# li199603/easy_gaussian_splatting

Hardware: AMD Instinct MI355X
Metric: train iters/sec + forward render fps, 1M Gaussians @ 1080p (higher is better)
Workload: dtype f32

## Files before the change

easy_gaussian_splatting_amd/_native.py:

```python
from __future__ import annotations

import ctypes as ct
import os
import subprocess
import threading
from typing import Optional

_HERE = os.path.dirname(os.path.abspath(__file__))
LIB_PATH = os.environ.get("GS_LIB_PATH") or os.path.join(_HERE, "libgsraster.so")
CSRC_DIR = os.path.join(_HERE, "csrc")
VARIANT_DIR = os.path.join(os.path.dirname(_HERE), "build", "variants")

GS_TILE = 16
GS_BUCKET = 64
GS_UNIT = 32
GS_REC_FLOATS = 12
GS_ROW_FLOATS = 12
GS_ROUND_BASE, GS_ROUND_SPLIT, GS_ROUND_LIVE, GS_ROUND_FRONT_N, GS_ROUND_LISTED_ALL, GS_ROUND_WORDS = 0, 1, 2, 3, 4, 8

_lib: Optional[ct.CDLL] = None
_lock = threading.Lock()

_P = ct.c_void_p
_I = ct.c_int
_L = ct.c_int64
_F = ct.c_float
_Z = ct.c_size_t

SIGNATURES = {
    "gs_version": (_I, []),
    "gs_build_flags": (ct.c_char_p, []),
    "gs_last_error": (ct.c_char_p, []),
    "gs_arch": (ct.c_char_p, []),
    "gs_bin_groups": (_I, [_L]),
    "gs_bin_workspace_bytes": (_Z, [_I, _L, _I, _I]),
    "gs_project_fwd": (_I, [_P, _I, _L, _I, _I, _P, _P, _P, _P, _P, _P, _I, _P, _P, _I, _I, _F, _F, _F, _F, _I, _I, _I,
                            _P, _P, _P, _P, _P, _P, _P, _P, _P, _P]),
    "gs_bin_count": (_I, [_P, _I, _L, _I, _I, _P, _P, _Z, _P, _P, _P, _P, _P]),
    "gs_bin_emit_sort": (_I, [_P, _I, _L, _I, _I, _P, _P, _P, _Z, _P, _L, _L, _P, _P, _P, _P, _P, _P]),
    "gs_bins_workspace_bytes": (_Z, [_I, _L, _I, _I, _I, _L]),
    "gs_bins_count": (_I, [_P, _I, _L, _I, _I, _I, _P, _P, _P, _Z, _P, _L, _L, _P, _P, _P, _P, _P, _P]),
    "gs_bins_lists": (_I, [_P, _I, _L, _I, _I, _I, _P, _P, _Z, _P, _L, _P, _P, _P, _P, _P, _P]),
    "gs_walk_state_ints": (_Z, [_L]),
    "gs_blend_fwd": (_I, [_P, _I, _I, _I, _P, _P, _P, _P, _P, _P, _L, _P, _P, _P, _P, _P, _P, _P, _L, _P, _L, _P]),
    "gs_blend_bwd": (_I, [_P, _I, _I, _I, _P, _P, _P, _P, _L, _P, _P, _P, _P, _P, _P, _P, _P, _P, _P]),
    "gs_unit_classes_ints": (_Z, [_L, _I, _I, _I]),
    "gs_rec_colors": (_I, [_P, _I, _L, _I, _P, _I, _P, _P]),
    "gs_blend_fwd_ch": (_I, [_P, _I, _I, _I, _I, _P, _P, _P, _P, _P, _P, _L, _P, _P, _P, _P, _P, _P, _P, _L, _P, _L, _P, _P]),
    "gs_blend_bwd_ch": (_I, [_P, _I, _I, _I, _I, _P, _P, _P, _P, _L, _P, _P, _P, _P, _P, _P, _P, _P, _P, _P, _P]),
    "gs_channel_grads": (_I, [_P, _I, _L, _I, _I, _P, _P, _P, _P, _P, _P, _P]),
    "gs_project_bwd": (_I, [_P, _I, _L, _I, _I, _P, _P, _P, _P, _P, _I, _P, _P, _I, _I, _F, _F, _F,
                            _P, _P, _P, _P, _P, _P, _P, _P, _P, _P, _P, _P, _P, _P, _P, _P, _P, _P, _P, _I, _P, _P, _P, _P]),
    "gs_cam_partials_doubles": (_Z, [_I, _L]),
    "gs_project_bwd_cam": (_I, [_P, _I, _L, _I, _I, _P, _P, _P, _P, _P, _I, _P, _P, _I, _I, _F, _F, _F,
                                _P, _P, _P, _P, _P, _P, _P, _P, _P, _P, _P, _P, _P, _P, _P, _P, _P, _P, _P, _I, _P, _P, _P, _P,
                                _P, _P, _P]),
    "gs_row_sums": (_I, [_P, _I, _L, _P, _P, _P, _P, _P, _P, _P, _P, _P, _P, _F, _P, _P]),
    "gs_sh_adam_views": (_I, [_P, _I, _L, _I, _I, _P, _P, _L, _P, _P, _P, _P, _P, _P, _F, _F, _F, _F, _F, _L, _F, _P]),
    "gs_sh_grad_views": (_I, [_P, _I, _L, _I, _I, _P, _P, _P, _P, _P]),
    "gs_loss_workspace_floats": (_Z, [_I, _I]),
    "gs_l1_ssim_fwd": (_I, [_P, _I, _I, _F, _P, _P, _P, _I, _P, _P]),
    "gs_l1_ssim_bwd": (_I, [_P, _I, _I, _F, _P, _P, _P, _I, _P, _P, _P]),
    "gs_l1_ssim_fwd_slots": (_I, [_P, _I, _I, _F, _P, _P, _I, _I, _P, _P]),
    "gs_l1_ssim_bwd_slots": (_I, [_P, _I, _I, _F, _P, _P, _I, _P, _P, _P]),
    "gs_clamp01": (_I, [_P, _L, _P, _P, _P]),
    "gs_pack_view_step": (_I, [_P, _L, _F, _P, _P, _P, _P, _P, _P, _P]),
    "gs_update_statistics": (_I, [_P, _L, _F, _P, _P, _P, _P, _P]),
    "gs_guard_set": (_I, [_P, _L, _L]),
    "gs_guard_set_call": (_I, [_P, _L, _L]),
    "gs_info_mirror_set": (_I, [_P]),
    "gs_walk_mirror_set": (_I, [_P]),
    "gs_rounds_set": (_I, [_P, _P, _P, _P, _I]),
    "gs_round_split": (_I, [_P, _L, _P, _P, _F, _P, _P]),
    "gs_round_footprints": (_I, [_P, _L, _I, _I, _P, _P, _P, _P]),
    "gs_round_status": (_I, [_P, _P, _P]),
    "gs_step_status": (_I, [_P, _P, _P, _P, _P, _P, _I, _P]),
    "gs_guard_flag_out": (_I, [_P, _P, _P, _P]),
    "gs_guard_merge": (_I, [_P, _P, _P, _I, _L]),
    "gs_step_applied": (_I, [_P, _P, _P]),
    "gs_adam_hyper": (_I, [_P, _I, _P, _F, _F, _L, _P]),
    "gs_step_inputs": (_I, [_P, _I, _P, _F, _F, _L, _P, _P, _P, _P, _P, _P, _P, _P]),
    "gs_adam_step_dev": (_I, [_P, _L, _P, _P, _P, _I, _P, _P, _P, _F, _F, _F, _F, _P, _P]),
    "gs_scan_rows_workspace_ints": (_Z, [_I, _L]),
    "gs_scan_rows_i32": (_I, [_P, _I, _L, _P, _P, _P]),
    "gs_refine_flags": (_I, [_P, _L, _I, _F, _F, _F, _F, _F, _P, _P, _P, _P, _P, _P, _P]),
    "gs_refine_apply": (_I, [_P, _L, _I, _I, _P, _P, _L, _L, _L, _P, _P, _P, _P, _P, _P, _P, _P, _P, _P, _P]),
    "gs_project_bwd_adam": (_I, [_P, _L, _I, _I, _P, _P, _P, _P, _P, _P, _I, _I, _F, _F, _F, _P, _P, _P, _P, _P, _P, _P, _P, _F, _F, _F, _P, _P,
                                  _P, _P, _P, _P]),
    "gs_project_bwd_adam_reg": (_I, [_P, _L, _I, _I, _P, _P, _P, _P, _P, _P, _I, _I, _F, _F, _F, _P, _P, _P, _P, _P, _P, _P, _P, _F, _F, _F, _P,
                                      _P, _P, _P, _P, _P, _F, _F]),
    "gs_scale_reg_workspace_floats": (_Z, [_L]),
    "gs_scale_reg": (_I, [_P, _L, _P, _F, _F, _P, _P, _P]),
    "gs_workspace_query": (_I, [_I, _L, _I, _I, _L, _L, _L, _L, _I, _I, _P, _P]),
    "gs_workspace_bind": (_I, [_P, _P, _L, _P, _L, _P, _L, _P, _P]),
    "gs_adam_step": (_I, [_P, _L, _P, _P, _P, _I, _P, _P, _P, _P, _F, _F, _F, _L, _F]),
    "gs_adam_step_stats": (_I, [_P, _L, _P, _P, _P, _I, _P, _P, _P, _P, _F, _F, _F, _L, _F, _L, _P, _P, _P, _P]),
}


class NativeLibraryError(RuntimeError):
    pass


def build(verbose: bool = False, clean: bool = False) -> str:
    if clean:
        subprocess.run(["make", "-C", CSRC_DIR, "clean"], capture_output=True, text=True)
    proc = subprocess.run(["make", "-C", CSRC_DIR, "-j4"], capture_output=True, text=True)
    if verbose or proc.returncode != 0:
        print(proc.stdout)
        print(proc.stderr)
    if proc.returncode != 0:
        raise NativeLibraryError("building libgsraster.so failed:\n" + proc.stderr[-4000:])
    return LIB_PATH


def build_variant(name: str, extra_flags: str) -> str:
    import glob
    import shutil
    import tempfile
    os.makedirs(VARIANT_DIR, exist_ok=True)
    out = os.path.join(VARIANT_DIR, f"libgsraster_{name}.so")
    srcs = [f for pat in ("*.hip", "*.h", "*.inc", "Makefile") for f in glob.glob(os.path.join(CSRC_DIR, pat))]
    if os.path.exists(out) and all(os.path.getmtime(out) >= os.path.getmtime(f) for f in srcs + [os.path.join(_HERE, "..", "include", "gs_raster.h")]):
        return out
    d = tempfile.mkdtemp(prefix=f"gsvar_{name}_")
    try:
        header = os.path.abspath(os.path.join(_HERE, "..", "include", "gs_raster.h"))
        for f in srcs:
            text = open(f).read().replace("../../include/gs_raster.h", header)
            open(os.path.join(d, os.path.basename(f)), "w").write(text)
        proc = subprocess.run(["make", "-C", d, "-j4", f"EXTRA={extra_flags}", f"LIB={out}"], capture_output=True, text=True)
        if proc.returncode != 0:
            raise NativeLibraryError(f"building {out} failed:\n" + proc.stderr[-4000:])
    finally:
        shutil.rmtree(d, ignore_errors=True)
    return out


def lib() -> ct.CDLL:
    global _lib
    if _lib is None:
        with _lock:
            if _lib is None:
                if not os.path.exists(LIB_PATH):
                    raise NativeLibraryError(
# ... 28 lines not shown
```

easy_gaussian_splatting_amd/csrc/gs_blend.hip:

```cpp
#include <algorithm>

#include "gs_common.h"
#include "gs_math.h"

namespace gs {

#ifdef GS_BWD_CHECK
struct BwdCheck {
    float* fwd_T;
    int32_t* fwd_cnt;
    float2* unit_out;
    int2* unit_hdr;
};
static BwdCheck g_bwd_check = {nullptr, nullptr, nullptr, nullptr};
#define GS_IF_CHECK(...) __VA_ARGS__
#else
#define GS_IF_CHECK(...)
#endif

constexpr int kUnit = GS_UNIT;
constexpr int kChunk = 8;
constexpr int kUnitLog = 128;
constexpr int kWalkUnits = GS_WALK_UNITS, kWalkStorage = GS_WALK_STORAGE, kWalkRows = GS_WALK_ROWS,
              kWalkFlags = GS_WALK_FLAGS, kWalkSkip = GS_WALK_SKIP;
constexpr int kScanThreads = 256, kScanPerThread = 32, kScanChunk = kScanThreads * kScanPerThread;

struct BlendFwdArgs {
    const int32_t* tile_order;
    int C, W, H, tw, tiles;
    const float4* rec;
    const float* bg;
    const int32_t *isect_offsets, *flatten_ids, *slots;
    float *out_colors, *out_alphas;
    float4* ckpt;
    int2* qlist;
    int32_t* qcnt;
    uint8_t* qmask;
    int4* unit_desc;
    int32_t* walk;
    int cap_units;
    unsigned long long* flags;
    const int64_t* guard;
    int64_t* rblk;
    uint8_t* live;
    float4* tstate;
    int4* trec;
    int solo;
    GS_IF_CHECK(BwdCheck chk;)
};

#ifdef GS_CLOCK_PROBE
__device__ unsigned long long gs_clk_acc[4];
struct ClockProbe {
    long long c0, w0; int slot;
    __device__ ClockProbe(int s) : c0(clock64()), w0(wall_clock64()), slot(s) {}
    __device__ ~ClockProbe() {
        if ((threadIdx.x & 63) == 0) {
            atomicAdd(&gs_clk_acc[slot], (unsigned long long)(clock64() - c0));
            atomicAdd(&gs_clk_acc[slot + 1], (unsigned long long)(wall_clock64() - w0));
        }
    }
};
#define GS_CLOCK_PROBE_SCOPE(slot) ClockProbe clock_probe_(slot)
#else
#define GS_CLOCK_PROBE_SCOPE(slot)
#endif

#ifdef GS_EXACT_MATH
__device__ __forceinline__ float fast_exp2(float x) { return (float)exp2((double)x); }
__device__ __forceinline__ float fast_rcp(float x) { return (float)(1.0 / (double)x); }
#else
__device__ __forceinline__ float fast_exp2(float x) { return __builtin_amdgcn_exp2f(x); }
__device__ __forceinline__ float fast_rcp(float x) { return __builtin_amdgcn_rcpf(x); }
#endif

constexpr float kDoneScale = 18446744073709551616.f;
constexpr float kDoneInv = 5.421010862427522e-20f;
__device__ __forceinline__ bool px_live(float T) { return T <= 1.f; }
__device__ __forceinline__ float px_final_T(float T) { return T > 2.f ? T * kDoneInv : T; }
__device__ __forceinline__ void blend_masked(const float am, const float r, const float g, const float b, float& T, float& cr,
                                             float& cg, float& cb) {
    float w = am * T;
    float Tn = fmaf(-am, T, T);
    const bool stop = Tn <= kTMin;
    if (__builtin_expect(__builtin_amdgcn_ballot_w64(stop) != 0ull, 0)) {
        w = stop ? 0.f : w;
        Tn = stop ? T * kDoneScale : Tn;
    }
    cr = fmaf(r, w, cr); cg = fmaf(g, w, cg); cb = fmaf(b, w, cb);
    T = Tn;
}
__device__ __forceinline__ void blend_pair(const float alpha, const bool ok, const float r,
                                           const float g, const float b, float& T, float& cr,
                                           float& cg, float& cb) {
    blend_masked(ok ? alpha : 0.f, r, g, b, T, cr, cg, cb);
}
__device__ __forceinline__ void blend_masked4(const float am, const float r, const float g, const float b, const float c3, float& T,
                                              float& cr, float& cg, float& cb, float& ca) {
    float w = am * T;
    float Tn = fmaf(-am, T, T);
    const bool stop = Tn <= kTMin;
    if (__builtin_expect(__builtin_amdgcn_ballot_w64(stop) != 0ull, 0)) {
        w = stop ? 0.f : w;
        Tn = stop ? T * kDoneScale : Tn;
    }
    cr = fmaf(r, w, cr); cg = fmaf(g, w, cg); cb = fmaf(b, w, cb); ca = fmaf(c3, w, ca);
    T = Tn;
}
__device__ __forceinline__ void blend_pair4(const float alpha, const bool ok, const float r, const float g, const float b,
                                            const float c3, float& T, float& cr, float& cg, float& cb, float& ca) {
    blend_masked4(ok ? alpha : 0.f, r, g, b, c3, T, cr, cg, cb, ca);
}

#define GS_FWD_ATTR __attribute__((amdgpu_waves_per_eu(CKPT ? 5 : 1, 8)))

__device__ __forceinline__ int64_t slots_in_use(int64_t n, const int64_t* guard) {
    return guard != nullptr ? min(n, guard[0]) : n;
}

__global__ __launch_bounds__(256) void qmask_clear_kernel(uint8_t* __restrict__ q, int64_t n_cap, int32_t* __restrict__ walk, int walk_ints,
                                                          const int64_t* __restrict__ guard, const int64_t* __restrict__ rblk, int phase) {
    bool skip = guard_tripped(guard);
    if (phase == 2) skip = skip || walk[kWalkSkip] != 0;
    if (blockIdx.x == 0 && threadIdx.x == 0) walk[kWalkSkip] = skip ? 1 : 0;
    if (skip) return;
    const int64_t first = phase == 2 ? min(rblk[GS_ROUND_BASE], slots_in_use(n_cap, guard)) : 0;
    const int64_t n = slots_in_use(n_cap, guard) - first;
    q += first;
    if (phase != 2)
        for (int i = (int)blockIdx.x * 256 + (int)threadIdx.x; i < walk_ints; i += (int)gridDim.x * 256)
            if (i != kWalkSkip) walk[i] = 0;
    const int64_t head = min(n, (int64_t)((16 - ((uintptr_t)q & 15)) & 15));
    const int64_t n16 = (n - head) >> 4;
    uint4* q16 = reinterpret_cast<uint4*>(q + head);
    for (int64_t i = (int64_t)blockIdx.x * 256 + threadIdx.x; i < n16; i += (int64_t)gridDim.x * 256) q16[i] = make_uint4(0u, 0u, 0u, 0u);
    if (blockIdx.x == 0) {
        if ((int64_t)threadIdx.x < head) q[threadIdx.x] = 0;
        const int64_t tail0 = head + (n16 << 4);
        if (tail0 + (int64_t)threadIdx.x < n) q[tail0 + threadIdx.x] = 0;
    }
}

template <bool CKPT, int WAVES, int ROUND, int NC>
__device__ __forceinline__ void blend_fwd_body(const BlendFwdArgs& a, float* __restrict__ ckpt_ext) {
    static_assert(NC >= 1 && NC <= 4 && (NC == 3 || ROUND == 0), "channels 1..4; depth rounds with 3 channels only");
    __shared__ float4 srec_all[WAVES][GS_BUCKET * 3];
    __shared__ int2 ulog_all[CKPT ? WAVES : 1][CKPT ? kUnitLog : 1];
    __shared__ int uring_all[CKPT ? WAVES : 1][CKPT ? 16 : 1];
    float4* srec = srec_all[threadIdx.x >> 6];
    int2* ulog = ulog_all[CKPT ? (threadIdx.x >> 6) : 0];
    int* uring = uring_all[CKPT ? (threadIdx.x >> 6) : 0];
    const int ti = CKPT ? __builtin_amdgcn_readfirstlane((int)blockIdx.x * WAVES + (int)(threadIdx.x >> 6))
                        : (int)blockIdx.x * WAVES + (int)(threadIdx.x >> 6);
    if (ti >= a.C * a.tiles) return;
    if (CKPT ? a.walk[kWalkSkip] != 0 : guard_tripped(a.guard)) return;
    if (ROUND == 2 && a.rblk[GS_ROUND_LIVE] == 0) return;
    GS_CLOCK_PROBE_SCOPE(0);
    const int t = a.tile_order ? a.tile_order[ti] : ti;
    const int cam = t / a.tiles, tt = t - cam * a.tiles;
    const int tyi = tt / a.tw, txi = tt - tyi * a.tw;
    const int lane = threadIdx.x & 63;
    const int x0 = txi * GS_TILE, y0 = tyi * GS_TILE;
    const int px0 = x0 + (lane & 7), py0 = y0 + (lane >> 3);
    const float fx0 = (float)px0 + 0.5f, fy0 = (float)py0 + 0.5f, fx1 = fx0 + 8.f, fy1 = fy0 + 8.f;
    const int lo = a.isect_offsets[t], hi = a.isect_offsets[t + 1];
    const int len = hi - lo;
    const int nb = (len + GS_BUCKET - 1) / GS_BUCKET;
    const unsigned long long lt_mask = (1ull << lane) - 1ull;
    if (ROUND == 2 && (len == 0 || a.live[t] == 0)) return;

    float T[4], cr[4], cg[4], cb[4];
    float ca[4];
    int cnt[4] = {0, 0, 0, 0};
    int pool_next = 0, pool_left = 0, log_n = 0;
    int room[4] = {0, 0, 0, 0};
    const int range_len = (a.cap_units / GS_WALK_RANGES) & ~(kChunk - 1), range0 = (ti & (GS_WALK_RANGES - 1)) * range_len;
    int32_t* range_ctr = a.walk + GS_WALK_RANGE0 + 32 * (ti & (GS_WALK_RANGES - 1));
    GS_IF_CHECK(int taken[4] = {0, 0, 0, 0};)
#pragma unroll
    for (int k = 0; k < 4; ++k) {
        cr[k] = cg[k] = cb[k] = 0.f;
        ca[k] = 0.f;
        T[k] = ((px0 + 8 * (k & 1)) < a.W && (py0 + 8 * (k >> 1)) < a.H) ? 1.f : kDoneScale;
    }
    if (ROUND == 2) {
#pragma unroll
        for (int k = 0; k < 4; ++k) {
            const float4 s4 = a.tstate[((size_t)t * 4 + k) * 64 + lane];
            T[k] = s4.x; cr[k] = s4.y; cg[k] = s4.z; cb[k] = s4.w;
        }
        if (CKPT) {
            const int4 rc = a.trec[2 * (size_t)t], ru = a.trec[2 * (size_t)t + 1];
            cnt[0] = __builtin_amdgcn_readfirstlane(rc.x); cnt[1] = __builtin_amdgcn_readfirstlane(rc.y);
            cnt[2] = __builtin_amdgcn_readfirstlane(rc.z); cnt[3] = __builtin_amdgcn_readfirstlane(rc.w);
            const int ru4[4] = {ru.x, ru.y, ru.z, ru.w};
#pragma unroll
            for (int k = 0; k < 4; ++k) {
                room[k] = -cnt[k] & (kUnit - 1);
                if (lane == 0 && cnt[k] > 0) uring[4 * k + (((cnt[k] - 1) / kUnit) & 3)] = ru4[k];
            }
        }
    }
    const float qxlo[2] = {(float)x0 + 0.5f, (float)x0 + 8.5f}, qxhi[2] = {(float)x0 + 7.5f, (float)x0 + 15.5f};
    const float qylo[2] = {(float)y0 + 0.5f, (float)y0 + 8.5f}, qyhi[2] = {(float)y0 + 7.5f, (float)y0 + 15.5f};

    auto publish = [&]() {
        if (log_n == 0) return;
        int base = 0;
        if (lane == 0) base = atomicAdd(a.walk + kWalkUnits, log_n);
        base = __builtin_amdgcn_readfirstlane(base);
        __builtin_amdgcn_wave_barrier();
        for (int j = lane; j < log_n; j += 64) {
            const int2 e = ulog[j];
            if (base + j < a.cap_units) a.unit_desc[base + j] = make_int4(4 * t + (e.y & 3), e.y >> 2, e.x, 0);
// ... 115 lines not shown
    if (ROUND == 1) {
        const bool lv = __builtin_amdgcn_ballot_w64(px_live(T[0]) || px_live(T[1]) || px_live(T[2]) || px_live(T[3])) != 0ull;
        if (lane == 0) {
            a.live[t] = lv ? 1 : 0;
            if (lv) atomicAdd(reinterpret_cast<unsigned long long*>(a.rblk + GS_ROUND_LIVE), 1ull);
            if (lv && a.solo && a.flags) atomicOr(a.flags, (unsigned long long)GS_FLAG_BACK);
        }
        if (lv && !a.solo) {
#pragma unroll
            for (int k = 0; k < 4; ++k) a.tstate[((size_t)t * 4 + k) * 64 + lane] = make_float4(T[k], cr[k], cg[k], cb[k]);
            if (CKPT && lane == 0) {
                a.trec[2 * (size_t)t] = make_int4(cnt[0], cnt[1], cnt[2], cnt[3]);
                int ru[4];
#pragma unroll
                for (int k = 0; k < 4; ++k) ru[k] = cnt[k] > 0 ? uring[4 * k + (((cnt[k] - 1) / kUnit) & 3)] : 0;
                a.trec[2 * (size_t)t + 1] = make_int4(ru[0], ru[1], ru[2], ru[3]);
            }
        }
    }
    float bgr = 0.f, bgg = 0.f, bgb = 0.f, bga = 0.f;
    if (a.bg) {
        bgr = a.bg[NC * cam];
        if (NC > 1) bgg = a.bg[NC * cam + 1];
        if (NC > 2) bgb = a.bg[NC * cam + 2];
        if (NC > 3) bga = a.bg[NC * cam + 3];
    }
#pragma unroll
    for (int k = 0; k < 4; ++k) {
        const int px = px0 + 8 * (k & 1), py = py0 + 8 * (k >> 1);
        if (px < a.W && py < a.H) {
            const size_t o = ((size_t)cam * a.H + py) * a.W + px;
            const float Tf = px_final_T(T[k]);
            a.out_colors[NC * o] = cr[k] + Tf * bgr;
            if (NC > 1) a.out_colors[NC * o + 1] = cg[k] + Tf * bgg;
            if (NC > 2) a.out_colors[NC * o + 2] = cb[k] + Tf * bgb;
            if (NC > 3) a.out_colors[NC * o + 3] = ca[k] + Tf * bga;
            a.out_alphas[o] = 1.f - Tf;
            GS_IF_CHECK(if (CKPT && a.chk.fwd_T) { a.chk.fwd_T[o] = Tf; a.chk.fwd_cnt[o] = taken[k]; })
        }
    }
}

template <bool CKPT, int WAVES, int ROUND>
__global__ __launch_bounds__(64 * WAVES) GS_FWD_ATTR void blend_fwd_kernel(const BlendFwdArgs a) {
    blend_fwd_body<CKPT, WAVES, ROUND, 3>(a, nullptr);
}
template <bool CKPT, int WAVES, int NC>
__global__ __launch_bounds__(64 * WAVES) __attribute__((amdgpu_waves_per_eu(CKPT ? (NC == 4 ? 4 : 5) : 1, 8))) void chan_fwd_kernel(const BlendFwdArgs a, float* ckpt_ext) {
    blend_fwd_body<CKPT, WAVES, 0, NC>(a, ckpt_ext);
}

struct RowScanArgs {
    const uint8_t* qmask;
    int32_t* row_base;
    int32_t* walk;
    int64_t n_cap, cap_rows;
    unsigned long long* flags;
    const int64_t* guard;
    volatile int64_t* mirror;
};

__device__ __forceinline__ int32_t row_counts32(const uint8_t* __restrict__ qmask, int64_t i0, int64_t n, uint32_t (&w)[8]) {
#pragma unroll
    for (int j = 0; j < 8; ++j) w[j] = 0u;
    if (i0 + kScanPerThread <= n) {
        const uint4 x = reinterpret_cast<const uint4*>(qmask + i0)[0], y = reinterpret_cast<const uint4*>(qmask + i0)[1];
        w[0] = x.x; w[1] = x.y; w[2] = x.z; w[3] = x.w; w[4] = y.x; w[5] = y.y; w[6] = y.z; w[7] = y.w;
    } else {
        for (int j = 0; j < kScanPerThread; ++j)
            if (i0 + j < n) w[j >> 2] |= (uint32_t)qmask[i0 + j] << (8 * (j & 3));
    }
    int32_t tot = 0;
#pragma unroll
    for (int j = 0; j < 8; ++j) {
        uint32_t v = w[j] & 0x0f0f0f0fu;
        v = v - ((v >> 1) & 0x55555555u);
        v = (v & 0x33333333u) + ((v >> 2) & 0x33333333u);
        w[j] = v;
        tot += (int32_t)((v * 0x01010101u) >> 24);
    }
    return tot;
}

__global__ __launch_bounds__(kScanThreads) void row_count_kernel(const RowScanArgs a) {
    __shared__ int32_t scratch[20];
    if (a.walk[kWalkSkip] != 0) return;
    const int64_t n = slots_in_use(a.n_cap, a.guard);
    const int64_t c0 = (int64_t)blockIdx.x * kScanChunk;
    if (c0 > n) return;
    uint32_t w[8];
    const int32_t tot = row_counts32(a.qmask, c0 + (int64_t)threadIdx.x * kScanPerThread, n, w);
    int32_t block_tot;
    block_excl_scan_add<int32_t>(tot, scratch, &block_tot);
    if (threadIdx.x == 0) a.walk[GS_WALK_WORDS + blockIdx.x] = block_tot;
}

__global__ __launch_bounds__(1024) void row_chunk_scan_kernel(const RowScanArgs a) {
    __shared__ int32_t scratch[20];
    if (a.walk[kWalkSkip] != 0) return;
    const int64_t n = slots_in_use(a.n_cap, a.guard);
    const int nb = (int)(n / kScanChunk) + 1;
    int32_t* part = a.walk + GS_WALK_WORDS;
    const int per = (nb + 1023) / 1024;
    const int j0 = (int)threadIdx.x * per, j1 = min(nb, j0 + per);
    int32_t mine = 0;
    for (int j = j0; j < j1; ++j) mine += part[j];
    int32_t total;
    int32_t run = block_excl_scan_add<int32_t>(mine, scratch, &total);
    for (int j = j0; j < j1; ++j) { const int32_t c = part[j]; part[j] = run; run += c; }
    if (threadIdx.x == 0) {
        int32_t fullest = 0;
        for (int r = 0; r < GS_WALK_RANGES; ++r) fullest = max(fullest, a.walk[GS_WALK_RANGE0 + 32 * r]);
        a.walk[kWalkStorage] = GS_WALK_RANGES * fullest;
        a.walk[kWalkRows] = total;
        int fl = a.walk[kWalkFlags];
        if (a.flags && (fl & GS_FLAG_UNITS)) atomicOr(a.flags, (unsigned long long)GS_FLAG_UNITS);
        if ((int64_t)total > a.cap_rows) {
            fl |= GS_FLAG_ROWS;
            a.walk[kWalkFlags] = fl;
            if (a.flags) atomicOr(a.flags, (unsigned long long)GS_FLAG_ROWS);
        }
        if (a.mirror) {
            a.mirror[0] = a.walk[kWalkUnits]; a.mirror[1] = a.walk[kWalkStorage]; a.mirror[2] = total; a.mirror[3] = fl;
            __threadfence_system();
        }
    }
}

__global__ __launch_bounds__(kScanThreads) void row_base_kernel(const RowScanArgs a) {
    __shared__ int32_t scratch[20];
    if (a.walk[kWalkSkip] != 0) return;
    const int64_t n = slots_in_use(a.n_cap, a.guard);
    const int64_t c0 = (int64_t)blockIdx.x * kScanChunk;
    if (c0 > n) return;
    const int64_t i0 = c0 + (int64_t)threadIdx.x * kScanPerThread;
    uint32_t w[8];
    const int32_t tot = row_counts32(a.qmask, i0, n, w);
    int32_t block_tot;
    const int32_t run = block_excl_scan_add<int32_t>(tot, scratch, &block_tot) + a.walk[GS_WALK_WORDS + blockIdx.x];
    int32_t first16 = 0;
#pragma unroll
    for (int j = 0; j < 4; ++j) first16 += (int32_t)((w[j] * 0x01010101u) >> 24);
    if (i0 <= n) a.row_base[i0 >> 4] = run;
    if (i0 + 16 <= n) a.row_base[(i0 >> 4) + 1] = run + first16;
}

struct BlendBwdArgs {
    int C, W, H, tw, tiles;
    const float4* rec;
    const int32_t* walk;
    const int2* qlist;
    const int32_t* qcnt;
    const int4* unit_desc;
    const float4* ckpt;
    const uint8_t* qmask;
    const int32_t* row_base;
    int cap_units;
    const int32_t* cls_hdr;
    const int4* cls_desc;
    int cls_cap;
    const float *out_colors, *out_alphas, *v_colors, *v_alphas;
    float4* rows;
    const int64_t* guard;
    GS_IF_CHECK(BwdCheck chk;)
};

constexpr int kBwdWaves = 4;
constexpr int kPipeLanes = 8;
constexpr int kPerLane = kUnit / kPipeLanes;
static_assert(kPerLane == 4, "bwd_wave is instantiated for 1 .. 4 entries per lane");
constexpr int kUnitsPerWave = 64 / kPipeLanes;
constexpr int kUnitPixels = 64;
constexpr int kBwdSteps = kUnitPixels + kPipeLanes - 1;

__device__ __forceinline__ float dpp_row_shr1(float v) {
    return __builtin_bit_cast(float, __builtin_amdgcn_update_dpp(__builtin_bit_cast(int, v), __builtin_bit_cast(int, v), 0x111, 0xf, 0xf, false));
}


#ifdef GS_BWD_ACC64
typedef double acc_t;
#define GS_ACC_FMA(a, b, c) ((double)(a) * (double)(b) + (c))
#else
typedef float acc_t;
#define GS_ACC_FMA(a, b, c) fmaf((a), (b), (c))
#endif
struct EntryState {
    float mx, my, hA, Bc, hC, op, colr, colg, colb, At, Bt, Ct;
    acc_t s_mx, s_my, s_ax, s_ay, s_A, s_B, s_C, s_vs, s_r, s_g, s_b;
    bool has;
    float col3; acc_t s_3;
};

template <int NC>
__device__ __forceinline__ void bwd_pair(EntryState& e, const float4 d0, const float v3, const float2 d1, float& T, float& P) {
    const float dx = e.mx - d1.x, dy = e.my - d1.y;
    const float sigma = fmaf(dy, fmaf(e.hC, dy, e.Bc * dx), e.hA * dx * dx);
    const float vis = fast_exp2(-sigma);
    const float ov = e.op * vis;
    const float alpha = fminf(kAlphaMax, ov);
    const bool ok = T > 0.f && sigma >= 0.f && alpha >= kAlphaMin;
    const float w = alpha * T;
    const float Tn = fmaf(-alpha, T, T);
    const bool stop = ok && Tn <= kTMin;
    const bool contrib = ok && !stop;
    float cv = e.colr * d0.x + e.colg * d0.y + e.colb * d0.z;
    if constexpr (NC == 4) cv = fmaf(e.col3, v3, cv);
    const float wm = contrib ? w : 0.f;
    const float Pn = fmaf(wm, cv, P);
    const float ra = fast_rcp(1.f - alpha);
    const float v_alpha = fmaf(T, cv, ra * (d0.w + Pn));
    e.s_r = GS_ACC_FMA(wm, d0.x, e.s_r); e.s_g = GS_ACC_FMA(wm, d0.y, e.s_g); e.s_b = GS_ACC_FMA(wm, d0.z, e.s_b);
    if constexpr (NC == 4) e.s_3 = GS_ACC_FMA(wm, v3, e.s_3);
    const float vs = (contrib && ov <= kAlphaMax) ? -ov * v_alpha : 0.f;
    const float hx = vs * dx, hy = vs * dy;
    e.s_A = GS_ACC_FMA(hx, dx, e.s_A); e.s_B = GS_ACC_FMA(hx, dy, e.s_B); e.s_C = GS_ACC_FMA(hy, dy, e.s_C);
    const float gx = fmaf(e.At, hx, e.Bt * hy), gy = fmaf(e.Bt, hx, e.Ct * hy);
    e.s_mx += (acc_t)gx; e.s_my += (acc_t)gy; e.s_ax += (acc_t)fabsf(gx); e.s_ay += (acc_t)fabsf(gy);
    e.s_vs += (acc_t)vs;
    T = contrib ? Tn : (stop ? -1.f : T);
    P = Pn;
}

template <int E, int NC>
__device__ __forceinline__ void bwd_wave(const BlendBwdArgs& a, const int4 ud, const bool valid, const int unit, float4* sd0, float* sd1,
                                         float2* sck, const int r, const float* __restrict__ ckpt_ext) {
    const int tq = ud.x, su = ud.z;
// ... 52 lines not shown
    }
#pragma unroll
    for (int i = 0; i < kPix; ++i) {
        const int p = r + kPipeLanes * i;
        const bool inside = valid && (qx0 + (p & 7)) < a.W && (qy0 + (p >> 3)) < a.H;
        const float vr = l_vr[i], vg = l_vg[i], vb = l_vb[i];
        const float Tf = 1.f - l_oa[i];
        const float va = a.v_alphas ? l_va[i] : 0.f;
        float Ev = Tf * va - (l_cr[i] * vr + l_cg[i] * vg + l_cb[i] * vb);
        const float4 ck = first_unit ? make_float4(1.f, 0.f, 0.f, 0.f) : l_ck[i];
        float Pk = ck.y * vr + ck.z * vg + ck.w * vb;
        if constexpr (NC == 4) {
            const float v3 = l_v3[i];
            Ev = Tf * va - fmaf(l_c3[i], v3, l_cr[i] * vr + l_cg[i] * vg + l_cb[i] * vb);
            Pk = fmaf(first_unit ? 0.f : l_k3[i], v3, Pk);
            sd1[p] = inside ? v3 : 0.f;
        }
        sd0[p] = inside ? make_float4(vr, vg, vb, Ev) : make_float4(0.f, 0.f, 0.f, 0.f);
        sck[p] = inside ? make_float2(ck.x, Pk) : make_float2(-1.f, 0.f);
    }

    EntryState e[E];
    int slot[E];
#pragma unroll
    for (int i = 0; i < E; ++i) {
        const int en = E * r + i;
        e[i].has = en < n_in;
        slot[i] = e[i].has ? gs[i].y : 0;
        const float4 z4 = make_float4(0.f, 0.f, 0.f, 0.f);
        const float4 q0 = e[i].has ? rq[i][0] : z4, q1 = e[i].has ? rq[i][1] : z4, q2 = e[i].has ? rq[i][2] : z4;
        e[i].mx = q0.x; e[i].my = q0.y; e[i].hA = q0.z; e[i].Bc = q0.w; e[i].hC = q1.x; e[i].op = q1.y;
        e[i].colr = q2.x; e[i].colg = q2.y; e[i].colb = q2.z;
        e[i].col3 = q2.w; e[i].s_3 = (acc_t)0;
        e[i].At = 2.f * kLn2 * q0.z; e[i].Bt = kLn2 * q0.w; e[i].Ct = 2.f * kLn2 * q1.x;
        e[i].s_mx = e[i].s_my = e[i].s_ax = e[i].s_ay = e[i].s_A = e[i].s_B = e[i].s_C = e[i].s_vs = (acc_t)0;
        e[i].s_r = e[i].s_g = e[i].s_b = (acc_t)0;
    }
    __builtin_amdgcn_wave_barrier();

    float T_out = -1.f, P_out = 0.f;
    GS_IF_CHECK(float D_out = -1.f, C_out = 0.f; if (valid && r == 0 && a.chk.unit_hdr) a.chk.unit_hdr[unit] = make_int2(tq, ud.y);)
    for (int s = 0; s < kBwdSteps; ++s) {
        float T = dpp_row_shr1(T_out), P = dpp_row_shr1(P_out);
        const int p = s - r;
        const bool act = (unsigned)p < (unsigned)kUnitPixels;
        const int pc = min(max(p, 0), kUnitPixels - 1);
        const float4 d0 = sd0[pc];
        const float v3 = NC == 4 ? sd1[pc] : 0.f;
        const float2 ck = sck[pc];
        const float2 d1 = make_float2(fx0 + (float)(pc & 7), fy0 + (float)(pc >> 3));
        if (r == 0) { T = ck.x; P = ck.y; }
        T = act ? T : -1.f;
        GS_IF_CHECK(float D = dpp_row_shr1(D_out), Cn = dpp_row_shr1(C_out); if (r == 0) { D = ck.x; Cn = 0.f; } if (!act) { D = -1.f; Cn = 0.f; })
#pragma unroll
        for (int i = 0; i < E; ++i) {
            GS_IF_CHECK(const float T_before = T;)
            bwd_pair<NC>(e[i], d0, v3, d1, T, P);
            GS_IF_CHECK(if (T > 0.f && T < T_before) { D = T; Cn += 1.f; })
        }
        GS_IF_CHECK(D_out = D; C_out = Cn;
                    if (valid && act && r == kPipeLanes - 1 && a.chk.unit_out) a.chk.unit_out[(size_t)unit * 64 + p] = make_float2(D, Cn);)
        T_out = T; P_out = P;
    }

    int row[E];
#pragma unroll
    for (int i = 0; i < E; ++i) {
        int m;
        row[i] = rows_before(a.row_base, a.qmask, slot[i], &m);
        row[i] += __popc((unsigned)m & ((1u << q) - 1u));
    }
#pragma unroll
    for (int i = 0; i < E; ++i) {
        if (e[i].has) {
            float4* rp = a.rows + (GS_ROW_FLOATS / 4) * (size_t)row[i];
            const float v_op = e[i].op > 0.f ? (float)(-e[i].s_vs / (acc_t)e[i].op) : 0.f;
            rp[0] = make_float4((float)e[i].s_mx, (float)e[i].s_my, (float)e[i].s_ax, (float)e[i].s_ay);
            rp[1] = make_float4((float)((acc_t)0.5f * e[i].s_A), (float)e[i].s_B, (float)((acc_t)0.5f * e[i].s_C), v_op);
            rp[2] = make_float4((float)e[i].s_r, (float)e[i].s_g, (float)e[i].s_b, NC == 4 ? (float)e[i].s_3 : 0.f);
        }
    }
}

constexpr int kClsHdrInts = 16, kClsThreads = 1024;
__global__ __launch_bounds__(64) void unit_classes_clear_kernel(int32_t* __restrict__ hdr) {
    if (threadIdx.x < kClsHdrInts) hdr[threadIdx.x] = 0;
}
__global__ __launch_bounds__(kClsThreads) void unit_classes_kernel(const int32_t* __restrict__ walk, const int4* __restrict__ unit_desc,
                                                                   const int32_t* __restrict__ qcnt, int cap_units, int cls_cap,
                                                                   int32_t* __restrict__ hdr, int4* __restrict__ cls, const int64_t* __restrict__ guard) {
    __shared__ int s_cnt[kClsThreads / 64][4], s_base[kClsThreads / 64][4];
    if (guard_tripped(guard)) return;
    const int n_units = min(walk[kWalkUnits], cap_units);
    if ((int)blockIdx.x * kClsThreads >= n_units) return;
    const int u = (int)blockIdx.x * kClsThreads + (int)threadIdx.x, wave = threadIdx.x >> 6, lane = threadIdx.x & 63;
    int c = 0;
    int4 ud = make_int4(0, 0, 0, 0);
    if (u < n_units) {
        ud = unit_desc[u];
        const int n_in = min(kUnit, qcnt[ud.x] - ud.y * kUnit);
        c = min(max((n_in + kPipeLanes - 1) / kPipeLanes, 1), 4);
        ud.w = u;
    }
    unsigned long long m[4];
#pragma unroll
    for (int k = 0; k < 4; ++k) m[k] = __ballot(c == k + 1);
    if (lane < 4) s_cnt[wave][lane] = (int)__popcll(lane == 0 ? m[0] : (lane == 1 ? m[1] : (lane == 2 ? m[2] : m[3])));
    __syncthreads();
    if (threadIdx.x < 4) {
        int tot = 0;
        for (int w = 0; w < kClsThreads / 64; ++w) { s_base[w][threadIdx.x] = tot; tot += s_cnt[w][threadIdx.x]; }
        const int base = tot ? atomicAdd(hdr + 1 + threadIdx.x, tot) : 0;
        for (int w = 0; w < kClsThreads / 64; ++w) s_base[w][threadIdx.x] += base;
    }
    __syncthreads();
    if (c) {
        const unsigned long long mine = c == 1 ? m[0] : (c == 2 ? m[1] : (c == 3 ? m[2] : m[3]));
        const int i = s_base[wave][c - 1] + (int)__popcll(mine & ((1ull << lane) - 1ull));
        if (i < (c == 4 ? cap_units : cls_cap)) cls[(c == 4 ? 0 : cap_units + (3 - c) * cls_cap) + i] = ud;
    }
}

template <int NC>
__device__ __forceinline__ void blend_bwd_body(const BlendBwdArgs& a, const float* __restrict__ ckpt_ext) {
    __shared__ float4 sd0_all[kBwdWaves][kUnitsPerWave][64];
    __shared__ float2 sck_all[kBwdWaves][kUnitsPerWave][64];
    const int wave = threadIdx.x >> 6, lane = threadIdx.x & 63;
    const int pipe = lane / kPipeLanes, r = lane & (kPipeLanes - 1);
    if (guard_tripped(a.guard)) return;
    constexpr int kPerBlock = kBwdWaves * kUnitsPerWave;
    int cls = 4, blk = (int)blockIdx.x, n_units, first = 0;
    if (a.cls_hdr == nullptr) {
        n_units = min(a.walk[kWalkUnits], a.cap_units);
    } else {
        const int b4 = (a.cap_units + kPerBlock - 1) / kPerBlock, bt = (a.cls_cap + kPerBlock - 1) / kPerBlock;
        if (blk >= b4) {
            const int k = (blk - b4) / bt;
            cls = 3 - k; blk -= b4 + k * bt; first = a.cap_units + k * a.cls_cap;
        }
        n_units = min(a.cls_hdr[cls], cls == 4 ? a.cap_units : a.cls_cap);
    }
    const int in_class = (blk * kBwdWaves + wave) * kUnitsPerWave + pipe;
    if ((blk * kBwdWaves + wave) * kUnitsPerWave >= n_units) return;
    GS_CLOCK_PROBE_SCOPE(2);
    const bool valid = in_class < n_units;
    float4* sd0 = sd0_all[wave][pipe];
    float2* sck = sck_all[wave][pipe];
    float* sd1 = nullptr;
    if constexpr (NC == 4) {
        __shared__ float sd1_all[kBwdWaves][kUnitsPerWave][64];
        sd1 = sd1_all[wave][pipe];
    }

    int4 ud = make_int4(0, 0, 0, 0);
    if (valid) ud = a.cls_hdr ? a.cls_desc[first + in_class] : a.unit_desc[in_class];
    const int unit = a.cls_hdr ? ud.w : in_class;
    if (cls == 4) bwd_wave<4, NC>(a, ud, valid, unit, sd0, sd1, sck, r, ckpt_ext);
    else if (cls == 3) bwd_wave<3, NC>(a, ud, valid, unit, sd0, sd1, sck, r, ckpt_ext);
    else if (cls == 2) bwd_wave<2, NC>(a, ud, valid, unit, sd0, sd1, sck, r, ckpt_ext);
    else bwd_wave<1, NC>(a, ud, valid, unit, sd0, sd1, sck, r, ckpt_ext);
}

__global__ __launch_bounds__(kBwdWaves * 64) void blend_bwd_kernel(const BlendBwdArgs a) {
    blend_bwd_body<3>(a, nullptr);
}
template <int NC>
__global__ __launch_bounds__(kBwdWaves * 64) void chan_bwd_kernel(const BlendBwdArgs a, const float* ckpt_ext) {
    blend_bwd_body<NC>(a, ckpt_ext);
}

}

using namespace gs;

#ifdef GS_BWD_CHECK
extern "C" int gs_debug_bwd_check_set(float* fwd_T, int32_t* fwd_cnt, float* unit_out, int32_t* unit_hdr) {
    g_bwd_check.fwd_T = fwd_T; g_bwd_check.fwd_cnt = fwd_cnt;
    g_bwd_check.unit_out = reinterpret_cast<float2*>(unit_out); g_bwd_check.unit_hdr = reinterpret_cast<int2*>(unit_hdr);
    return GS_OK;
}
#endif

#ifdef GS_CLOCK_PROBE
extern "C" int gs_debug_clock_probe(int64_t* out4, int reset) {
    unsigned long long h[4] = {0, 0, 0, 0};
    if (out4) { GS_HIP_CHECK(hipMemcpyFromSymbol(h, HIP_SYMBOL(gs_clk_acc), sizeof(h))); for (int i = 0; i < 4; ++i) out4[i] = (int64_t)h[i]; }
    if (reset) { unsigned long long z[4] = {0, 0, 0, 0}; GS_HIP_CHECK(hipMemcpyToSymbol(HIP_SYMBOL(gs_clk_acc), z, sizeof(z))); }
    return GS_OK;
}
#endif

extern "C" size_t gs_walk_state_ints(int64_t n_isects) {
    if (n_isects < 0) return 0;
    return (size_t)GS_WALK_WORDS + (size_t)(n_isects / kScanChunk + 1);
}

template <int NC>
static int blend_fwd_launch(void* stream, int C, int width, int height, const float* rec,
                            const float* backgrounds, const int32_t* isect_offsets, const int32_t* tile_order,
                            const int32_t* flatten_ids, const int32_t* slots, int64_t n_isects, float* render_colors,
                            float* render_alphas, float* ckpt, int32_t* qlist, int32_t* qcnt, uint8_t* qmask,
                            int32_t* unit_desc, int64_t cap_units, int32_t* row_base, int64_t cap_rows, int32_t* walk_state,
                            float* ckpt_ext) {
    GS_REQUIRE(C >= 1 && width > 0 && height > 0 && n_isects >= 0, "C>=1, positive image size, n_isects>=0");
    GS_REQUIRE(isect_offsets && render_colors && render_alphas, "null pointer");
    const bool train = ckpt != nullptr;
    GS_REQUIRE(!train || (qlist && qcnt && qmask && unit_desc && row_base && walk_state && slots), "training mode needs every list output");
    GS_REQUIRE(!train || (cap_units >= kChunk * GS_WALK_RANGES && cap_units < (1ll << 26) && cap_rows >= 0 && cap_rows < (1ll << 31)),
               "training mode: 256 <= cap_units < 2^26 work units, cap_rows < 2^31 gradient rows");
    GS_REQUIRE(!train || n_isects < (1ll << 31) - kScanChunk, "training mode: the slots of a call are indexed by int32");
    static_assert(kScanPerThread == 32, "row_base_kernel writes two groups of 16 slots per thread");
    GS_REQUIRE(!train || (((uintptr_t)qmask & 15) == 0 && ((uintptr_t)row_base & 15) == 0 && ((uintptr_t)walk_state & 7) == 0),
               "training mode: qmask / row_base 16-byte aligned, walk_state 8-byte aligned");
    BlendFwdArgs a;
    a.C = C; a.W = width; a.H = height;
    a.tw = (width + GS_TILE - 1) / GS_TILE;
    a.tiles = a.tw * ((height + GS_TILE - 1) / GS_TILE);
    a.rec = reinterpret_cast<const float4*>(rec); a.bg = backgrounds; a.isect_offsets = isect_offsets;
    a.flatten_ids = flatten_ids; a.slots = slots;
    a.out_colors = render_colors; a.out_alphas = render_alphas;
    a.ckpt = reinterpret_cast<float4*>(ckpt); a.qlist = reinterpret_cast<int2*>(qlist); a.qcnt = qcnt; a.qmask = qmask;
    a.unit_desc = reinterpret_cast<int4*>(unit_desc); a.walk = walk_state; a.cap_units = (int)cap_units;
    a.tile_order = tile_order;
    a.guard = current_guard().info;
    a.flags = a.guard ? reinterpret_cast<unsigned long long*>(const_cast<int64_t*>(a.guard) + 3) : nullptr;
    const Rounds R = current_rounds();
    const int phase = (R.phase == 1 || R.phase == 4) ? 1 : (R.phase == 2 ? 2 : 0);
    a.solo = R.phase == 4 ? 1 : 0;
    GS_REQUIRE(R.phase != 4 || a.flags != nullptr, "depth rounds, front round alone: needs a step guard (gs_guard_set)");
    GS_REQUIRE(phase == 0 || C == 1, "depth rounds: one camera per call");
    GS_REQUIRE(phase == 0 || !train || R.tile_rec, "depth rounds, training mode: gs_rounds_set needs tile_rec");
    GS_REQUIRE(NC == 3 || phase == 0, "depth rounds render 3 channels only (tile_state holds T, r, g, b): clear gs_rounds_set");
    GS_REQUIRE(NC != 4 || !train || ckpt_ext, "channels = 4, training mode: ckpt_ext (cap_units * 64 floats) is required");
    a.rblk = R.blk; a.live = R.live; a.tstate = R.state; a.trec = reinterpret_cast<int4*>(R.tile_rec);
    GS_IF_CHECK(a.chk = g_bwd_check;)
    const unsigned n_tiles = (unsigned)(C * a.tiles);
    hipStream_t st = (hipStream_t)stream;
    constexpr int kFwdWaves = 4;
    const dim3 grid((n_tiles + kFwdWaves - 1) / kFwdWaves), block(64 * kFwdWaves);
    if (train) {
        const int walk_ints = (int)gs_walk_state_ints(n_isects);
        const unsigned cg = (unsigned)std::min<int64_t>(1024, std::max<int64_t>(1, (n_isects / 16 + 255) / 256));
        hipLaunchKernelGGL(qmask_clear_kernel, dim3(cg), dim3(256), 0, st, qmask, n_isects, walk_state, walk_ints, a.guard,
                           (const int64_t*)R.blk, phase);
        GS_LAUNCH_CHECK("qmask_clear_kernel");
        if constexpr (NC != 3) hipLaunchKernelGGL((chan_fwd_kernel<true, kFwdWaves, NC>), grid, block, 0, st, a, ckpt_ext);
        else if (phase == 1) hipLaunchKernelGGL((blend_fwd_kernel<true, kFwdWaves, 1>), grid, block, 0, st, a);
        else if (phase == 2) hipLaunchKernelGGL((blend_fwd_kernel<true, kFwdWaves, 2>), grid, block, 0, st, a);
        else hipLaunchKernelGGL((blend_fwd_kernel<true, kFwdWaves, 0>), grid, block, 0, st, a);
        GS_LAUNCH_CHECK("blend_fwd_kernel");
        if (phase == 1 && !a.solo) return GS_OK;
        RowScanArgs s;
        s.qmask = qmask; s.row_base = row_base; s.walk = walk_state; s.n_cap = n_isects; s.cap_rows = cap_rows;
        s.flags = a.flags; s.guard = a.guard; s.mirror = current_walk_mirror();
        const unsigned chunks = (unsigned)(n_isects / kScanChunk + 1);
        hipLaunchKernelGGL(row_count_kernel, dim3(chunks), dim3(kScanThreads), 0, st, s);
        hipLaunchKernelGGL(row_chunk_scan_kernel, dim3(1), dim3(1024), 0, st, s);
        hipLaunchKernelGGL(row_base_kernel, dim3(chunks), dim3(kScanThreads), 0, st, s);
        GS_LAUNCH_CHECK("row_base_kernel");
    } else {
        if constexpr (NC != 3) hipLaunchKernelGGL((chan_fwd_kernel<false, kFwdWaves, NC>), grid, block, 0, st, a, nullptr);
        else if (phase == 1) hipLaunchKernelGGL((blend_fwd_kernel<false, kFwdWaves, 1>), grid, block, 0, st, a);
        else if (phase == 2) hipLaunchKernelGGL((blend_fwd_kernel<false, kFwdWaves, 2>), grid, block, 0, st, a);
        else hipLaunchKernelGGL((blend_fwd_kernel<false, kFwdWaves, 0>), grid, block, 0, st, a);
        GS_LAUNCH_CHECK("blend_fwd_kernel");
    }
    return GS_OK;
}

extern "C" int gs_blend_fwd(void* stream, int C, int width, int height, const float* rec,
                            const float* backgrounds, const int32_t* isect_offsets, const int32_t* tile_order,
                            const int32_t* flatten_ids, const int32_t* slots, int64_t n_isects, float* render_colors,
                            float* render_alphas, float* ckpt, int32_t* qlist, int32_t* qcnt, uint8_t* qmask,
                            int32_t* unit_desc, int64_t cap_units, int32_t* row_base, int64_t cap_rows, int32_t* walk_state) {
    return blend_fwd_launch<3>(stream, C, width, height, rec, backgrounds, isect_offsets, tile_order, flatten_ids, slots, n_isects,
                               render_colors, render_alphas, ckpt, qlist, qcnt, qmask, unit_desc, cap_units, row_base, cap_rows,
                               walk_state, nullptr);
}

extern "C" int gs_blend_fwd_ch(void* stream, int C, int width, int height, int channels, const float* rec,
                               const float* backgrounds, const int32_t* isect_offsets, const int32_t* tile_order,
                               const int32_t* flatten_ids, const int32_t* slots, int64_t n_isects, float* render_colors,
                               float* render_alphas, float* ckpt, int32_t* qlist, int32_t* qcnt, uint8_t* qmask,
                               int32_t* unit_desc, int64_t cap_units, int32_t* row_base, int64_t cap_rows, int32_t* walk_state,
                               float* ckpt_ext) {
    GS_REQUIRE(channels >= 1 && channels <= 4, "channels must be 1, 2, 3 or 4");
#define GS_FWD_CH(NC) blend_fwd_launch<NC>(stream, C, width, height, rec, backgrounds, isect_offsets, tile_order, flatten_ids, slots, \
                                           n_isects, render_colors, render_alphas, ckpt, qlist, qcnt, qmask, unit_desc, cap_units,   \
                                           row_base, cap_rows, walk_state, ckpt_ext)
    switch (channels) {
        case 1: return GS_FWD_CH(1);
        case 2: return GS_FWD_CH(2);
        case 3: return GS_FWD_CH(3);
        default: return GS_FWD_CH(4);
    }
#undef GS_FWD_CH
}

static int64_t cls_region(int C, int width, int height) {
    const int64_t tiles = (int64_t)((width + GS_TILE - 1) / GS_TILE) * ((height + GS_TILE - 1) / GS_TILE);
    const int64_t per_block = kBwdWaves * kUnitsPerWave;
    return (4 * (int64_t)C * tiles + per_block - 1) / per_block * per_block;
}

extern "C" size_t gs_unit_classes_ints(int64_t cap_units, int C, int width, int height) {
    if (cap_units < 0 || C < 1 || width <= 0 || height <= 0) return 0;
    return (size_t)kClsHdrInts + 4 * ((size_t)cap_units + 3 * (size_t)cls_region(C, width, height));
}

template <int NC>
static int blend_bwd_launch(void* stream, int C, int width, int height, const float* rec,
                            const int32_t* qlist, const int32_t* qcnt, const int32_t* unit_desc, int64_t cap_units,
                            const float* ckpt, const uint8_t* qmask, const int32_t* row_base, const int32_t* walk_state,
                            const float* render_colors, const float* render_alphas, const float* v_render_colors,
                            const float* v_render_alphas, float* rows, int32_t* unit_classes, const float* ckpt_ext) {
    GS_REQUIRE(C >= 1 && width > 0 && height > 0 && cap_units >= 0 && cap_units < (1ll << 26), "C>=1, positive image size, 0 <= cap_units < 2^26");
    if (cap_units == 0) return GS_OK;
    GS_REQUIRE(rec && qlist && qcnt && unit_desc && ckpt && qmask && row_base && walk_state, "null list pointer");
    GS_REQUIRE(render_colors && render_alphas && v_render_colors && rows, "null image pointer");
    GS_REQUIRE(NC != 4 || ckpt_ext, "channels = 4: ckpt_ext (gs_blend_fwd_ch's fourth-channel checkpoints) is required");
    BlendBwdArgs a;
    a.C = C; a.W = width; a.H = height;
    a.tw = (width + GS_TILE - 1) / GS_TILE;
    a.tiles = a.tw * ((height + GS_TILE - 1) / GS_TILE);
    a.rec = reinterpret_cast<const float4*>(rec);
    a.qlist = reinterpret_cast<const int2*>(qlist); a.qcnt = qcnt; a.walk = walk_state;
    a.unit_desc = reinterpret_cast<const int4*>(unit_desc); a.cap_units = (int)cap_units;
    a.ckpt = reinterpret_cast<const float4*>(ckpt); a.qmask = qmask; a.row_base = row_base;
    a.out_colors = render_colors;
    a.out_alphas = render_alphas; a.v_colors = v_render_colors; a.v_alphas = v_render_alphas;
    a.rows = reinterpret_cast<float4*>(rows);
    a.guard = current_guard().info;
    GS_IF_CHECK(a.chk = g_bwd_check;)
    unsigned grid = (unsigned)((cap_units + kUnitsPerWave * kBwdWaves - 1) / (kUnitsPerWave * kBwdWaves));
    a.cls_hdr = nullptr; a.cls_desc = nullptr; a.cls_cap = 0;
    if (unit_classes) {
        GS_REQUIRE(((uintptr_t)unit_classes & 15) == 0, "unit_classes must be 16-byte aligned");
        a.cls_hdr = unit_classes; a.cls_desc = reinterpret_cast<const int4*>(unit_classes + kClsHdrInts);
        a.cls_cap = (int)cls_region(C, width, height);
        hipLaunchKernelGGL(unit_classes_clear_kernel, dim3(1), dim3(64), 0, (hipStream_t)stream, unit_classes);
        hipLaunchKernelGGL(unit_classes_kernel, dim3((unsigned)((cap_units + kClsThreads - 1) / kClsThreads)), dim3(kClsThreads), 0, (hipStream_t)stream,
                           walk_state, a.unit_desc, qcnt, (int)cap_units, a.cls_cap, unit_classes, reinterpret_cast<int4*>(unit_classes + kClsHdrInts),
                           a.guard);
        GS_LAUNCH_CHECK("unit_classes_kernel");
        grid += 3u * (unsigned)(a.cls_cap / (kUnitsPerWave * kBwdWaves));
    }
    if constexpr (NC == 3) hipLaunchKernelGGL(blend_bwd_kernel, dim3(grid), dim3(kBwdWaves * 64), 0, (hipStream_t)stream, a);
    else hipLaunchKernelGGL((chan_bwd_kernel<NC>), dim3(grid), dim3(kBwdWaves * 64), 0, (hipStream_t)stream, a, ckpt_ext);
    GS_LAUNCH_CHECK("blend_bwd_kernel");
    return GS_OK;
}

extern "C" int gs_blend_bwd(void* stream, int C, int width, int height, const float* rec,
                            const int32_t* qlist, const int32_t* qcnt, const int32_t* unit_desc, int64_t cap_units,
                            const float* ckpt, const uint8_t* qmask, const int32_t* row_base, const int32_t* walk_state,
                            const float* render_colors, const float* render_alphas, const float* v_render_colors,
                            const float* v_render_alphas, float* rows, int32_t* unit_classes) {
    return blend_bwd_launch<3>(stream, C, width, height, rec, qlist, qcnt, unit_desc, cap_units, ckpt, qmask, row_base, walk_state,
                               render_colors, render_alphas, v_render_colors, v_render_alphas, rows, unit_classes, nullptr);
}

extern "C" int gs_blend_bwd_ch(void* stream, int C, int width, int height, int channels, const float* rec,
                               const int32_t* qlist, const int32_t* qcnt, const int32_t* unit_desc, int64_t cap_units,
                               const float* ckpt, const uint8_t* qmask, const int32_t* row_base, const int32_t* walk_state,
                               const float* render_colors, const float* render_alphas, const float* v_render_colors,
                               const float* v_render_alphas, float* rows, int32_t* unit_classes, const float* ckpt_ext) {
    GS_REQUIRE(channels >= 1 && channels <= 4, "channels must be 1, 2, 3 or 4");
#define GS_BWD_CH(NC) blend_bwd_launch<NC>(stream, C, width, height, rec, qlist, qcnt, unit_desc, cap_units, ckpt, qmask, row_base, \
                                           walk_state, render_colors, render_alphas, v_render_colors, v_render_alphas, rows,         \
                                           unit_classes, ckpt_ext)
    switch (channels) {
        case 1: return GS_BWD_CH(1);
        case 2: return GS_BWD_CH(2);
        case 3: return GS_BWD_CH(3);
        default: return GS_BWD_CH(4);
    }
#undef GS_BWD_CH
}
```

easy_gaussian_splatting_amd/csrc/gs_capi.hip:

```cpp
#include <stdarg.h>

#include "gs_common.h"

namespace gs {
static thread_local char g_err[512] = "";
void set_error(const char* fmt, ...) {
    va_list ap;
    va_start(ap, fmt);
    vsnprintf(g_err, sizeof(g_err), fmt, ap);
    va_end(ap);
}
static thread_local Guard g_guard = {nullptr, 0, 0, 0};
Guard current_guard() { return g_guard; }
static thread_local int64_t* g_info_mirror = nullptr;
int64_t* current_info_mirror() { return g_info_mirror; }
static thread_local int64_t* g_walk_mirror = nullptr;
int64_t* current_walk_mirror() { return g_walk_mirror; }
static thread_local Rounds g_rounds = {nullptr, nullptr, nullptr, nullptr, 0};
Rounds current_rounds() { return g_rounds; }
}

extern "C" int gs_rounds_set(int64_t* rounds_dev, uint8_t* tile_live, float* tile_state, int32_t* tile_rec, int phase) {
    if (phase < 0 || phase > 4 || (phase != 0 && !rounds_dev) || ((phase == 1 || phase == 2 || phase == 4) && (!tile_live || !tile_state))) {
        gs::set_error("invalid argument: phase 0 (off), 1 (front round), 2 (back round), 3 (behind both) or 4 (front round alone); a round needs its buffers");
        return GS_ERR_ARG;
    }
    if ((((uintptr_t)tile_state) & 15) != 0 || (((uintptr_t)tile_rec) & 15) != 0) {
        gs::set_error("invalid argument: tile_state / tile_rec 16-byte aligned");
        return GS_ERR_ARG;
    }
    gs::g_rounds.blk = phase ? rounds_dev : nullptr;
    gs::g_rounds.live = phase ? tile_live : nullptr;
    gs::g_rounds.state = phase ? reinterpret_cast<float4*>(tile_state) : nullptr;
    gs::g_rounds.tile_rec = phase ? tile_rec : nullptr;
    gs::g_rounds.phase = phase;
    return GS_OK;
}

extern "C" int gs_info_mirror_set(int64_t* info_host_mapped) {
    gs::g_info_mirror = info_host_mapped;
    return GS_OK;
}

extern "C" int gs_walk_mirror_set(int64_t* walk_host_mapped) {
    gs::g_walk_mirror = walk_host_mapped;
    return GS_OK;
}

extern "C" int gs_guard_set(const int64_t* info_dev, int64_t cap_isects, int64_t cap_tile) {
    if (info_dev != nullptr && (cap_isects <= 0 || cap_tile <= 0)) {
        gs::set_error("invalid argument: a guard needs positive capacities");
        return GS_ERR_ARG;
    }
    gs::g_guard.info = info_dev;
    gs::g_guard.cap_isects = info_dev ? cap_isects : 0;
    gs::g_guard.cap_tile = info_dev ? cap_tile : 0;
    gs::g_guard.per_call = 0;
    return GS_OK;
}

extern "C" int gs_guard_set_call(const int64_t* info_dev, int64_t cap_isects, int64_t cap_tile) {
    if (int rc = gs_guard_set(info_dev, cap_isects, cap_tile)) return rc;
    gs::g_guard.per_call = info_dev != nullptr;
    return GS_OK;
}

namespace gs {
__global__ void step_status_kernel(const int64_t* __restrict__ info, const int64_t* __restrict__ applied,
                                   volatile int64_t* __restrict__ status, const float* __restrict__ loss3,
                                   float* __restrict__ loss_ring, int ring_len, const int32_t* __restrict__ walk,
                                   const int64_t* __restrict__ rblk) {
    if (threadIdx.x < 4) status[threadIdx.x] = info[threadIdx.x];
    if (threadIdx.x == 7) status[7] = rblk ? rblk[GS_ROUND_LIVE] : -1;
    if (threadIdx.x == 4) status[4] = applied ? applied[0] : 0;
    if (threadIdx.x == 5) status[5] = walk ? walk[GS_WALK_STORAGE] : 0;
    if (threadIdx.x == 6) status[6] = walk ? walk[GS_WALK_ROWS] : 0;
    if (loss_ring != nullptr && applied != nullptr && info[3] == 0 && threadIdx.x < 3 && applied[0] > 0)
        loss_ring[3 * ((applied[0] - 1) % ring_len) + threadIdx.x] = loss3[threadIdx.x];
    __threadfence_system();
}
}

extern "C" int gs_step_status(void* stream, const int64_t* info_dev, const int64_t* applied_dev, int64_t* status,
                              const float* loss3_dev, float* loss_ring_dev, int ring_len, const int32_t* walk_state) {
    if (!info_dev || !status || (loss_ring_dev && (!loss3_dev || ring_len <= 0))) {
        gs::set_error("invalid argument: null pointer / empty ring");
        return GS_ERR_ARG;
    }
    const gs::Rounds R = gs::current_rounds();
    hipLaunchKernelGGL(gs::step_status_kernel, dim3(1), dim3(64), 0, (hipStream_t)stream, info_dev, applied_dev, status, loss3_dev,
                       loss_ring_dev, ring_len, walk_state, (const int64_t*)(R.phase == 3 ? R.blk : nullptr));
    GS_LAUNCH_CHECK("step_status_kernel");
    return GS_OK;
}

namespace gs {
__global__ void guard_flag_out_kernel(const int64_t* __restrict__ info, float* __restrict__ dst0, float* __restrict__ dst1) {
    const float f = info[3] != 0 ? 1.f : 0.f;
    if (dst0) dst0[0] = f;
    if (dst1) dst1[0] = f;
}
__global__ void guard_merge_kernel(int64_t* __restrict__ info, const float* __restrict__ src, int n, int64_t stride) {
    bool any = false;
    for (int i = threadIdx.x; i < n; i += 64) any |= src[(int64_t)i * stride] != 0.f;
    if (__ballot(any) != 0ull && threadIdx.x == 0) info[3] |= GS_FLAG_PEER;
}
__global__ void step_applied_kernel(const int64_t* __restrict__ info, int64_t* __restrict__ applied) {
    if (info[3] == 0) applied[0] += 1;
}
}

extern "C" int gs_guard_flag_out(void* stream, const int64_t* info_dev, float* dst0, float* dst1) {
    if (!info_dev || (!dst0 && !dst1)) { gs::set_error("invalid argument: null pointer"); return GS_ERR_ARG; }
    hipLaunchKernelGGL(gs::guard_flag_out_kernel, dim3(1), dim3(1), 0, (hipStream_t)stream, info_dev, dst0, dst1);
    GS_LAUNCH_CHECK("guard_flag_out_kernel");
    return GS_OK;
}

extern "C" int gs_guard_merge(void* stream, int64_t* info_dev, const float* flags, int n, int64_t stride) {
    if (!info_dev || !flags || n < 1) { gs::set_error("invalid argument: null pointer / n < 1"); return GS_ERR_ARG; }
    hipLaunchKernelGGL(gs::guard_merge_kernel, dim3(1), dim3(64), 0, (hipStream_t)stream, info_dev, flags, n, stride);
    GS_LAUNCH_CHECK("guard_merge_kernel");
    return GS_OK;
}

extern "C" int gs_step_applied(void* stream, const int64_t* info_dev, int64_t* applied_dev) {
    if (!info_dev || !applied_dev) { gs::set_error("invalid argument: null pointer"); return GS_ERR_ARG; }
    hipLaunchKernelGGL(gs::step_applied_kernel, dim3(1), dim3(1), 0, (hipStream_t)stream, info_dev, applied_dev);
// ... 12 lines not shown
```

easy_gaussian_splatting_amd/csrc/gs_common.h:

```cpp
#pragma once
#include <hip/hip_runtime.h>
#include <stdint.h>
#include <stdio.h>
#include <string.h>

#include <map>
#include <mutex>
#include <utility>

#include "../../include/gs_raster.h"

namespace gs {

void set_error(const char* fmt, ...);

#define GS_HIP_CHECK(expr)                                                                   \
    do {                                                                                     \
        hipError_t _e = (expr);                                                              \
        if (_e != hipSuccess) {                                                              \
            gs::set_error("%s failed: %s (%s:%d)", #expr, hipGetErrorString(_e), __FILE__,   \
                          __LINE__);                                                         \
            return GS_ERR_HIP;                                                               \
        }                                                                                    \
    } while (0)

#define GS_LAUNCH_CHECK(name)                                                                \
    do {                                                                                     \
        hipError_t _e = hipGetLastError();                                                   \
        if (_e != hipSuccess) {                                                              \
            gs::set_error("launch of %s failed: %s", name, hipGetErrorString(_e));           \
            return GS_ERR_HIP;                                                               \
        }                                                                                    \
    } while (0)

inline int ensure_lds(const void* fn, size_t bytes) {
    if (bytes > 64 * 1024) {
        static std::mutex mu;
        static std::map<std::pair<int, const void*>, size_t> done;
        int dev = 0;
        GS_HIP_CHECK(hipGetDevice(&dev));
        std::lock_guard<std::mutex> lock(mu);
        size_t& have = done[{dev, fn}];
        if (have < bytes) {
            GS_HIP_CHECK(hipFuncSetAttribute(fn, hipFuncAttributeMaxDynamicSharedMemorySize, (int)bytes));
            have = bytes;
        }
    }
    return GS_OK;
}

#define GS_REQUIRE(cond, msg)                                                                \
    do {                                                                                     \
        if (!(cond)) {                                                                       \
            gs::set_error("invalid argument: %s (%s)", msg, #cond);                          \
            return GS_ERR_ARG;                                                               \
        }                                                                                    \
    } while (0)

constexpr int kWave = 64;

struct Guard {
    const int64_t* info;
    int64_t cap_isects;
    int64_t cap_tile;
    int per_call;
};
Guard current_guard();
int64_t* current_info_mirror();
int64_t* current_walk_mirror();
__device__ __forceinline__ bool guard_tripped(const int64_t* info) { return info != nullptr && info[3] != 0; }

struct Rounds {
    int64_t* blk;
    uint8_t* live;
    float4* state;
    int32_t* tile_rec;
    int phase;
};
Rounds current_rounds();
__device__ __forceinline__ bool round_idle(const int64_t* blk, int phase) { return phase == 2 && blk[GS_ROUND_LIVE] == 0; }

__device__ __forceinline__ int rows_before(const int32_t* __restrict__ row_base16, const uint8_t* __restrict__ qmask, int s, int* slot_mask = nullptr) {
    const int g = s >> 4, k = s & 15;
    const uint4 q = reinterpret_cast<const uint4*>(qmask)[g];
    const uint32_t w[4] = {q.x, q.y, q.z, q.w};
    int n = row_base16[g];
#pragma unroll
    for (int j = 0; j < 4; ++j) {
        const int b = min(max(k - 4 * j, 0), 4);
        const uint32_t m = b >= 4 ? 0xffffffffu : ((1u << (8 * b)) - 1u);
        n += __popc(w[j] & m & 0x0f0f0f0fu);
    }
    if (slot_mask) *slot_mask = (int)((w[k >> 2] >> (8 * (k & 3))) & 0xfu);
    return n;
}

struct BinLayout {
    int groups;
    int64_t per_group;
    size_t hist_off;
    size_t tile_cnt_off;
    size_t grp_tot_off;
    size_t grp_base_off;
    size_t items_off;
    size_t total;
};
BinLayout bin_layout(int C, int64_t N, int tiles);

__device__ __forceinline__ int div_by_width(int i, float inv_w) { return (int)(((float)i + 0.5f) * inv_w); }

__device__ __forceinline__ int lane_id() { return threadIdx.x & 63; }

template <typename T>
__device__ __forceinline__ T wave_incl_scan_add(T v) {
#pragma unroll
    for (int d = 1; d < 64; d <<= 1) {
        T o = __shfl_up(v, d, 64);
        if (lane_id() >= d) v += o;
    }
    return v;
}

template <typename T>
__device__ __forceinline__ T wave_reduce_add(T v) {
#pragma unroll
    for (int d = 32; d > 0; d >>= 1) v += __shfl_xor(v, d, 64);
    return v;
}

__device__ __forceinline__ float wave_reduce_add_dpp(float v) {
#define GS_DPP_ADD(ctrl, row_mask) \
    v += __builtin_bit_cast(float, __builtin_amdgcn_update_dpp(0, __builtin_bit_cast(int, v), ctrl, row_mask, 0xf, false))
    GS_DPP_ADD(0xB1, 0xf);
    GS_DPP_ADD(0x4E, 0xf);
    GS_DPP_ADD(0x141, 0xf);
    GS_DPP_ADD(0x140, 0xf);
    GS_DPP_ADD(0x142, 0xa);
    GS_DPP_ADD(0x143, 0xc);
#undef GS_DPP_ADD
    return __builtin_bit_cast(float, __builtin_amdgcn_readlane(__builtin_bit_cast(int, v), 63));
}

template <typename T>
__device__ __forceinline__ T block_excl_scan_add(T v, T* scratch, T* total) {
    const int lane = lane_id(), wave = threadIdx.x >> 6, nw = (blockDim.x + 63) >> 6;
    T incl = wave_incl_scan_add(v);
    if (lane == 63) scratch[wave] = incl;
    __syncthreads();
    if (wave == 0) {
        T w = lane < nw ? scratch[lane] : T(0);
        T wi = wave_incl_scan_add(w);
        if (lane < nw) scratch[lane] = wi - w;
// ... 65 lines not shown
```

easy_gaussian_splatting_amd/csrc/gs_loss.hip:

```cpp
#include "gs_common.h"

namespace gs {

constexpr int kLT = 32;
constexpr int kHalo = 5;
constexpr int kLR = kLT + 2 * kHalo;
constexpr int kLRP = kLR + 1;
constexpr int kHP = kLT + 1;
static_assert(kLT * (kLT / 4) == 256 && kLR * 6 <= 256 && kLR % 6 == 0, "thread mapping of the staging and the separable passes");
static_assert(kLR % 2 == 0 && kLR * 3 <= 128, "backward staging: two 128-thread halves, one staged row each");
constexpr int64_t kLossMaxPixels = (int64_t)1 << 28;
constexpr int kLossMaxWidth = 1 << 20;
constexpr float kC1 = 0.01f * 0.01f, kC2 = 0.03f * 0.03f;

#define GS_WIN_TAPS {1.0283800845e-03f, 7.5987581352e-03f, 3.6000772128e-02f, 1.0936068951e-01f, 2.1300553771e-01f, \
                     2.6601172486e-01f, 2.1300553771e-01f, 1.0936068951e-01f, 3.6000772128e-02f, 7.5987581352e-03f, 1.0283800845e-03f}

struct LossArgs {
    int H, W;
    int clamp_input;
    float lambda_ssim;
    const float *render, *gt, *mask;
    const float* const* slots;
    float* maps;
    float* partial;
    const float* gout;
    float* v_render;
};

__device__ __forceinline__ int clampi(int v, int lo, int hi) { return v < lo ? lo : (v > hi ? hi : v); }
__device__ __forceinline__ float ld_off(const float* base, unsigned byte_off) {
    return *reinterpret_cast<const float*>(reinterpret_cast<const char*>(base) + byte_off);
}
__device__ __forceinline__ void st_off(float* base, unsigned byte_off, float v) {
    *reinterpret_cast<float*>(reinterpret_cast<char*>(base) + byte_off) = v;
}

struct F3 { float x, y, z; };
__device__ __forceinline__ F3 ld3_off(const float* base, unsigned byte_off) {
    return *reinterpret_cast<const F3*>(reinterpret_cast<const char*>(base) + byte_off);
}
__device__ __forceinline__ void st3_off(float* base, unsigned byte_off, float x, float y, float z) {
    *reinterpret_cast<F3*>(reinterpret_cast<char*>(base) + byte_off) = F3{x, y, z};
}

__device__ __forceinline__ bool loss_tile(const LossArgs& a, int& x0, int& y0) {
    const int ntx = (a.W + kLT - 1) / kLT, nt = ntx * ((a.H + kLT - 1) / kLT), per = (nt + 7) >> 3;
    const int id = blockIdx.x, t = (id & 7) * per + (id >> 3);
    if ((id >> 3) >= per || t >= nt) return false;
    const int ty = t / ntx;
    x0 = (t - ty * ntx) * kLT; y0 = ty * kLT;
    return true;
}

__device__ __forceinline__ bool loss_tile_channel(const LossArgs& a, int& x0, int& y0, int& ch) {
    const int ntx = (a.W + kLT - 1) / kLT, nt = ntx * ((a.H + kLT - 1) / kLT), per = (nt + 7) >> 3;
    const int id = blockIdx.x, k = id >> 3, local = k / 3, t = (id & 7) * per + local;
    ch = k - 3 * local;
    if (t >= nt) return false;
    const int ty = t / ntx;
    x0 = (t - ty * ntx) * kLT; y0 = ty * kLT;
    return true;
}

constexpr int kHOut = 6, kHWin = kHOut + 10;

template <bool MASK>
__global__ __launch_bounds__(256) void l1_ssim_fwd_kernel(const LossArgs a) {
    constexpr float kWin[11] = GS_WIN_TAPS;
    extern __shared__ __attribute__((aligned(16))) float lds[];
    float* sx = lds;
    float* sy = sx + kLR * kLRP;
    float* hp = sy + kLR * kLRP;
    __shared__ float red[2][4];
    int x0, y0;
    if (!loss_tile(a, x0, y0)) {
        if (threadIdx.x == 0) { a.partial[2 * blockIdx.x] = 0.f; a.partial[2 * blockIdx.x + 1] = 0.f; }
        return;
    }
    const int tid = threadIdx.x;
    const unsigned row_bytes = 12u * (unsigned)a.W;
    const float* gt_img = a.slots ? a.slots[0] : a.gt;
    const float* mask_img = a.slots ? a.slots[1] : a.mask;
    constexpr int kPer = kLR / 6;
    float rv[kPer][3], gv[kPer][3], mv[MASK ? kPer : 1];
    if (tid < kLR * 6) {
        const int rg = tid / kLR, col = tid - rg * kLR;
        const int cx = clampi(x0 - kHalo + col, 0, a.W - 1), ytop = y0 - kHalo + rg;
#pragma unroll
        for (int i = 0; i < kPer; ++i) {
            const unsigned cy = (unsigned)clampi(ytop + 6 * i, 0, a.H - 1);
            const unsigned o = __umul24(cy, row_bytes) + 12u * (unsigned)cx;
            const F3 g3 = ld3_off(gt_img, o), r3 = ld3_off(a.render, o);
            gv[i][0] = g3.x; gv[i][1] = g3.y; gv[i][2] = g3.z;
            rv[i][0] = r3.x; rv[i][1] = r3.y; rv[i][2] = r3.z;
            if (MASK) mv[i] = ld_off(mask_img, __umul24(cy, 4u * (unsigned)a.W) + 4u * (unsigned)cx);
        }
    }
    float l1 = 0.f, ssim_sum = 0.f;
#pragma unroll 1
    for (int ch = 0; ch < 3; ++ch) {
        int t = tid;
        asm volatile("" : "+v"(t));
        const bool st_on = t < kLR * 6;
        const int rg = t / kLR, col = t - rg * kLR;
        if (st_on) {
            const int gx = x0 - kHalo + col;
            const bool col_own = col >= kHalo && col < kHalo + kLT && gx < a.W;
            float* dx = sx + rg * kLRP + col;
            float* dy = sy + rg * kLRP + col;
#pragma unroll
            for (int i = 0; i < kPer; ++i) {
                const int row = rg + 6 * i, gy = y0 - kHalo + row;
                const float g = gv[i][0];
                float r = rv[i][0];
                if (a.clamp_input) r = fminf(fmaxf(r, 0.f), 1.f);
                if (MASK) r = mv[i] * g + (1.f - mv[i]) * r;
                dx[6 * i * kLRP] = r;
                dy[6 * i * kLRP] = g;
                if (col_own && row >= kHalo && row < kHalo + kLT && gy < a.H) l1 += fabsf(r - g);
                gv[i][0] = gv[i][1]; gv[i][1] = gv[i][2];
                rv[i][0] = rv[i][1]; rv[i][1] = rv[i][2];
            }
        }
        __syncthreads();
        float* maps_c = a.maps + (size_t)ch * a.H * a.W * 3;
        {
            const bool h_on = st_on;
            const int row = col, c0 = min(kHOut * rg, kLT - kHOut);
            if (h_on) {
                float* h = hp + row * kHP + c0;
                float xv[kHWin], yv[kHWin];
#pragma unroll
                for (int i = 0; i < kHWin; ++i) { xv[i] = sx[row * kLRP + c0 + i]; yv[i] = sy[row * kLRP + c0 + i]; }
#pragma unroll
                for (int j = 0; j < kHOut; ++j) {
                    float m0 = kWin[0] * xv[j], m1 = kWin[0] * yv[j], m2 = kWin[0] * fmaf(xv[j], xv[j], yv[j] * yv[j]),
                          m3 = kWin[0] * (xv[j] * yv[j]);
#pragma unroll
                    for (int kk = 1; kk < 11; ++kk) {
                        const float w = kWin[kk], x = xv[j + kk], y = yv[j + kk];
                        m0 = fmaf(w, x, m0); m1 = fmaf(w, y, m1); m2 = fmaf(w, fmaf(x, x, y * y), m2); m3 = fmaf(w, x * y, m3);
                    }
                    h[j] = m0; h[kLR * kHP + j] = m1; h[2 * kLR * kHP + j] = m2; h[3 * kLR * kHP + j] = m3;
                }
            }
        }
        __syncthreads();
        {
            const int q = t / kLT, vcol = t - q * kLT, r0 = 4 * q;
            float mom[4][4];
#pragma unroll
            for (int mi = 0; mi < 4; ++mi) {
                float hv[14];
#pragma unroll
                for (int i = 0; i < 14; ++i) hv[i] = hp[mi * kLR * kHP + (r0 + i) * kHP + vcol];
#pragma unroll
                for (int j = 0; j < 4; ++j) {
                    float acc = kWin[0] * hv[j];
#pragma unroll
                    for (int kk = 1; kk < 11; ++kk) acc = fmaf(kWin[kk], hv[j + kk], acc);
                    mom[mi][j] = acc;
                }
            }
            const int gx = x0 + vcol;
#pragma unroll
            for (int j = 0; j < 4; ++j) {
                const int gy = y0 + r0 + j;
                const float mu_x = mom[0][j], mu_y = mom[1][j], ess = mom[2][j], exy = mom[3][j];
                const bool interior = gy >= kHalo && gy < a.H - kHalo && gx >= kHalo && gx < a.W - kHalo;
                if (gy < a.H && gx < a.W) {
                    float dmu = 0.f, dxx = 0.f, dxy = 0.f;
                    if (interior) {
                        const float mm = mu_x * mu_x + mu_y * mu_y, sxy = exy - mu_x * mu_y;
                        const float n1 = 2.f * mu_x * mu_y + kC1, n2 = 2.f * sxy + kC2;
                        const float d1 = mm + kC1, d2 = (ess - mm) + kC2;
                        const float i1 = __builtin_amdgcn_rcpf(d1), i2 = __builtin_amdgcn_rcpf(d2), inv = i1 * i2;
                        const float sv = n1 * n2 * inv;
                        ssim_sum += sv;
                        dxx = -sv * i2;
                        dxy = 2.f * n1 * inv;
                        dmu = 2.f * mu_y * (n2 - n1) * inv + 2.f * mu_x * sv * (i2 - i1);
                    }
                    st3_off(maps_c, __umul24((unsigned)gy, row_bytes) + 12u * (unsigned)gx, dmu, dxx, dxy);
                }
            }
        }
        if (ch < 2) __syncthreads();
    }
    l1 = wave_reduce_add(l1);
    ssim_sum = wave_reduce_add(ssim_sum);
    if (lane_id() == 0) { red[0][tid >> 6] = l1; red[1][tid >> 6] = ssim_sum; }
    __syncthreads();
    if (tid == 0) {
        a.partial[2 * blockIdx.x] = red[0][0] + red[0][1] + red[0][2] + red[0][3];
        a.partial[2 * blockIdx.x + 1] = red[1][0] + red[1][1] + red[1][2] + red[1][3];
    }
}

__global__ __launch_bounds__(256) void loss_reduce_kernel(int nblocks, const float* __restrict__ partial, int H, int W,
                                                          float lambda_ssim, float* __restrict__ out) {
    __shared__ double red[2][4];
    double s0 = 0.0, s1 = 0.0;
    for (int i = threadIdx.x; i < nblocks; i += 256) { s0 += partial[2 * i]; s1 += partial[2 * i + 1]; }
#pragma unroll
    for (int d = 32; d > 0; d >>= 1) { s0 += __shfl_xor(s0, d, 64); s1 += __shfl_xor(s1, d, 64); }
    if (lane_id() == 0) { red[0][threadIdx.x >> 6] = s0; red[1][threadIdx.x >> 6] = s1; }
    __syncthreads();
    if (threadIdx.x == 0) {
        const double l1 = (red[0][0] + red[0][1] + red[0][2] + red[0][3]) / ((double)H * W * 3.0);
        const double cnt = (double)(H - 2 * kHalo) * (double)(W - 2 * kHalo) * 3.0;
        const double ssim = (red[1][0] + red[1][1] + red[1][2] + red[1][3]) / cnt;
        out[0] = (float)l1; out[1] = (float)(1.0 - ssim);
        out[2] = (float)((1.0 - lambda_ssim) * l1 + lambda_ssim * (1.0 - ssim));
    }
}

__global__ __launch_bounds__(256) void l1_ssim_bwd_kernel(const LossArgs a) {
    constexpr float kWin[11] = GS_WIN_TAPS;
    extern __shared__ __attribute__((aligned(16))) float lds[];
    float* sm = lds;
    float* hp = lds;
    int x0, y0, ch;
    if (!loss_tile_channel(a, x0, y0, ch)) return;
    const int tid = threadIdx.x;
    const size_t plane = (size_t)a.H * a.W;
    const float g = a.gout[0];
    const float cnt = (float)(a.H - 2 * kHalo) * (float)(a.W - 2 * kHalo) * 3.f;
    const float k_ssim = -g * a.lambda_ssim / cnt;
    const float k_l1 = g * (1.f - a.lambda_ssim) / ((float)a.H * (float)a.W * 3.f);
    const unsigned row_bytes = 12u * (unsigned)a.W;
    const int q = tid / kLT, ocol = tid - q * kLT, r0 = 4 * q, ogx = x0 + ocol;
    const bool col_in = ogx < a.W;
    const unsigned o0 = __umul24((unsigned)min(y0 + r0, a.H - 1), row_bytes) + 12u * (unsigned)min(ogx, a.W - 1);
    const float* mask_img = a.slots ? a.slots[1] : a.mask;
    const float* gt_c = (a.slots ? a.slots[0] : a.gt) + ch;
    const float* render_c = a.render + ch;
    float gtv[4], rr[4], mk[4];
#pragma unroll
    for (int j = 0; j < 4; ++j) {
        const unsigned o = o0 + (y0 + r0 + j < a.H ? j * row_bytes : 0u);
        gtv[j] = ld_off(gt_c, o); rr[j] = ld_off(render_c, o);
        if (mask_img) mk[j] = ld_off(mask_img, o / 3u);
    }
    {
        constexpr int kRowsPer = kLR / 2;
        const int half = __builtin_amdgcn_readfirstlane(tid >> 7), jj = tid & 127;
        const int scol = jj / 3, smi = jj - scol * 3;
        const int sgx = x0 - kHalo + scol;
        const float* maps_c = a.maps + (size_t)ch * plane * 3;
        if (jj < kLR * 3) {
            const bool col_ok = sgx >= 0 && sgx < a.W;
            const unsigned lane_off = 4u * (unsigned)(clampi(sgx, 0, a.W - 1) * 3 + smi);
            float v[kRowsPer];
            const int gy0 = y0 - kHalo + half;
            const char* rowp = reinterpret_cast<const char*>(maps_c) + (int64_t)gy0 * row_bytes;
#pragma unroll
            for (int i = 0; i < kRowsPer; ++i) {
                const int gy = gy0 + 2 * i;
                v[i] = 0.f;
                if (gy >= 0 && gy < a.H) v[i] = ld_off(reinterpret_cast<const float*>(rowp), lane_off);
                rowp += 2 * row_bytes;
            }
            float* d = sm + (smi * kLR + half) * kLRP + scol;
#pragma unroll
            for (int i = 0; i < kRowsPer; ++i) d[2 * i * kLRP] = col_ok ? v[i] : 0.f;
        }
    }
    __syncthreads();
    {
        const bool h_on = tid < kLR * 6;
        const int hg = tid / kLR, row = tid - hg * kLR, c0 = min(kHOut * hg, kLT - kHOut);
        float ho[3][kHOut];
        if (h_on) {
#pragma unroll
            for (int mi = 0; mi < 3; ++mi) {
                float w[kHWin];
#pragma unroll
                for (int i = 0; i < kHWin; ++i) w[i] = sm[(mi * kLR + row) * kLRP + c0 + i];
#pragma unroll
                for (int j = 0; j < kHOut; ++j) {
                    float acc = kWin[0] * w[j];
#pragma unroll
                    for (int k = 1; k < 11; ++k) acc = fmaf(kWin[k], w[j + k], acc);
                    ho[mi][j] = acc;
                }
            }
        }
        __syncthreads();
        if (h_on) {
#pragma unroll
            for (int mi = 0; mi < 3; ++mi)
#pragma unroll
                for (int j = 0; j < kHOut; ++j) hp[mi * kLR * kHP + row * kHP + c0 + j] = ho[mi][j];
        }
    }
    __syncthreads();
    {
        float c[3][4];
#pragma unroll
        for (int mi = 0; mi < 3; ++mi) {
            float hv[14];
#pragma unroll
            for (int i = 0; i < 14; ++i) hv[i] = hp[mi * kLR * kHP + (r0 + i) * kHP + ocol];
#pragma unroll
            for (int j = 0; j < 4; ++j) {
                float acc = kWin[0] * hv[j];
#pragma unroll
                for (int k = 1; k < 11; ++k) acc = fmaf(kWin[k], hv[j + k], acc);
                c[mi][j] = acc;
            }
        }
        float* out_c = a.v_render + ch;
#pragma unroll
        for (int j = 0; j < 4; ++j) {
            if (y0 + r0 + j >= a.H || !col_in) continue;
            float r = rr[j], keep = 1.f;
            if (a.clamp_input) { keep = (r >= 0.f && r <= 1.f) ? 1.f : 0.f; r = fminf(fmaxf(r, 0.f), 1.f); }
            if (mask_img) { r = mk[j] * gtv[j] + (1.f - mk[j]) * r; keep *= 1.f - mk[j]; }
            const float d = r - gtv[j];
            const float sgn = d > 0.f ? 1.f : (d < 0.f ? -1.f : 0.f);
            st_off(out_c, o0 + j * row_bytes, keep * (k_ssim * (c[0][j] + 2.f * r * c[1][j] + gtv[j] * c[2][j]) + k_l1 * sgn));
        }
    }
}

__global__ __launch_bounds__(256) void clamp01_kernel(int64_t n4, int64_t n, const float* __restrict__ x,
                                                      const float* __restrict__ v_out, float* __restrict__ out) {
    const int64_t i = (int64_t)blockIdx.x * blockDim.x + threadIdx.x;
    if (i < n4) {
        const float4 a = reinterpret_cast<const float4*>(x)[i];
        float4 r;
        if (v_out) {
            const float4 g = reinterpret_cast<const float4*>(v_out)[i];
            r.x = (a.x >= 0.f && a.x <= 1.f) ? g.x : 0.f; r.y = (a.y >= 0.f && a.y <= 1.f) ? g.y : 0.f;
            r.z = (a.z >= 0.f && a.z <= 1.f) ? g.z : 0.f; r.w = (a.w >= 0.f && a.w <= 1.f) ? g.w : 0.f;
        } else {
            r.x = fminf(fmaxf(a.x, 0.f), 1.f); r.y = fminf(fmaxf(a.y, 0.f), 1.f);
            r.z = fminf(fmaxf(a.z, 0.f), 1.f); r.w = fminf(fmaxf(a.w, 0.f), 1.f);
        }
        reinterpret_cast<float4*>(out)[i] = r;
    }
    if (i == 0)
        for (int64_t k = n4 * 4; k < n; ++k) {
            const float a = x[k];
            out[k] = v_out ? ((a >= 0.f && a <= 1.f) ? v_out[k] : 0.f) : fminf(fmaxf(a, 0.f), 1.f);
        }
}

}

using namespace gs;

extern "C" int gs_clamp01(void* stream, int64_t n, const float* x, const float* v_out, float* out) {
    GS_REQUIRE(n >= 0, "n >= 0");
    if (n == 0) return GS_OK;
    GS_REQUIRE(x && out, "null pointer");
    GS_REQUIRE((((uintptr_t)x | (uintptr_t)out | (uintptr_t)v_out) & 15) == 0, "buffers must be 16-byte aligned");
    const int64_t n4 = n >> 2, blocks = (n4 + 255) / 256;
    hipLaunchKernelGGL(clamp01_kernel, dim3((unsigned)(blocks > 0 ? blocks : 1)), dim3(256), 0, (hipStream_t)stream, n4, n, x, v_out, out);
    GS_LAUNCH_CHECK("clamp01_kernel");
    return GS_OK;
}

static int loss_tile_count(int height, int width) { return ((width + kLT - 1) / kLT) * ((height + kLT - 1) / kLT); }
static dim3 loss_grid(int nt) { return dim3((unsigned)(8 * ((nt + 7) / 8))); }

extern "C" size_t gs_loss_workspace_floats(int height, int width) {
    const size_t nb = (size_t)((width + kLT - 1) / kLT) * ((height + kLT - 1) / kLT);
    return 9 * (size_t)height * width + 2 * (nb + 8);
}

static int loss_fwd_launch(void* stream, int height, int width, float lambda_ssim, const float* render, const float* gt,
                           const float* mask, const float* const* slots, bool has_mask, int clamp_input, float* workspace, float* out3) {
    GS_REQUIRE(height > 2 * kHalo && width > 2 * kHalo, "image must be larger than the 11x11 window");
    GS_REQUIRE((int64_t)height * width <= kLossMaxPixels && width <= kLossMaxWidth && height <= (1 << 24),
               "image too large for the loss kernels' 32-bit byte offsets (H * W <= 2^28, W <= 2^20, H <= 2^24: row indices go through 24-bit multiplies)");
    GS_REQUIRE(render && (gt || slots) && workspace && out3, "null pointer");
    LossArgs a;
    a.H = height; a.W = width; a.lambda_ssim = lambda_ssim; a.render = render; a.gt = gt; a.mask = mask; a.slots = slots;
    a.clamp_input = clamp_input != 0;
    a.maps = workspace; a.partial = workspace + 9 * (size_t)height * width; a.gout = nullptr; a.v_render = nullptr;
    const int blocks = (int)loss_grid(loss_tile_count(height, width)).x;
    const size_t lds = sizeof(float) * (2 * kLR * kLRP + 4 * kLR * kHP);
    hipStream_t st = (hipStream_t)stream;
    if (has_mask) hipLaunchKernelGGL(l1_ssim_fwd_kernel<true>, dim3((unsigned)blocks), dim3(256), lds, st, a);
    else hipLaunchKernelGGL(l1_ssim_fwd_kernel<false>, dim3((unsigned)blocks), dim3(256), lds, st, a);
    GS_LAUNCH_CHECK("l1_ssim_fwd_kernel");
    hipLaunchKernelGGL(loss_reduce_kernel, dim3(1), dim3(256), 0, st, blocks, a.partial, height, width, lambda_ssim, out3);
    GS_LAUNCH_CHECK("loss_reduce_kernel");
    return GS_OK;
}

static int loss_bwd_launch(void* stream, int height, int width, float lambda_ssim, const float* render, const float* gt,
                           const float* mask, const float* const* slots, int clamp_input, const float* workspace,
                           const float* v_total, float* v_render) {
    GS_REQUIRE(height > 2 * kHalo && width > 2 * kHalo, "image must be larger than the 11x11 window");
    GS_REQUIRE((int64_t)height * width <= kLossMaxPixels && width <= kLossMaxWidth && height <= (1 << 24),
               "image too large for the loss kernels' 32-bit byte offsets (H * W <= 2^28, W <= 2^20, H <= 2^24: row indices go through 24-bit multiplies)");
    GS_REQUIRE(render && (gt || slots) && workspace && v_total && v_render, "null pointer");
    LossArgs a;
    a.H = height; a.W = width; a.lambda_ssim = lambda_ssim; a.render = render; a.gt = gt; a.mask = mask; a.slots = slots;
    a.clamp_input = clamp_input != 0;
    a.maps = const_cast<float*>(workspace); a.partial = nullptr; a.gout = v_total; a.v_render = v_render;
    const size_t lds = sizeof(float) * (3 * kLR * kLRP);
    hipLaunchKernelGGL(l1_ssim_bwd_kernel, dim3(3 * loss_grid(loss_tile_count(height, width)).x), dim3(256), lds, (hipStream_t)stream, a);
    GS_LAUNCH_CHECK("l1_ssim_bwd_kernel");
    return GS_OK;
}

extern "C" int gs_l1_ssim_fwd(void* stream, int height, int width, float lambda_ssim, const float* render,
                              const float* gt, const float* mask, int clamp_input, float* workspace, float* out3) {
    return loss_fwd_launch(stream, height, width, lambda_ssim, render, gt, mask, nullptr, mask != nullptr, clamp_input, workspace, out3);
}

extern "C" int gs_l1_ssim_bwd(void* stream, int height, int width, float lambda_ssim, const float* render,
                              const float* gt, const float* mask, int clamp_input, const float* workspace,
                              const float* v_total, float* v_render) {
    return loss_bwd_launch(stream, height, width, lambda_ssim, render, gt, mask, nullptr, clamp_input, workspace, v_total, v_render);
}

extern "C" int gs_l1_ssim_fwd_slots(void* stream, int height, int width, float lambda_ssim, const float* render,
                                    const float* const* slots_dev, int has_mask, int clamp_input, float* workspace, float* out3) {
    GS_REQUIRE(slots_dev != nullptr, "slots_dev is required");
    return loss_fwd_launch(stream, height, width, lambda_ssim, render, nullptr, nullptr, slots_dev, has_mask != 0, clamp_input, workspace, out3);
}

extern "C" int gs_l1_ssim_bwd_slots(void* stream, int height, int width, float lambda_ssim, const float* render,
                                    const float* const* slots_dev, int clamp_input, const float* workspace,
                                    const float* v_total, float* v_render) {
    GS_REQUIRE(slots_dev != nullptr, "slots_dev is required");
    return loss_bwd_launch(stream, height, width, lambda_ssim, render, nullptr, nullptr, slots_dev, clamp_input, workspace, v_total, v_render);
}
```

easy_gaussian_splatting_amd/loss.py:

```python
from __future__ import annotations

from typing import Dict

import torch
import torch.nn.functional as F
from torch import Tensor


def _gaussian_window(size: int, sigma: float, device, dtype) -> Tensor:
    x = torch.arange(size, device=device, dtype=dtype) - (size - 1) / 2.0
    g = torch.exp(-(x / sigma) ** 2 / 2)
    return g / g.sum()


def ssim(preds: Tensor, target: Tensor, data_range: float = 1.0, kernel_size: int = 11,
         sigma: float = 1.5, k1: float = 0.01, k2: float = 0.03) -> Tensor:
    c1, c2 = (k1 * data_range) ** 2, (k2 * data_range) ** 2
    ch = preds.shape[1]
    pad = (kernel_size - 1) // 2
    g = _gaussian_window(kernel_size, sigma, preds.device, preds.dtype)
    kern_h = g.view(1, 1, -1, 1).expand(ch * 5, 1, -1, 1).contiguous()
    kern_w = g.view(1, 1, 1, -1).expand(ch * 5, 1, 1, -1).contiguous()
    p = F.pad(preds, (pad, pad, pad, pad), mode="reflect")
    t = F.pad(target, (pad, pad, pad, pad), mode="reflect")
    stack = torch.cat([p, t, p * p, t * t, p * t], dim=1)
    out = F.conv2d(F.conv2d(stack, kern_h, groups=ch * 5), kern_w, groups=ch * 5)
    mu_p, mu_t, e_pp, e_tt, e_pt = out.split(ch, dim=1)
    s_pp = e_pp - mu_p * mu_p
    s_tt = e_tt - mu_t * mu_t
    s_pt = e_pt - mu_p * mu_t
    num = (2 * mu_p * mu_t + c1) * (2 * s_pt + c2)
    den = (mu_p * mu_p + mu_t * mu_t + c1) * (s_pp + s_tt + c2)
    full = num / den
    full = full[..., pad:-pad, pad:-pad]
    return full.mean()


class _FusedL1SSIM(torch.autograd.Function):

    @staticmethod
    def forward(ctx, render_img: Tensor, gt_img: Tensor, mask, lambda_ssim: float, clamp_input: bool = False):
        from . import _native as nat
        L = nat.lib()
        H, W = render_img.shape[:2]
        dev = render_img.device
        ctx.set_materialize_grads(False)
        r, g = render_img.contiguous(), gt_img.contiguous()
        m = None if mask is None else mask.contiguous()
        ws = torch.empty((int(L.gs_loss_workspace_floats(H, W)),), dtype=torch.float32, device=dev)
        out = torch.empty((3,), dtype=torch.float32, device=dev)
        st = torch.cuda.current_stream(dev).cuda_stream
        with torch.cuda.device(dev):
            nat.check(L.gs_l1_ssim_fwd(st, H, W, float(lambda_ssim), r.data_ptr(), g.data_ptr(),
                                       None if m is None else m.data_ptr(), int(clamp_input), ws.data_ptr(), out.data_ptr()),
                      "gs_l1_ssim_fwd")
        ctx.clamp_input = bool(clamp_input)
        ctx.save_for_backward(r, g, ws) if m is None else ctx.save_for_backward(r, g, ws, m)
        ctx.lam = float(lambda_ssim)
        total, l1, ssim_loss = out[2], out[0], out[1]
        ctx.mark_non_differentiable(l1, ssim_loss)
        return total, l1, ssim_loss

    @staticmethod
    def backward(ctx, v_total, _v_l1, _v_ssim):
        from . import _native as nat
        L = nat.lib()
        saved = ctx.saved_tensors
        if v_total is None:
            return None, None, None, None, None
        r, g, ws = saved[:3]
        m = saved[3] if len(saved) > 3 else None
        H, W = r.shape[:2]
        v_render = torch.empty_like(r)
        vt = v_total.contiguous().float()
        st = torch.cuda.current_stream(r.device).cuda_stream
        with torch.cuda.device(r.device):
            nat.check(L.gs_l1_ssim_bwd(st, H, W, ctx.lam, r.data_ptr(), g.data_ptr(), None if m is None else m.data_ptr(),
                                       int(ctx.clamp_input), ws.data_ptr(), vt.data_ptr(), v_render.data_ptr()), "gs_l1_ssim_bwd")
        return v_render, None, None, None, None


class LossComputer:

    def __init__(self, lambda_ssim: float = 0.2, fused: bool = True, clamp_input: bool = False,
                 model=None, lambda_scale: float = 0.0):
        self.lambda_ssim = lambda_ssim
        self.fused = fused
        self.clamp_input = clamp_input
        self.model = model
        self.lambda_scale = lambda_scale

    def _add_regularization(self, d: Dict[str, Tensor]) -> Dict[str, Tensor]:
        if self.model is not None:
            reg = self.model.get_regularization_dict()
            if "scale_reg" in reg:
                d["scale_reg"] = reg["scale_reg"]
                d["total"] = d["total"] + self.lambda_scale * reg["scale_reg"]
        return d

    def get_loss_dict(self, render_img: Tensor, gt_img: Tensor, mask: Tensor = None) -> Dict[str, Tensor]:
        if self.fused and render_img.is_cuda and render_img.dtype == torch.float32:
            total, l1, ssim_loss = _FusedL1SSIM.apply(render_img, gt_img, mask, self.lambda_ssim, self.clamp_input)
            return self._add_regularization({"l1": l1, "ssim": ssim_loss, "total": total})
        if self.clamp_input:
            render_img = torch.clamp(render_img, min=0.0, max=1.0)
        if mask is not None:
            m = mask.unsqueeze(2)
            render_img = m * gt_img + (1.0 - m) * render_img
        l1 = F.l1_loss(render_img, gt_img)
        r = render_img.permute(2, 0, 1)[None]
        g = gt_img.permute(2, 0, 1)[None]
        ssim_loss = 1.0 - ssim(g, r)
        total = (1.0 - self.lambda_ssim) * l1 + self.lambda_ssim * ssim_loss
        return self._add_regularization({"l1": l1, "ssim": ssim_loss, "total": total})
```

easy_gaussian_splatting_amd/rendering.py:

```python
from __future__ import annotations

import ctypes as _ct
import math
import os
import threading
import time
import weakref
from typing import Dict, Optional, Tuple

import torch
from torch import Tensor

from . import _native as nat
from . import workspace as WS

_TILE = nat.GS_TILE
_BWD_CLASSES = os.environ.get("GS_BWD_CLASSES", "1") != "0"


def _ptr(t: Optional[Tensor]) -> Optional[int]:
    return None if t is None else t.data_ptr()


def _stream(device: torch.device) -> int:
# ... 352 lines not shown
        if tiles > MAX_TILES_PER_TILE_PIPELINE:
            raise NotImplementedError("list arrays of a two-round call at this image size: render with GS_ROUNDS=off to read them")
        if torch.cuda.is_current_stream_capturing():
            raise RuntimeError("meta's list arrays of a two-round call are built on first access with a host read-back: read them "
                               "before the capture starts, or render with GS_ROUNDS=off")
        L, dev = nat.lib(), self.depths.device
        with torch.cuda.device(dev):
            st = _stream(dev)
            i32 = dict(dtype=torch.int32, device=dev)
            ws_bytes = int(L.gs_bin_workspace_bytes(C, N, tw, th))
            ws = torch.empty((ws_bytes,), dtype=torch.uint8, device=dev)
            offs, bko, info = torch.empty((C * tiles + 1,), **i32), torch.empty((C * tiles + 1,), **i32), torch.zeros((8,), dtype=torch.int64, device=dev)
            host = torch.zeros((4,), dtype=torch.int64)
            bbox = self.lease.ptr(WS.BBOX)
            nat.check(L.gs_bin_count(st, C, N, tw, th, bbox, ws.data_ptr(), ws_bytes, offs.data_ptr(), bko.data_ptr(), None, info.data_ptr(),
                                     host.data_ptr()), "gs_bin_count")
            n_isects, max_tile = int(host[0]), int(host[2])
            keys = torch.empty((max(n_isects, 1),), dtype=torch.int64, device=dev)
            flat, cum = torch.empty((max(n_isects, 1),), **i32), torch.empty((C * N,), **i32)
            nat.check(L.gs_bin_emit_sort(st, C, N, tw, th, bbox, self.depths.data_ptr(), ws.data_ptr(), ws_bytes, offs.data_ptr(), n_isects,
                                         max(max_tile, 1), keys.data_ptr(), None, cum.data_ptr(), None, flat.data_ptr(), None), "gs_bin_emit_sort")
        return {"flatten_ids": flat[:n_isects], "isect_offsets": offs[: C * tiles].view(C, th, tw)}


def _sort_class(n: int) -> int:
    for c in (1024, 4096, 8192, 16384):
        if n <= c:
            return c
    return 1 << 30


def _forward_stages(means, quats, scales, opacities, colors, colors_rest, viewmats, Ks, backgrounds, cfg, need_grad):
    L = nat.lib()
    dev = means.device
    C, N = viewmats.shape[0], means.shape[0]
    W, H = cfg["width"], cfg["height"]
    sh_degree = cfg["sh_degree"]
    tw, th = math.ceil(W / _TILE), math.ceil(H / _TILE)
    tiles = tw * th
    st = _stream(dev)
    f32 = dict(dtype=torch.float32, device=dev)
    i32 = dict(dtype=torch.int32, device=dev)

    if sh_degree is None:
        deg, K = -1, 0
        per_cam = 1 if colors.dim() == 3 else 0
    else:
        deg, per_cam = int(sh_degree), 0
        K = colors.shape[1] + (0 if colors_rest is None else colors_rest.shape[1])
    ch = 3 if sh_degree is not None else int(colors.shape[-1])

    radii = torch.empty((C, N), **i32)
    means2d = torch.empty((C, N, 2), **f32)
    depths = torch.empty((C, N), **f32)
    conics = torch.empty((C, N, 3), **f32)
    render_colors = torch.empty((C, H, W, ch), **f32)
    render_alphas = torch.empty((C, H, W, 1), **f32)

    lazy_ref = bool(cfg.get("lazy_ref_lists"))
    rect_ref = torch.empty((C * N, 2), **i32) if lazy_ref else None
    dev_index = dev.index if dev.index is not None else torch.cuda.current_device()
    hint_key = (dev_index, C, W, H, bool(need_grad), cfg["tile_culling"])
    with _state_lock:
        hint = dict(_hints.get(hint_key, {}))
    two_level = binning_choice(hint.get("footprint"), tiles) == "bins"
    shift = bin_shift_for(hint.get("footprint")) if two_level else 0
    rmode = cfg.get("rounds") or rounds_mode()
    rounds = (not need_grad) and C == 1 and N > 0 and ch == 3 and rmode != "off" and (rmode == "on" or (
        two_level and int(hint.get("n", -1)) == N and int(hint.get("listed_one_round", 0)) >= ROUNDS_MIN_LISTED and not hint.get("rounds_off")))
    rb = _round_buffers(dev, st, N, tiles) if rounds else None
    eager_ids = os.environ.get("GS_EAGER_ISECT_IDS") == "1"
    factorised = cfg.get("sh_grads") == "colors_pre"
    flags = (WS.F_TRAIN if need_grad else 0) | (WS.F_TWO_LEVEL if two_level else 0) | (WS.F_ISECT_IDS if eager_ids else 0)
    cap = max(int(hint.get("cap", 0)), 2 * C * N + 4096 if not hint else 0, 4096)
    cap_tile = int(hint.get("cap_tile", 1024)) if not two_level else (1 << 30)
    coarse_cap = max(int(hint.get("entries", 0)), 2 * C * N + 1024) if two_level else 0
    coarse_list_cap = int(hint.get("longest", 0)) if two_level else 0
    cap, coarse_cap = _quantize_up(cap), (_quantize_up(coarse_cap) if two_level else 0)
    cap_units = cap_rows = 0
    if need_grad:
        cap_units = _quantize_up(max(int(hint.get("cap_units", 0)), (cap // 16 + 12 * C * tiles) if "cap_units" not in hint else 0, 256))
        cap_rows = _quantize_up(max(int(hint.get("cap_rows", 0)), cap if "cap_rows" not in hint else 0, 4096))
    walk = _WalkRecord() if need_grad else None

    lease = WS.pool.acquire(dev, st)
    lease.bind(WS.Layout(C, N, W, H, cap, coarse_cap, shift, flags, max(cap_units, 256), cap_rows), st)
    P = lease.ptr
    info_dev = lease.view(WS.INFO, 8)
    info_host = _pinned_info(dev)
    bin_bytes = lambda: int(L.gs_bins_workspace_bytes(C, N, tw, th, shift, coarse_cap) if two_level else L.gs_bin_workspace_bytes(C, N, tw, th))

    use_jac = bool(need_grad and _SH_JAC and deg >= 1)

    def project(stage: int, tag: str):
        _stage(tag, dev, lambda: nat.check(L.gs_project_fwd(
            st, C, N, K, deg, _ptr(means), _ptr(quats), _ptr(scales), _ptr(opacities), _ptr(colors), _ptr(colors_rest),
            per_cam, _ptr(viewmats), _ptr(Ks), W, H, cfg["eps2d"], cfg["near_plane"], cfg["far_plane"],
            cfg["radius_clip"], cfg["tile_culling"], stage, cfg.get("activations", 0), _ptr(radii), _ptr(means2d), _ptr(depths), _ptr(conics),
            P(WS.COLORS_POST), P(WS.REC), P(WS.BBOX), P(WS.TILES_PER_GAUSS), _ptr(rect_ref),
            P(WS.SH_JAC) if use_jac else None), "gs_project_fwd"))

    def bbox_ptr():
        return rb["bbox"].data_ptr() if rounds else P(WS.BBOX)

    def count():
        if two_level:
            nat.check(L.gs_bins_count(st, C, N, tw, th, shift, bbox_ptr(), _ptr(depths), P(WS.BIN), bin_bytes(),
                                      P(WS.COARSE_KEYS), coarse_cap, coarse_list_cap, P(WS.CUM_TILES), P(WS.ISECT_OFFSETS),
                                      P(WS.BUCKET_OFFSETS), P(WS.TILE_ORDER), P(WS.INFO), None), "gs_bins_count")
        else:
            nat.check(L.gs_bin_count(st, C, N, tw, th, bbox_ptr(), P(WS.BIN), bin_bytes(), P(WS.ISECT_OFFSETS),
                                     P(WS.BUCKET_OFFSETS), P(WS.TILE_ORDER), P(WS.INFO), None), "gs_bin_count")

    def lists_and_blend():
        if two_level:
            _stage("gs_bin_emit_sort", dev, lambda: nat.check(L.gs_bins_lists(
                st, C, N, tw, th, shift, bbox_ptr(), P(WS.BIN), bin_bytes(), P(WS.COARSE_KEYS), coarse_cap,
                P(WS.CUM_TILES), P(WS.ISECT_OFFSETS), P(WS.ISECT_IDS), P(WS.FLATTEN_IDS), P(WS.SLOTS), P(WS.INFO)), "gs_bins_lists"))
        else:
            _stage("gs_bin_emit_sort", dev, lambda: nat.check(L.gs_bin_emit_sort(
                st, C, N, tw, th, bbox_ptr(), _ptr(depths), P(WS.BIN), bin_bytes(), P(WS.ISECT_OFFSETS), cap,
                min(cap_tile, cap), P(WS.KEYS_TMP), P(WS.SLOT_GID), P(WS.CUM_TILES), P(WS.ISECT_IDS), P(WS.FLATTEN_IDS),
                P(WS.SLOTS)), "gs_bin_emit_sort"))
        if walk is not None:
            nat.check(L.gs_walk_mirror_set(walk.host.data_ptr()), "gs_walk_mirror_set")
        try:
            if ch == 3:
                _stage("gs_blend_fwd", dev, lambda: nat.check(L.gs_blend_fwd(
                    st, C, W, H, P(WS.REC), _ptr(backgrounds), P(WS.ISECT_OFFSETS), P(WS.TILE_ORDER),
                    P(WS.FLATTEN_IDS), P(WS.SLOTS), cap, _ptr(render_colors), _ptr(render_alphas), P(WS.CKPT), P(WS.QLIST), P(WS.QCNT),
                    P(WS.QMASK), P(WS.UNIT_DESC), lease.layout.cap_units, P(WS.ROW_BASE), lease.layout.cap_rows, P(WS.WALK_STATE)),
                    "gs_blend_fwd"))
            else:
                _stage("gs_blend_fwd", dev, lambda: nat.check(L.gs_blend_fwd_ch(
                    st, C, W, H, ch, P(WS.REC), _ptr(backgrounds), P(WS.ISECT_OFFSETS), P(WS.TILE_ORDER),
                    P(WS.FLATTEN_IDS), P(WS.SLOTS), cap, _ptr(render_colors), _ptr(render_alphas), P(WS.CKPT), P(WS.QLIST), P(WS.QCNT),
                    P(WS.QMASK), P(WS.UNIT_DESC), lease.layout.cap_units, P(WS.ROW_BASE), lease.layout.cap_rows, P(WS.WALK_STATE),
                    lease.ckpt_ext() if (need_grad and ch == 4) else None), "gs_blend_fwd_ch"))
        finally:
            if walk is not None:
                L.gs_walk_mirror_set(None)
                walk.event = torch.cuda.Event()
                walk.event.record(tstream)

    if ch == 3:
        project(1 if _SPLIT_PROJECT else 0, "gs_project_fwd")
    else:
        project(1, "gs_project_fwd")
        _stage("gs_rec_colors", dev, lambda: nat.check(L.gs_rec_colors(st, C, N, ch, _ptr(colors), per_cam, _ptr(radii), P(WS.REC)),
                                                       "gs_rec_colors"))
    sizes = {"attempt": 0, "waited": 0, "info": None}
    tstream = torch.cuda.current_stream(dev)

    def enqueue_attempt():
        nat.check(L.gs_guard_set_call(P(WS.INFO), cap, min(cap_tile, cap)), "gs_guard_set_call")
        nat.check(L.gs_info_mirror_set(info_host.data_ptr()), "gs_info_mirror_set")
        try:
            if rounds:
                if sizes["attempt"] == 0 and _SPLIT_PROJECT:
                    project(2, "gs_project_fwd_color")
                nat.check(L.gs_round_split(st, N, _ptr(depths), P(WS.TILES_PER_GAUSS), ROUND_FRACTION, rb["hist"].data_ptr(), rb["blk"].data_ptr()),
                          "gs_round_split")
                ev = None
                for phase in (1, 2):
                    nat.check(L.gs_rounds_set(rb["blk"].data_ptr(), rb["live"].data_ptr(), rb["state"].data_ptr(), None, phase), "gs_rounds_set")
                    nat.check(L.gs_info_mirror_set(info_host.data_ptr()), "gs_info_mirror_set")
                    _stage("gs_round_footprints", dev, lambda: nat.check(L.gs_round_footprints(
                        st, N, tw, th, P(WS.BBOX), _ptr(depths), rb["bbox"].data_ptr(), rb["tpg"].data_ptr()), "gs_round_footprints"))
                    _stage("gs_bin_count", dev, count)
                    nat.check(L.gs_info_mirror_set(None), "gs_info_mirror_set")
                    if phase == 2:
                        ev = torch.cuda.Event()
                        ev.record(tstream)
                    lists_and_blend()
                    if phase == 1 and not deferred:
                        nat.check(L.gs_round_status(st, rb["blk"].data_ptr(), rb["host"].data_ptr()), "gs_round_status")
                        ev = torch.cuda.Event()
                        ev.record(tstream)
                        t_wait = time.perf_counter_ns()
                        ev.synchronize()
                        sizes["waited"] += time.perf_counter_ns() - t_wait
                        if int(info_host[3]) != 0 or int(rb["host"][nat.GS_ROUND_LIVE]) == 0:
                            break
                return ev
            _stage("gs_bin_count", dev, count)
            nat.check(L.gs_info_mirror_set(None), "gs_info_mirror_set")
            ev = torch.cuda.Event()
            ev.record(tstream)
            if sizes["attempt"] == 0 and _SPLIT_PROJECT and ch == 3:
                project(2, "gs_project_fwd_color")
            lists_and_blend()
        finally:
            L.gs_guard_set(None, 0, 0)
            L.gs_info_mirror_set(None)
            L.gs_rounds_set(None, None, None, None, 0)
        return ev

    def settle(ev, whole_stream: bool) -> bool:
        nonlocal cap, cap_tile, coarse_cap, coarse_list_cap, info_dev
        t_wait = time.perf_counter_ns()
        if whole_stream:
            tstream.synchronize()
        else:
            ev.synchronize()
        sizes["waited"] += time.perf_counter_ns() - t_wait
        info = sizes["info"] = [int(v) for v in info_host.tolist()]
        n_isects, max_tile, fl = info[0], info[2], info[3]
        if fl == 0:
            return True
        sizes["attempt"] += 1
        if sizes["attempt"] > 6:
            raise nat.NativeLibraryError(f"rasterization: list capacities did not settle (info {info})")
        if two_level and fl & 12:
            if fl & 4:
                coarse_cap = info[4] + (info[4] >> 2) + 1024
            coarse_list_cap = 0
            with _state_lock:
                stats["coarse_retries"] += 1
        else:
            if fl & 1:
                cap = n_isects + (n_isects >> 3) + 1024
            if fl & 2:
                cap_tile = _sort_class(max_tile)
        with _state_lock:
# ... 15 lines not shown
                       cap_tile=max(_sort_class(max_tile + (max_tile >> 2)), int(old.get("cap_tile", 1024))), footprint=n_isects / max(1, C * N),
                       mode="bins" if two_level else "tiles", n=N, listed_one_round=n_isects)
            if rounds:
                new["footprint"], new["listed_one_round"] = info[7] / max(1, C * N), info[7]
                strikes = int(old.get("live_strikes", 0)) + 1 if info[6] > ROUNDS_MAX_LIVE * C * tiles else 0
                new["live_strikes"], new["rounds_off"] = strikes, strikes >= 3
            elif old.get("rounds_off") and int(old.get("n", -1)) == N:
                new["rounds_off"] = True
            if two_level:
                new.update(entries=max(info[4] + (info[4] >> 2) + 1024, int(old.get("entries", 0) * 0.995)),
                           longest=max(info[5] + (info[5] >> 2) + 64, int(old.get("longest", 0) * 0.995)))
            _hints[hint_key] = new
            _coarse_hint[dev_index] = dict(mode=new["mode"], footprint=new["footprint"])

    deferred = bool(cfg.get("defer_size_check")) and bool(hint) and int(hint.get("n", N)) == N
    ev0 = enqueue_attempt()
    state_late = {}
    if deferred:
        n_buckets_bound = cap // nat.GS_BUCKET + C * tiles + 1

        def resolve_late() -> bool:
            late = False
            ev, whole = ev0, False
            with torch.cuda.device(dev):
                while not settle(ev, whole):
                    late = True
                    ev, whole = enqueue_attempt(), True
            learn()
            state_late["n_isects"], state_late["n_buckets"] = sizes["info"][0], sizes["info"][1]
            if late:
                with _state_lock:
                    stats["late_overflows"] += 1
            return late

        pending = _PendingCheck(resolve_late)
        _pending_checks().append(pending)
        with _state_lock:
            stats["deferred_calls"] += 1
        n_isects, n_buckets, max_tile = None, n_buckets_bound, None
    else:
        pending = None
        ev, whole = ev0, False
        while not settle(ev, whole):
            ev, whole = enqueue_attempt(), True
        learn()
        n_isects, n_buckets, max_tile = sizes["info"][0], sizes["info"][1], sizes["info"][2]

    def isects() -> int:
        if pending is not None:
            pending.resolve()
            return state_late["n_isects"]
        return n_isects

    ref = WS.LeaseRef(lease)
    lazy = _LazyMeta.Lazy
    if lazy_ref:
        ref_lists = _ReferenceLists(rect_ref, depths, C, N, tw, th, eager_ids)
        list_entries = {"tiles_per_gauss": lazy(lambda: ref_lists.get("tiles_per_gauss")),
                        "isect_ids": lazy(lambda: ref_lists.get("isect_ids")) if eager_ids else _LazyMeta.PENDING,
                        "flatten_ids": lazy(lambda: ref_lists.get("flatten_ids")),
                        "isect_offsets": lazy(lambda: ref_lists.get("isect_offsets"))}
    elif rounds:
        one = _OneRoundLists(lease, depths, C, N, tw, th)
        list_entries = {"tiles_per_gauss": lazy(lambda: lease.view(WS.TILES_PER_GAUSS, C * N).clone().view(C, N)),
                        "isect_ids": _LazyMeta.PENDING, "flatten_ids": lazy(lambda: one.get("flatten_ids")),
                        "isect_offsets": lazy(lambda: one.get("isect_offsets"))}
    else:
        list_entries = {
            "tiles_per_gauss": lazy(lambda: (isects(), lease.view(WS.TILES_PER_GAUSS, C * N).clone().view(C, N))[1]),
            "isect_ids": lazy(lambda: lease.view(WS.ISECT_IDS, isects()).clone()) if eager_ids else _LazyMeta.PENDING,
            "flatten_ids": lazy(lambda: lease.view(WS.FLATTEN_IDS, isects()).clone()),
            "isect_offsets": lazy(lambda: (isects(), lease.view(WS.ISECT_OFFSETS, C * tiles).clone().view(C, th, tw))[1])}
    meta = _LazyMeta({
        "camera_ids": None, "gaussian_ids": None,
        "radii": radii, "means2d": means2d, "depths": depths, "conics": conics,
        "opacities": opacities[None, :].expand(C, N),
        "tile_width": tw, "tile_height": th, **list_entries,
        "width": W, "height": H, "tile_size": _TILE, "n_cameras": C,
    })
    if not lazy_ref:
        meta._lease = ref
    state = dict(C=C, N=N, K=K, deg=deg, per_cam=per_cam, ch=ch, sh_jac=use_jac, n_isects=n_isects, n_buckets=n_buckets, radii=radii, lease=lease,
                 lease_ref=WS.LeaseRef(lease) if need_grad else None, factorised=factorised, pending=pending, late=state_late,
                 walk=walk, hint_key=hint_key, backgrounds=backgrounds)
    if pending is not None:
        pending.lease_ref = WS.LeaseRef(lease)
    del ref
    return render_colors, render_alphas, meta, state


def _settle_walk(s: dict, cfg: dict, render_colors: Tensor, render_alphas: Tensor) -> int:
    walk, lease = s.get("walk"), s["lease"]
    if walk is None:
        return 0
    L = nat.lib()
    dev = render_colors.device
    walk.event.synchronize()
    units, storage, rows, fl = (int(v) for v in walk.host.tolist())
    if fl < 0:
        raise nat.NativeLibraryError("rasterization: the forward of this call left no walk record (was it skipped by a step guard?)")
    tries = 0
    while fl & (WS.FLAG_UNITS | WS.FLAG_ROWS):
        tries += 1
        if tries > 3:
            raise nat.NativeLibraryError(f"rasterization: the walk capacities did not settle (units {storage}, rows {rows}, flags {fl})")
        lay = lease.layout
        cu = _quantize_up(storage + (storage >> 2) + 512) if fl & WS.FLAG_UNITS else lay.cap_units
        cr = _quantize_up(rows + (rows >> 2) + 4096) if fl & WS.FLAG_ROWS else lay.cap_rows
        C, N, W, H, cap, coarse_cap, shift, flags = lay.key[:8]
        lease.grow_walk(WS.Layout(C, N, W, H, cap, coarse_cap, shift, flags, cu, cr))
        P = lease.ptr
        with _state_lock:
            stats["walk_reruns"] += 1
        with torch.cuda.device(dev):
            st = _stream(dev)
            sc, sa = torch.empty_like(render_colors), torch.empty_like(render_alphas)
            nat.check(L.gs_walk_mirror_set(walk.host.data_ptr()), "gs_walk_mirror_set")
            try:
                if s["ch"] == 3:
                    nat.check(L.gs_blend_fwd(st, C, W, H, P(WS.REC), _ptr(s["backgrounds"]), P(WS.ISECT_OFFSETS), P(WS.TILE_ORDER),
                                             P(WS.FLATTEN_IDS), P(WS.SLOTS), s["n_isects"], _ptr(sc), _ptr(sa), P(WS.CKPT), P(WS.QLIST),
                                             P(WS.QCNT), P(WS.QMASK), P(WS.UNIT_DESC), cu, P(WS.ROW_BASE), cr, P(WS.WALK_STATE)), "gs_blend_fwd")
                else:
                    nat.check(L.gs_blend_fwd_ch(st, C, W, H, s["ch"], P(WS.REC), _ptr(s["backgrounds"]), P(WS.ISECT_OFFSETS),
                                                P(WS.TILE_ORDER), P(WS.FLATTEN_IDS), P(WS.SLOTS), s["n_isects"], _ptr(sc), _ptr(sa), P(WS.CKPT),
                                                P(WS.QLIST), P(WS.QCNT), P(WS.QMASK), P(WS.UNIT_DESC), cu, P(WS.ROW_BASE), cr, P(WS.WALK_STATE),
                                                lease.ckpt_ext() if s["ch"] == 4 else None), "gs_blend_fwd_ch")
            finally:
                L.gs_walk_mirror_set(None)
            torch.cuda.current_stream(dev).synchronize()
        units, storage, rows, fl = (int(v) for v in walk.host.tolist())
    with _state_lock:
        old = _hints.get(s["hint_key"])
        if old is not None:
            old["cap_units"] = max(storage + (storage >> 2) + 512, int(old.get("cap_units", 0) * 0.995))
            old["cap_rows"] = max(rows + (rows >> 2) + 4096, int(old.get("cap_rows", 0) * 0.995))
    return rows


class _Rasterize(torch.autograd.Function):

    @staticmethod
    def forward(ctx, means, quats, scales, opacities, colors, colors_rest, viewmats, Ks, backgrounds, cfg, holder, campos=None):
        ctx.camera_grads = bool(cfg.get("camera_grads")) and ctx.needs_input_grad[6]
        need_grad = bool(cfg.get("grad_enabled", True)) and (any(ctx.needs_input_grad[:6]) or ctx.camera_grads)
        ctx.set_materialize_grads(False)
        render_colors, render_alphas, meta, state = _forward_stages(
            means, quats, scales, opacities, colors, colors_rest, viewmats, Ks, backgrounds, cfg, need_grad)
        holder.meta = meta
        if holder.debug is not None and need_grad:
            lease, tiles = state["lease"], meta["tile_width"] * meta["tile_height"]
            wstate = lease.view(WS.WALK_STATE, 8).clone()
            holder.debug.update(unit_counter=wstate[WS.WALK_UNITS:WS.WALK_UNITS + 1], walk_state=wstate,
                                qcnt=lease.view(WS.QCNT, state["C"] * tiles * 4).clone(), unit_entries=nat.GS_UNIT)
            if state["n_isects"] is not None:
                holder.debug["walked_isects"] = lease.view(WS.QMASK, max(state["n_isects"], 1))[: state["n_isects"]].count_nonzero()
        holder.lease_ref = state.pop("lease_ref")
        holder.out_ptrs = (render_colors.data_ptr(), render_alphas.data_ptr())
        ctx.cfg, ctx.holder, ctx.state = cfg, holder, state
        ctx.split = colors_rest is not None
        if need_grad:
            extra = (colors_rest,) if ctx.split else ()
            ctx.save_for_backward(means, quats, scales, colors, viewmats, Ks, render_colors, render_alphas, opacities, *extra)
        return render_colors, render_alphas

    @staticmethod
    def backward(ctx, v_render_colors, v_render_alphas):
        L = nat.lib()
        means, quats, scales, colors, viewmats, Ks, render_colors, render_alphas, opacities = ctx.saved_tensors[:9]
        colors_rest = ctx.saved_tensors[9] if ctx.split else None
        s, cfg, holder = ctx.state, ctx.cfg, ctx.holder
        dev = means.device
        st = _stream(dev)
        C, N, K = s["C"], s["N"], s["K"]
        W, H = cfg["width"], cfg["height"]
        f32 = dict(dtype=torch.float32, device=dev)
        v_rc = torch.zeros_like(render_colors) if v_render_colors is None else v_render_colors.contiguous()
        v_ra = None if v_render_alphas is None else v_render_alphas.contiguous()
        lease, factorised = s["lease"], s["factorised"]
        if s.get("pending") is not None:
            if s["pending"].resolve():
                raise RuntimeError("rasterization(_size_check='deferred'): the forward of this call outgrew its list capacities and was "
                                   "repaired only now -- the loss and the upstream gradient of this backward were computed from unwritten "
                                   "memory.  Re-run the step (the capacities have been raised), or use the default immediate size check.")
            s["n_isects"], s["n_buckets"] = s["late"]["n_isects"], s["late"]["n_buckets"]
        P = lease.ptr
        n_rows = _settle_walk(s, cfg, render_colors, render_alphas)
        ucls = torch.empty((int(L.gs_unit_classes_ints(lease.layout.cap_units, C, W, H)),), dtype=torch.int32, device=dev) if _BWD_CLASSES else None
        ch = s["ch"]
        if ch == 3:
            _stage("gs_blend_bwd", dev, lambda: nat.check(L.gs_blend_bwd(st, C, W, H, P(WS.REC), P(WS.QLIST), P(WS.QCNT),
                                     P(WS.UNIT_DESC), lease.layout.cap_units, P(WS.CKPT), P(WS.QMASK), P(WS.ROW_BASE), P(WS.WALK_STATE),
                                     _ptr(render_colors), _ptr(render_alphas), _ptr(v_rc), _ptr(v_ra), P(WS.ROWS), _ptr(ucls)), "gs_blend_bwd"))
        else:
            _stage("gs_blend_bwd", dev, lambda: nat.check(L.gs_blend_bwd_ch(st, C, W, H, ch, P(WS.REC), P(WS.QLIST), P(WS.QCNT),
                                     P(WS.UNIT_DESC), lease.layout.cap_units, P(WS.CKPT), P(WS.QMASK), P(WS.ROW_BASE), P(WS.WALK_STATE),
                                     _ptr(render_colors), _ptr(render_alphas), _ptr(v_rc), _ptr(v_ra), P(WS.ROWS), _ptr(ucls),
                                     lease.ckpt_ext() if ch == 4 else None), "gs_blend_bwd_ch"))
        go = holder.grad_out or {}
        for k_, shp in (("means", (N, 3)), ("quats", (N, 4)), ("scales", (N, 3)), ("opacities", (N,)), ("grad_norm", (N,)), ("count", (N,))):
            if k_ in go and not (go[k_].shape == shp and go[k_].is_contiguous() and go[k_].dtype == torch.float32 and go[k_].device == dev):
                raise ValueError(f"_grad_out['{k_}'] must be a contiguous float32 tensor of shape {shp} on {dev}")
        if ("grad_norm" in go) != ("count" in go) or ("count" in go and not (factorised and C == 1)):
            raise ValueError("_grad_out['grad_norm'] / ['count'] come together, with _sh_grads='colors_pre' and a single camera")
        v_means = go["means"] if "means" in go else torch.empty((N, 3), **f32)
        v_quats = go["quats"] if "quats" in go else torch.empty((N, 4), **f32)
        v_scales = go["scales"] if "scales" in go else torch.empty((N, 3), **f32)
        v_opac = go["opacities"] if "opacities" in go else torch.empty((N,), **f32)
        v_colors = None if factorised else torch.empty(colors.shape, **f32)
        v_pc, pc_cam = (v_colors, s["per_cam"]) if ch == 3 else (torch.empty((C, N, 3), **f32), 1)
        v_rest = torch.empty(colors_rest.shape, **f32) if (ctx.split and not factorised) else None
        v_pre = row_sums = None
        if factorised:
            row_sums = torch.empty((C * N, 12), **f32)
            pay = holder.view_payload
            if pay is not None:
                if not (C == 1 and pay.dim() == 1 and pay.numel() >= 4 * N + 16 and pay.is_contiguous() and pay.dtype == torch.float32 and pay.device == dev):
                    raise ValueError(f"_view_payload must be a contiguous 1-D float32 tensor of >= 4 N + 16 elements on {dev} (single camera)")
                v_pre, rad_out, cam_out = pay[:3 * N].view(1, N, 3), pay[3 * N:4 * N], pay[4 * N:4 * N + 16]
            else:
                v_pre, rad_out, cam_out = torch.empty((C, N, 3), **f32), None, None
            _stage("gs_row_sums", dev, lambda: nat.check(L.gs_row_sums(
                st, C, N, _ptr(s["radii"]), P(WS.COLORS_POST), P(WS.TILES_PER_GAUSS), P(WS.CUM_TILES), P(WS.ROWS), P(WS.ROW_BASE), P(WS.QMASK),
                _ptr(row_sums), _ptr(v_pre), _ptr(rad_out), float(max(W, H)), _ptr(viewmats), _ptr(cam_out)), "gs_row_sums"))
            if holder.means2d_ref is not None and holder.means2d_ref() is not None:
                holder.means2d_ref().colors_pre_grad = v_pre
            if holder.on_colors_pre is not None:
                holder.on_colors_pre(v_pre)
        v_abs = torch.empty((C, N, 2), **f32)
        dbg = holder.debug
        v_m2 = v_cn = v_cp = None
        m2_out = holder.means2d_ref() if holder.means2d_ref is not None else None
        if dbg is not None or (m2_out is not None and m2_out.requires_grad):
            v_m2 = torch.empty((C, N, 2), **f32)
        if dbg is not None:
            v_cn = torch.empty((C, N, 3), **f32)
            v_cp = torch.empty((C, N, 3), **f32)
        v_viewmats = v_campos = None
        bwd_args = lambda: (st, C, N, K, s["deg"], _ptr(means), _ptr(quats), _ptr(scales), _ptr(colors),
                            _ptr(colors_rest), pc_cam, _ptr(viewmats), _ptr(Ks), W, H, cfg["eps2d"],
                            cfg["near_plane"], cfg["far_plane"], _ptr(s["radii"]),
                            P(WS.COLORS_POST), P(WS.TILES_PER_GAUSS), P(WS.CUM_TILES),
                            P(WS.ROWS), P(WS.ROW_BASE), P(WS.QMASK), _ptr(v_means), _ptr(v_quats), _ptr(v_scales), _ptr(v_opac),
                            _ptr(v_pc), _ptr(v_rest), _ptr(v_abs), _ptr(v_m2), _ptr(v_cn), _ptr(v_cp), None,
                            _ptr(opacities), cfg.get("activations", 0), P(WS.SH_JAC) if s.get("sh_jac") else None,
                            _ptr(row_sums), _ptr(go.get("grad_norm")), _ptr(go.get("count")))
        if ctx.camera_grads:
            v_m2 = torch.empty((C, N, 2), **f32) if v_m2 is None else v_m2
            v_cn = torch.empty((C, N, 3), **f32) if v_cn is None else v_cn
            v_cp = torch.empty((C, N, 3), **f32) if v_cp is None else v_cp
            partials = torch.empty((int(L.gs_cam_partials_doubles(C, N)),), dtype=torch.float64, device=dev)
            v_viewmats, v_campos = torch.empty((C, 4, 4), **f32), torch.empty((C, 3), **f32)
            _stage("gs_project_bwd", dev, lambda: nat.check(L.gs_project_bwd_cam(*bwd_args(), _ptr(partials), _ptr(v_viewmats), _ptr(v_campos)),
                                                            "gs_project_bwd_cam"))
        else:
            _stage("gs_project_bwd", dev, lambda: nat.check(L.gs_project_bwd(*bwd_args()), "gs_project_bwd"))
        if ch != 3:
            _stage("gs_channel_grads", dev, lambda: nat.check(L.gs_channel_grads(
                st, C, N, ch, s["per_cam"], _ptr(s["radii"]), P(WS.TILES_PER_GAUSS), P(WS.CUM_TILES), P(WS.ROWS), P(WS.ROW_BASE),
                P(WS.QMASK), _ptr(v_colors)), "gs_channel_grads"))
        if holder.grad_out is not None:
            holder.grad_out["_written"] = True
        if dbg is not None:
            dbg.update(v_means2d=v_m2, v_conics=v_cn, v_colors_post=v_cp,
                       rows=lease.view(WS.ROWS, max(n_rows, 1) * nat.GS_ROW_FLOATS)[: n_rows * nat.GS_ROW_FLOATS].clone().view(-1, nat.GS_ROW_FLOATS))
        if m2_out is not None:
            if holder.absgrad:
                m2_out.absgrad = v_abs
            if m2_out.requires_grad and v_m2 is not None:
                m2_out.grad = v_m2 if m2_out.grad is None else m2_out.grad + v_m2
        ni = ctx.needs_input_grad
# ... 179 lines not shown
```

easy_gaussian_splatting_amd/train_graph.py:

```python
from __future__ import annotations

import ctypes as ct
import math
import time
from collections import deque
from collections.abc import Mapping
from typing import Any, Dict, Optional

import torch
from torch import Tensor

from . import _native as nat
from .optim import FusedAdam
from . import rendering
from .rendering import _SH_JAC


_TILE = nat.GS_TILE
_SORT_CLASSES = (1024, 4096, 8192, 16384)


def _p(t: Optional[Tensor]):
    return None if t is None else t.data_ptr()

# ... 25 lines not shown
        if not isinstance(optimizer, FusedAdam):
            raise TypeError("TrainStepGraph drives optim.FusedAdam (flat parameter / moment buffers)")
        if not getattr(loss_computer, "clamp_input", False) or not getattr(loss_computer, "fused", True):
            raise ValueError("TrainStepGraph needs LossComputer(fused=True, clamp_input=True)")
        self.scale_reg = getattr(loss_computer, "model", None) is not None and bool(getattr(model, "USE_SCALE_REGULARIZATION", False))
        if self.scale_reg:
            if loss_computer.model is not model:
                raise ValueError("TrainStepGraph: the LossComputer regularises another model than the one it trains")
            r = model.MAX_SCALE_RATIO
            self.max_scale_ratio = float(r.detach().cpu()) if isinstance(r, Tensor) else float(r)
            self.lambda_scale = float(loss_computer.lambda_scale)
        self.model, self.opt, self.lc = model, optimizer, loss_computer
        self.margin, self.use_graph, self.check_every = float(margin), bool(use_graph), int(check_every)
        self.fuse_adam = bool(fuse_adam)
        self.dev = model.means.device
        self.W, self.H = int(data["width"]), int(data["height"])
        self.has_mask = mask is not None
        self.graph: Optional[torch.cuda.CUDAGraph] = None
        self.stream = torch.cuda.Stream(self.dev)
        self.cap = 0
        self.cap_units = self.cap_rows = 0
        self.cap_floor = 0
        self.walk_floor = (0, 0)
        self.seen_isects = 0
        self.seen_tile = 0
        self.seen_units = self.seen_rows = 0
        self.probed_walk = (0, 0)
        self._walk_history_void = False
        self.binning = None
        self.probed = (0, 0)
        self.cap_tile = _SORT_CLASSES[0]
        self.pending: deque = deque()
        self.status = torch.zeros((8,), dtype=torch.int64, pin_memory=True)
        self.confirmed = 0
        self.issued = 0
        self.stats = {"captures": 0, "overflows": 0, "replayed_steps": 0, "rebuilds": 0}
        self._pool: Dict[str, Tensor] = {}
        self._warm = set()
        self._key = None
        self.confirmed_at_build = 0
        self._last_inputs = (data["w2c"], data["K"], gt_img, mask)
        self._build(data, gt_img, mask)

    def _state_key(self, W: Optional[int] = None, H: Optional[int] = None):
        m = self.model
        return (m.means.shape[0], self.opt.flat_param.data_ptr(), m.max_radii.data_ptr(), m.grad_norm_accum.data_ptr(),
                m.collecting_counts.data_ptr(), m.active_sh_degree, getattr(m, "tile_culling", "tight"),
                self.W if W is None else int(W), self.H if H is None else int(H))

    def _build(self, data, gt_img, mask, min_cap: int = 0, min_cap_tile: int = 0, projected=None, min_walk=(0, 0)):
        m, dev = self.model, self.dev
        L = nat.lib()
        t_build = time.perf_counter()
        self.N = N = m.means.shape[0]
        self.K = 1 + m.sh_rest.shape[1]
        W, H = self.W, self.H
        self.tw, self.th = math.ceil(W / _TILE), math.ceil(H / _TILE)
        tiles = self.tw * self.th
        f32 = dict(dtype=torch.float32, device=dev)
        i32 = dict(dtype=torch.int32, device=dev)
        b = self.buf = {}
        b["viewmats"] = torch.empty((1, 4, 4), **f32)
        b["Ks"] = torch.empty((1, 3, 3), **f32)
        b["img_slots"] = torch.zeros((2,), dtype=torch.int64, device=dev)
        b["bg"] = m.BACKGROUND.detach().reshape(1, 3).to(dev, torch.float32).contiguous().clone()
        b["radii"] = self._take("radii", (1, N), torch.int32)
        b["means2d"] = self._take("means2d", (1, N, 2), torch.float32)
        b["depths"] = self._take("depths", (1, N), torch.float32)
        b["conics"] = self._take("conics", (1, N, 3), torch.float32)
        b["colors_post"] = self._take("colors_post", (1, N, 3), torch.float32)
        b["sh_jac"] = self._take("sh_jac", (N * 9,), torch.float32) if _SH_JAC else None
        b["rec"] = self._take("rec", (N, nat.GS_REC_FLOATS), torch.float32)
        b["bbox"] = self._take("bbox", (N, 4), torch.int32)
        b["tiles_per_gauss"] = self._take("tiles_per_gauss", (1, N), torch.int32)
        b["cum_tiles"] = self._take("cum_tiles", (N,), torch.int32)
        b["isect_offsets"] = torch.empty((tiles + 1,), **i32)
        b["bucket_offsets"] = torch.empty((tiles + 1,), **i32)
        b["tile_order"] = torch.empty((tiles,), **i32)
        b["info"] = torch.zeros((8,), dtype=torch.int64, device=dev)
        b["applied"] = torch.zeros((1,), dtype=torch.int64, device=dev)
        b["render_colors"] = torch.empty((1, H, W, 3), **f32)
        b["render_alphas"] = torch.empty((1, H, W, 1), **f32)
        b["loss_ws"] = torch.empty((int(L.gs_loss_workspace_floats(H, W)),), **f32)
        b["loss3"] = torch.zeros((3,), **f32)
        b["loss_ring"] = torch.zeros((self.LOSS_RING, 3), **f32)
        b["one"] = torch.ones((), **f32)
        b["v_render"] = torch.empty((H, W, 3), **f32)
        b["qcnt"] = torch.empty((tiles * 4,), **i32)
        b["v_abs"] = self._take("v_abs", (1, N, 2), torch.float32)
        self.grads = None if self.fuse_adam else {
            "means": torch.empty((N, 3), **f32), "log_scales": torch.empty((N, 3), **f32),
            "quats": torch.empty((N, 4), **f32), "sh_0": torch.empty((N, 1, 3), **f32),
            "sh_rest": torch.empty((N, self.K - 1, 3), **f32) if self.K > 1 else None,
            "logit_opacities": torch.empty((N,), **f32)}
        b["hyper"] = torch.zeros((16,), **f32)
        b["scale_reg"] = self._take("scale_reg", (int(L.gs_scale_reg_workspace_floats(N)),), torch.float32) if self.scale_reg else None
        self._stage_inputs(max(self.opt._step, 0) + 1, [float(grp["lr"]) for grp, _ in self.opt._plist], data["w2c"], data["K"], gt_img, mask)
        probe_walk = False
        front_before, self.front_only = self.front_only, False
        if projected is not None:
            n_isects, max_tile, units, rows = projected
            self.cap = int(n_isects * self.margin) + 4096
            need_tile = int(max_tile * self.margin)
            self.cap_tile = next((c for c in _SORT_CLASSES if c >= need_tile), 1 << 30)
            self.cap_units, self.cap_rows = int(units * self.margin) + 512, int(rows * self.margin) + 4096
            self.stats["projected_rebuilds"] = self.stats.get("projected_rebuilds", 0) + 1
        elif self.cap == 0 or min_cap or min_cap_tile or min_walk[0] or min_walk[1]:
            n_isects, max_tile = self._probe()
            self.probed = (n_isects, max_tile)
            self.cap = max(int(max(n_isects, min_cap) * self.margin) + 4096, self.cap, self.cap_floor)
            need_tile = max(int(max(max_tile, min_cap_tile) * self.margin), self.cap_tile)
            self.cap_tile = next((c for c in _SORT_CLASSES if c >= need_tile), 1 << 30)
            probe_walk = True
        self._alloc_binning()
        self._alloc_lists()
        self._alloc_rounds()
        if probe_walk:
            floor = (max(min_walk[0], self.walk_floor[0]), max(min_walk[1], self.walk_floor[1]))
            self.cap_units = max(self.cap_units, int(floor[0] * self.margin) + 512, self.cap // 64 + 4 * tiles + 512)
            self.cap_rows = max(self.cap_rows, int(floor[1] * self.margin) + 4096, self.cap // 8 + 4096)
            while True:
                self._alloc_walk()
                units, rows, fl = self._probe_walk()
                if not fl:
                    break
                self.cap_units = max(self.cap_units, int(units * self.margin) + 512)
                self.cap_rows = max(self.cap_rows, int(rows * self.margin) + 4096)
            self.probed_walk = (units, rows)
            scale = max(1.0, (self.cap / self.margin) / max(n_isects, 1))
            wm = self.margin * (2.0 if self._walk_history_void else 1.0)
            self.cap_units = max(int(max(units * scale, floor[0]) * wm) + 512, 256)
            self.cap_rows = max(int(max(rows * scale, floor[1]) * wm) + 4096, 4096)
            self._walk_history_void = False
            if self.rounds_mode == "auto":
                self.rounds_on = n_isects >= self.ROUNDS_MIN_LISTED and n_isects >= self.ROUNDS_MIN_RATIO * max(rows, 1)
        elif self.rounds_mode == "auto" and self.rounds_on and self._live_n > 0 and self._live_sum > self.ROUNDS_MAX_LIVE * tiles * self._live_n:
            self.rounds_on = False
        self.front_only = bool(front_before and not probe_walk and self.rounds_on and self.rounds_mode == "auto" and self._live_sum == 0)
        self._alloc_walk()
        self._alloc_rounds()
        if probe_walk and self.rounds_mode == "auto" and self.rounds_on:
            self._probe_walk()
            live = int(b["rounds"][nat.GS_ROUND_LIVE])
            self.stats["probed_live_tiles"] = live
            if live > self.ROUNDS_MAX_LIVE * tiles:
                self.rounds_on = False
            self.front_only = self.rounds_on and live == 0 and self.speculate_front and not self._back_needed
            self._back_needed = False
        self._live_sum = self._live_n = 0
        self._key = self._state_key()
        self._opacity_resets = getattr(m, "opacity_resets", 0)
        t_cap = time.perf_counter()
        self._capture(warm_up=projected is None)
        self.stats["rebuilds"] += 1
        now = time.perf_counter()
        self.stats["build_ms"] = round(self.stats.get("build_ms", 0.0) + 1e3 * (now - t_build), 2)
        self.stats["capture_ms"] = round(self.stats.get("capture_ms", 0.0) + 1e3 * (now - t_cap), 2)

    def _take(self, name: str, shape, dtype, shrink: bool = False) -> Tensor:
        n = 1
        for d in shape:
            n *= int(d)
        t = self._pool.get(name)
        if shrink and t is not None and t.numel() > 2 * n + 4096:
            t = None
        if t is None or t.dtype != dtype or t.numel() < n:
# ... 200 lines not shown
                                   _p(m.logit_opacities), _p(m.sh_0), _p(m.sh_rest) if self.K > 1 else None, 0,
                                   _p(b["viewmats"]), _p(b["Ks"]), self.W, self.H, 0.3, 0.01, 1e10, 0.0, culling, 0, 1,
                                   _p(b["radii"]), _p(b["means2d"]), _p(b["depths"]), _p(b["conics"]), _p(b["colors_post"]),
                                   _p(b["rec"]), _p(b["bbox"]), _p(b["tiles_per_gauss"]), None, _p(b["sh_jac"])), "gs_project_fwd")

    def _count(self, bbox: str = "bbox"):
        L, b = nat.lib(), self.buf
        if self.binning == "bins":
            self._ck(L.gs_bins_count(self._st(), 1, self.N, self.tw, self.th, self.bin_shift, _p(b[bbox]), _p(b["depths"]), _p(b["ws"]),
                                      self.ws_bytes, _p(b["coarse_keys"]), self.cap_coarse, self.cap_coarse_list, _p(b["cum_tiles"]),
                                      _p(b["isect_offsets"]), _p(b["bucket_offsets"]), _p(b["tile_order"]), _p(b["info"]), None),
                     "gs_bins_count")
        else:
            self._ck(L.gs_bin_count(self._st(), 1, self.N, self.tw, self.th, _p(b[bbox]), _p(b["ws"]), self.ws_bytes,
                                     _p(b["isect_offsets"]), _p(b["bucket_offsets"]), _p(b["tile_order"]), _p(b["info"]), None),
                     "gs_bin_count")

    def _probe(self):
        from .rendering import MAX_TILES_PER_TILE_PIPELINE, bin_shift_for, binning_choice
        L, b, dev = nat.lib(), self.buf, self.dev
        tiles = self.tw * self.th
        n_isects = max_tile = 0
        footprint = None
        if tiles <= MAX_TILES_PER_TILE_PIPELINE:
            self.binning = "tiles"
            self.ws_bytes = int(L.gs_bin_workspace_bytes(1, self.N, self.tw, self.th))
            b["ws"] = torch.empty((self.ws_bytes,), dtype=torch.uint8, device=dev)
            with torch.cuda.device(dev), self._on_stream():
                self._project()
                self._count()
            info = b["info"].tolist()
            n_isects, max_tile = int(info[0]), int(info[2])
            footprint = n_isects / max(1, self.N)
        else:
            with torch.cuda.device(dev), self._on_stream():
                self._project()
        self.binning = binning_choice(footprint, tiles)
        if self.binning == "bins":
            self.bin_shift = bin_shift_for(footprint) or 2
            self.cap_coarse, self.cap_coarse_list = 2 * self.N + 1024, 0
            while True:
                self._alloc_binning()
                with torch.cuda.device(dev), self._on_stream():
                    self._count()
                info = b["info"].tolist()
                if not int(info[3]) & 12:
                    break
                self.cap_coarse = int(int(info[4]) * self.margin) + 4096
            self.cap_coarse = int(int(info[4]) * self.margin) + 4096
            self.cap_coarse_list = int(int(info[5]) * 1.5) + 64
            self.probed_coarse = (int(info[4]), int(info[5]))
            n_isects, max_tile = int(info[0]), int(info[2])
        b["info"].zero_()
        return n_isects, max_tile

    def _enqueue_forward(self):
        L, b = nat.lib(), self.buf
        self._project()
        if not self.rounds_on:
            self._lists_and_blend("bbox")
            return
        self._ck(L.gs_round_split(self._st(), self.N, _p(b["depths"]), _p(b["tiles_per_gauss"]), self.round_fraction, _p(b["depth_hist"]),
                                   _p(b["rounds"])), "gs_round_split")
        for phase in ((4,) if self.front_only else (1, 2)):
            self._rounds_phase(phase)
            self._ck(L.gs_round_footprints(self._st(), self.N, self.tw, self.th, _p(b["bbox"]), _p(b["depths"]), _p(b["bbox_round"]),
                                            _p(b["tpg_round"])), "gs_round_footprints")
            self._lists_and_blend("bbox_round")
        self._rounds_phase(3)

    def _lists_and_blend(self, bbox: str):
        L, b = nat.lib(), self.buf
        st = self._st()
        N, W, H = self.N, self.W, self.H
        self._count(bbox)
        if self.binning == "bins":
            self._ck(L.gs_bins_lists(st, 1, N, self.tw, self.th, self.bin_shift, _p(b[bbox]), _p(b["ws"]), self.ws_bytes,
                                      _p(b["coarse_keys"]), self.cap_coarse, _p(b["cum_tiles"]), _p(b["isect_offsets"]),
                                      None, _p(b["flatten_ids"]), _p(b["slots"]), _p(b["info"])), "gs_bins_lists")
        else:
            self._ck(L.gs_bin_emit_sort(st, 1, N, self.tw, self.th, _p(b[bbox]), _p(b["depths"]), _p(b["ws"]), self.ws_bytes,
                                         _p(b["isect_offsets"]), self.cap, self.cap_tile, _p(b["keys_tmp"]), _p(b["slot_gid"]),
                                         _p(b["cum_tiles"]), None, _p(b["flatten_ids"]), _p(b["slots"])), "gs_bin_emit_sort")
        self._ck(L.gs_blend_fwd(st, 1, W, H, _p(b["rec"]), _p(b["bg"]), _p(b["isect_offsets"]),
                                 _p(b["tile_order"]), _p(b["flatten_ids"]), _p(b["slots"]), self.cap, _p(b["render_colors"]),
                                 _p(b["render_alphas"]), _p(b["ckpt"]), _p(b["qlist"]), _p(b["qcnt"]), _p(b["qmask"]),
                                 _p(b["unit_desc"]), self.cap_units, _p(b["row_base"]), self.cap_rows, _p(b["walk_state"])),
                 "gs_blend_fwd")

    def _enqueue_step(self):
        L, b, m, opt = nat.lib(), self.buf, self.model, self.opt
        st = self._st()
        N, W, H = self.N, self.W, self.H
        nat.check(L.gs_guard_set(_p(b["info"]), self.cap, self.cap_tile), "gs_guard_set")
        self._stage_no = 0
        try:
            self._enqueue_forward()
            lam = float(self.lc.lambda_ssim)
            self._ck(L.gs_l1_ssim_fwd_slots(st, H, W, lam, _p(b["render_colors"]), _p(b["img_slots"]), int(self.has_mask), 1, _p(b["loss_ws"]),
                                             _p(b["loss3"])), "gs_l1_ssim_fwd_slots")
            self._ck(L.gs_l1_ssim_bwd_slots(st, H, W, lam, _p(b["render_colors"]), _p(b["img_slots"]), 1, _p(b["loss_ws"]),
                                             _p(b["one"]), _p(b["v_render"])), "gs_l1_ssim_bwd_slots")
            if self.scale_reg and self.fuse_adam:
                self._scale_reg(None)
            self._ck(L.gs_blend_bwd(st, 1, W, H, _p(b["rec"]), _p(b["qlist"]), _p(b["qcnt"]), _p(b["unit_desc"]), self.cap_units,
                                     _p(b["ckpt"]), _p(b["qmask"]), _p(b["row_base"]), _p(b["walk_state"]),
                                     _p(b["render_colors"]), _p(b["render_alphas"]), _p(b["v_render"]), None, _p(b["rows"]), _p(b["unit_cls"])),
                      "gs_blend_bwd")
            b1, b2 = opt.defaults["betas"]
            if self.fuse_adam:
                offs = (ct.c_int64 * 6)(*opt._offs)
                args = (st, N, self.K, int(m.active_sh_degree), _p(opt.flat_param), _p(opt.exp_avg),
                        _p(opt.exp_avg_sq), offs, _p(b["viewmats"]), _p(b["Ks"]), W, H, 0.3, 0.01, 1e10,
                        _p(b["radii"]), _p(b["colors_post"]), self._tpg(), _p(b["cum_tiles"]),
                        _p(b["rows"]), _p(b["row_base"]), _p(b["qmask"]), _p(b["v_abs"]), float(b1), float(b2),
                        float(opt.defaults["eps"]), _p(b["hyper"]), _p(b["applied"]), _p(m.max_radii),
                        _p(m.grad_norm_accum), _p(m.collecting_counts), _p(b["sh_jac"]))
                if self.scale_reg:
                    self._ck(L.gs_project_bwd_adam_reg(*args, self.max_scale_ratio, self.lambda_scale), "gs_project_bwd_adam_reg")
                else:
                    self._ck(L.gs_project_bwd_adam(*args), "gs_project_bwd_adam")
            else:
                g = self.grads
                self._ck(L.gs_project_bwd(st, 1, N, self.K, int(m.active_sh_degree), _p(m.means), _p(m.quats), _p(m.log_scales),
                                          _p(m.sh_0), _p(m.sh_rest) if self.K > 1 else None, 0, _p(b["viewmats"]), _p(b["Ks"]), W, H,
                                          0.3, 0.01, 1e10, _p(b["radii"]), _p(b["colors_post"]), self._tpg(),
                                          _p(b["cum_tiles"]), _p(b["rows"]), _p(b["row_base"]), _p(b["qmask"]), _p(g["means"]), _p(g["quats"]),
                                          _p(g["log_scales"]), _p(g["logit_opacities"]), _p(g["sh_0"]), _p(g["sh_rest"]), _p(b["v_abs"]),
                                          None, None, None, None, _p(m.logit_opacities), 1, _p(b["sh_jac"]), None, None, None), "gs_project_bwd")
                if self.scale_reg:
                    self._scale_reg(g["log_scales"])
                self._ck(L.gs_update_statistics(st, N, float(max(H, W)), _p(b["radii"]), _p(b["v_abs"]), _p(m.max_radii),
                                                _p(m.grad_norm_accum), _p(m.collecting_counts)), "gs_update_statistics")
                ns = len(opt._plist)
                ends = (ct.c_int64 * ns)(*opt._ends)
                lens = (ct.c_int64 * ns)(*opt._lens)
                gptr = (ct.c_void_p * ns)(*[_p(g[grp["name"]]) for grp, _ in opt._plist])
                self._ck(L.gs_adam_step_dev(st, opt.flat_param.numel(), _p(opt.flat_param), _p(opt.exp_avg), _p(opt.exp_avg_sq), ns,
                                            ends, lens, gptr, float(b1), float(b2), float(opt.defaults["eps"]), 1.0, _p(b["hyper"]),
                                            _p(b["applied"])), "gs_adam_step_dev")
            self._ck(L.gs_step_status(st, _p(b["info"]), _p(b["applied"]), self.status.data_ptr(), _p(b["loss3"]), _p(b["loss_ring"]),
                                      self.LOSS_RING, _p(b["walk_state"])), "gs_step_status")
        except TrainStepGraph._Stop:
            pass
        finally:
            L.gs_guard_set(None, 0, 0)
            L.gs_rounds_set(None, None, None, None, 0)

    def _scale_reg(self, v_log_scales: Optional[Any], check=None):
        b, m = self.buf, self.model
        v = v_log_scales if (v_log_scales is None or isinstance(v_log_scales, int)) else v_log_scales.data_ptr()
        (check or self._ck)(nat.lib().gs_scale_reg(self._st(), self.N, _p(m.log_scales), self.max_scale_ratio, self.lambda_scale, _p(b["loss3"]),
                                        _p(b["scale_reg"]), v), "gs_scale_reg")

    def _tail(self, t: int, lrs):
        """What a step enqueues behind its graph (nothing: the single-GPU step is the graph)."""

    def _hyper(self, t: int, lrs):
        L, opt = nat.lib(), self.opt
        ns = len(opt._plist)
        b1, b2 = opt.defaults["betas"]
        nat.check(L.gs_adam_hyper(self._st(), ns, (ct.c_float * ns)(*lrs), float(b1), float(b2), int(t), _p(self.buf["hyper"])),
                  "gs_adam_hyper")

    def _capture(self, warm_up: bool = True):
        opt, m = self.opt, self.model
        names = ("max_radii", "grad_norm_accum", "collecting_counts")
        with torch.cuda.device(self.dev), self._on_stream():
            if warm_up:
                self._warm.add((self.binning, self.cap_tile))
                saved = [opt.flat_param.clone(), opt.exp_avg.clone(), opt.exp_avg_sq.clone()] + [getattr(m, n).clone() for n in names]
# ... 331 lines not shown
```

include/gs_raster.h:

```cpp
#ifndef GS_RASTER_H_
#define GS_RASTER_H_

#include <stddef.h>
#include <stdint.h>

#ifdef __cplusplus
extern "C" {
#endif

#define GS_TILE 16
#define GS_BUCKET 64
#define GS_UNIT 32
#define GS_REC_FLOATS 12
#ifndef GS_ROW_FLOATS
#define GS_ROW_FLOATS 12
#endif

#define GS_WALK_UNITS 0
#define GS_WALK_STORAGE 1
#define GS_WALK_ROWS 3
#define GS_WALK_FLAGS 4
#define GS_WALK_SKIP 5
#define GS_WALK_RANGES 32
#define GS_WALK_RANGE0 32
#define GS_WALK_WORDS (GS_WALK_RANGE0 + 32 * GS_WALK_RANGES)
#define GS_FLAG_ISECTS 1
#define GS_FLAG_TILE 2
#define GS_FLAG_COARSE 4
#define GS_FLAG_COARSE_LIST 8
#define GS_FLAG_UNITS 16
#define GS_FLAG_ROWS 32
#define GS_FLAG_BACK 64
#define GS_FLAG_PEER 128

#define GS_OK 0
#define GS_ERR_ARG (-1)
#define GS_ERR_HIP (-2)
#define GS_ERR_UNSUPPORTED (-3)

int gs_version(void);
const char* gs_build_flags(void);
const char* gs_last_error(void);
const char* gs_arch(void);

int gs_guard_set(const int64_t* info_dev, int64_t cap_isects, int64_t cap_tile);
int gs_guard_set_call(const int64_t* info_dev, int64_t cap_isects, int64_t cap_tile);

int gs_info_mirror_set(int64_t* info_host_mapped);
int gs_walk_mirror_set(int64_t* walk_host_mapped);

int gs_guard_flag_out(void* stream, const int64_t* info_dev, float* dst0, float* dst1);
int gs_guard_merge(void* stream, int64_t* info_dev, const float* flags, int n, int64_t stride);
int gs_step_applied(void* stream, const int64_t* info_dev, int64_t* applied_dev);

#define GS_ROUND_BASE 0
#define GS_ROUND_SPLIT 1
#define GS_ROUND_LIVE 2
#define GS_ROUND_FRONT_N 3
#define GS_ROUND_LISTED_ALL 4
#define GS_ROUND_WORDS 8
int gs_rounds_set(int64_t* rounds_dev, uint8_t* tile_live, float* tile_state, int32_t* tile_rec, int phase);
int gs_round_split(void* stream, int64_t N, const float* depths, const int32_t* tiles_per_gauss, float fraction,
                   uint32_t* hist_ws, int64_t* rounds_dev);
int gs_round_footprints(void* stream, int64_t N, int tile_w, int tile_h, const uint32_t* bbox, const float* depths,
                        uint32_t* bbox_round, int32_t* tiles_per_gauss_round);

int gs_round_status(void* stream, const int64_t* rounds_dev, int64_t* status_host_mapped);

int gs_step_status(void* stream, const int64_t* info_dev, const int64_t* applied_dev, int64_t* status,
                   const float* loss3_dev, float* loss_ring_dev, int ring_len, const int32_t* walk_state);

#define GS_WS_INFO 0
#define GS_WS_REC 1
#define GS_WS_BBOX 2
#define GS_WS_TILES_PER_GAUSS 3
#define GS_WS_CUM_TILES 4
#define GS_WS_COLORS_POST 5
#define GS_WS_ISECT_OFFSETS 6
#define GS_WS_BUCKET_OFFSETS 7
#define GS_WS_TILE_ORDER 8
#define GS_WS_QCNT 9
#define GS_WS_SH_JAC 10
#define GS_WS_LIST_FIRST 11
#define GS_WS_BIN 11
#define GS_WS_COARSE_KEYS 12
#define GS_WS_KEYS_TMP 13
#define GS_WS_SLOT_GID 14
#define GS_WS_FLATTEN_IDS 15
#define GS_WS_SLOTS_BUF 16
#define GS_WS_ISECT_IDS_BUF 17
#define GS_WS_QMASK 18
#define GS_WS_ROW_BASE 19
#define GS_WS_WALK_STATE 20
#define GS_WS_WALK_FIRST 21
#define GS_WS_CKPT 21
#define GS_WS_QLIST 22
#define GS_WS_UNIT_DESC 23
#define GS_WS_ROWS 24
#define GS_WS_SLOTS 25
#define GS_WS_TRAIN 1
#define GS_WS_TWO_LEVEL 2
#define GS_WS_ISECT_IDS 4
int gs_workspace_query(int C, int64_t N, int width, int height, int64_t cap_isects, int64_t coarse_cap, int64_t cap_units,
                       int64_t cap_rows, int bin_shift, int flags, int64_t* offsets, int64_t* arena_bytes);
int gs_workspace_bind(void* stream, void* fixed_base, int64_t fixed_bytes, void* list_base, int64_t list_bytes,
                      void* walk_base, int64_t walk_bytes, const int64_t* offsets, const int64_t* arena_bytes);

int gs_bin_groups(int64_t N);
size_t gs_bin_workspace_bytes(int C, int64_t N, int tile_w, int tile_h);

int gs_project_fwd(void* stream, int C, int64_t N, int K, int sh_degree, const float* means,
                   const float* quats, const float* scales, const float* opacities,
                   const float* colors_in, const float* sh_rest, int colors_per_camera,
                   const float* viewmats, const float* Ks, int width, int height, float eps2d,
                   float near_plane, float far_plane, float radius_clip, int tile_culling, int stage, int activations,
                   int32_t* radii,
                   float* means2d, float* depths, float* conics, float* colors_out, float* rec, uint32_t* bbox,
                   int32_t* tiles_per_gauss, uint32_t* rect_ref, float* sh_jac);

int gs_bin_count(void* stream, int C, int64_t N, int tile_w, int tile_h, const uint32_t* bbox,
                 void* workspace, size_t workspace_bytes, int32_t* isect_offsets,
                 int32_t* bucket_offsets, int32_t* tile_order, int64_t* info_dev, int64_t* info_host);

int gs_bin_emit_sort(void* stream, int C, int64_t N, int tile_w, int tile_h, const uint32_t* bbox,
                     const float* depths, void* workspace, size_t workspace_bytes,
                     const int32_t* isect_offsets, int64_t n_isects, int64_t max_tile_count,
                     uint64_t* keys_tmp, int32_t* slot_gid, int32_t* cum_tiles, int64_t* isect_ids,
                     int32_t* flatten_ids, int32_t* slots);

size_t gs_bins_workspace_bytes(int C, int64_t N, int tile_w, int tile_h, int bin_shift, int64_t coarse_cap);
int gs_bins_count(void* stream, int C, int64_t N, int tile_w, int tile_h, int bin_shift, const uint32_t* bbox,
                  const float* depths, void* workspace, size_t workspace_bytes, uint64_t* coarse_keys,
                  int64_t coarse_cap, int64_t coarse_list_cap, int32_t* cum_tiles, int32_t* isect_offsets,
                  int32_t* bucket_offsets, int32_t* tile_order, int64_t* info_dev, int64_t* info_host);
int gs_bins_lists(void* stream, int C, int64_t N, int tile_w, int tile_h, int bin_shift, const uint32_t* bbox,
                  void* workspace, size_t workspace_bytes, const uint64_t* coarse_keys, int64_t coarse_cap,
                  const int32_t* cum_tiles, const int32_t* isect_offsets, int64_t* isect_ids, int32_t* flatten_ids,
                  int32_t* slots, const int64_t* info_dev);

size_t gs_walk_state_ints(int64_t n_isects);
int gs_blend_fwd(void* stream, int C, int width, int height, const float* rec,
                 const float* backgrounds, const int32_t* isect_offsets, const int32_t* tile_order,
                 const int32_t* flatten_ids, const int32_t* slots, int64_t n_isects, float* render_colors,
                 float* render_alphas, float* ckpt, int32_t* qlist, int32_t* qcnt, uint8_t* qmask,
                 int32_t* unit_desc, int64_t cap_units, int32_t* row_base, int64_t cap_rows, int32_t* walk_state);

size_t gs_unit_classes_ints(int64_t cap_units, int C, int width, int height);
int gs_blend_bwd(void* stream, int C, int width, int height, const float* rec,
                 const int32_t* qlist, const int32_t* qcnt, const int32_t* unit_desc, int64_t cap_units,
                 const float* ckpt, const uint8_t* qmask, const int32_t* row_base, const int32_t* walk_state,
                 const float* render_colors, const float* render_alphas, const float* v_render_colors,
                 const float* v_render_alphas, float* rows, int32_t* unit_classes);

int gs_rec_colors(void* stream, int C, int64_t N, int channels, const float* colors, int colors_per_camera, const int32_t* radii,
                  float* rec);
int gs_blend_fwd_ch(void* stream, int C, int width, int height, int channels, const float* rec,
                    const float* backgrounds, const int32_t* isect_offsets, const int32_t* tile_order,
                    const int32_t* flatten_ids, const int32_t* slots, int64_t n_isects, float* render_colors,
                    float* render_alphas, float* ckpt, int32_t* qlist, int32_t* qcnt, uint8_t* qmask,
                    int32_t* unit_desc, int64_t cap_units, int32_t* row_base, int64_t cap_rows, int32_t* walk_state,
                    float* ckpt_ext);
int gs_blend_bwd_ch(void* stream, int C, int width, int height, int channels, const float* rec,
                    const int32_t* qlist, const int32_t* qcnt, const int32_t* unit_desc, int64_t cap_units,
                    const float* ckpt, const uint8_t* qmask, const int32_t* row_base, const int32_t* walk_state,
                    const float* render_colors, const float* render_alphas, const float* v_render_colors,
                    const float* v_render_alphas, float* rows, int32_t* unit_classes, const float* ckpt_ext);
int gs_channel_grads(void* stream, int C, int64_t N, int channels, int colors_per_camera, const int32_t* radii,
                     const int32_t* tiles_per_gauss, const int32_t* cum_tiles, const float* rows, const int32_t* row_base,
                     const uint8_t* qmask, float* v_colors);

int gs_project_bwd(void* stream, int C, int64_t N, int K, int sh_degree, const float* means,
                   const float* quats, const float* scales, const float* colors_in,
                   const float* sh_rest, int colors_per_camera, const float* viewmats,
                   const float* Ks, int width, int height, float eps2d, float near_plane, float far_plane,
                   const int32_t* radii, const float* colors_post, const int32_t* tiles_per_gauss,
                   const int32_t* cum_tiles, const float* rows, const int32_t* row_base, const uint8_t* qmask,
                   float* v_means, float* v_quats, float* v_scales, float* v_opacities,
                   float* v_colors, float* v_sh_rest, float* v_means2d_abs, float* v_means2d,
                   float* v_conics, float* v_colors_post, float* v_colors_pre,
                   const float* opacities, int activations, const float* sh_jac, const float* row_sums,
                   float* stat_grad_norm, float* stat_count);

size_t gs_cam_partials_doubles(int C, int64_t N);
int gs_project_bwd_cam(void* stream, int C, int64_t N, int K, int sh_degree, const float* means,
                       const float* quats, const float* scales, const float* colors_in,
                       const float* sh_rest, int colors_per_camera, const float* viewmats,
                       const float* Ks, int width, int height, float eps2d, float near_plane, float far_plane,
                       const int32_t* radii, const float* colors_post, const int32_t* tiles_per_gauss,
                       const int32_t* cum_tiles, const float* rows, const int32_t* row_base, const uint8_t* qmask,
                       float* v_means, float* v_quats, float* v_scales, float* v_opacities,
                       float* v_colors, float* v_sh_rest, float* v_means2d_abs, float* v_means2d,
                       float* v_conics, float* v_colors_post, float* v_colors_pre,
                       const float* opacities, int activations, const float* sh_jac, const float* row_sums,
                       float* stat_grad_norm, float* stat_count, double* cam_partials, float* v_viewmats,
                       float* v_campos);

int gs_row_sums(void* stream, int C, int64_t N, const int32_t* radii, const float* colors_post,
                const int32_t* tiles_per_gauss, const int32_t* cum_tiles, const float* rows, const int32_t* row_base, const uint8_t* qmask,
                float* row_sums, float* v_colors_pre, float* radii_norm, float max_hw, const float* viewmats, float* cam_out);

int gs_sh_grad_views(void* stream, int R, int64_t N, int K, int sh_degree, const float* means,
                     const float* viewmats, const float* v_colors_pre, float* v_colors,
                     float* v_sh_rest);

int gs_sh_adam_views(void* stream, int R, int64_t N, int K, int sh_degree, const float* means, const float* payload,
                     int64_t payload_stride, float* sh_0, float* sh_0_exp_avg, float* sh_0_exp_avg_sq, float* sh_rest,
                     float* sh_rest_exp_avg, float* sh_rest_exp_avg_sq, float lr_sh_0, float lr_sh_rest, float beta1, float beta2,
                     float eps, int64_t step, float grad_scale, float* max_radii);

size_t gs_loss_workspace_floats(int height, int width);
int gs_l1_ssim_fwd(void* stream, int height, int width, float lambda_ssim, const float* render,
                   const float* gt, const float* mask, int clamp_input, float* workspace, float* out3);
int gs_l1_ssim_bwd(void* stream, int height, int width, float lambda_ssim, const float* render,
                   const float* gt, const float* mask, int clamp_input, const float* workspace,
                   const float* v_total, float* v_render);

int gs_l1_ssim_fwd_slots(void* stream, int height, int width, float lambda_ssim, const float* render,
                         const float* const* slots_dev, int has_mask, int clamp_input, float* workspace, float* out3);
int gs_l1_ssim_bwd_slots(void* stream, int height, int width, float lambda_ssim, const float* render,
                         const float* const* slots_dev, int clamp_input, const float* workspace,
                         const float* v_total, float* v_render);

int gs_clamp01(void* stream, int64_t n, const float* x, const float* v_out, float* out);

int gs_adam_step(void* stream, int64_t n, float* params, float* exp_avg, float* exp_avg_sq,
                 int n_segments, const int64_t* seg_ends_host, const int64_t* seg_lens_host,
                 const float* const* seg_grads_host, const float* seg_lrs_host, float beta1,
                 float beta2, float eps, int64_t step, float grad_scale);

int gs_adam_step_stats(void* stream, int64_t n, float* params, float* exp_avg, float* exp_avg_sq,
                       int n_segments, const int64_t* seg_ends_host, const int64_t* seg_lens_host,
                       const float* const* seg_grads_host, const float* seg_lrs_host, float beta1, float beta2,
                       float eps, int64_t step, float grad_scale, int64_t stat_n, const float* stat_src0,
                       const float* stat_src1, float* stat_dst0, float* stat_dst1);

int gs_adam_hyper(void* stream, int n_segments, const float* seg_lrs_host, float beta1, float beta2, int64_t step,
                  float* hyper_dev);
int gs_step_inputs(void* stream, int n_segments, const float* seg_lrs_host, float beta1, float beta2, int64_t step,
                   float* hyper_dev, const float* viewmat_src, float* viewmat_dst, const float* K_src, float* K_dst,
                   const float* gt, const float* mask, const float** slots_dev);
int gs_adam_step_dev(void* stream, int64_t n, float* params, float* exp_avg, float* exp_avg_sq, int n_segments,
                     const int64_t* seg_ends_host, const int64_t* seg_lens_host, const float* const* seg_grads_host,
                     float beta1, float beta2, float eps, float grad_scale, const float* hyper_dev, int64_t* applied_dev);

size_t gs_scan_rows_workspace_ints(int rows, int64_t n);
int gs_scan_rows_i32(void* stream, int rows, int64_t n, const int32_t* in, int32_t* out, int32_t* workspace);
int gs_refine_flags(void* stream, int64_t n, int num_splits, float densify_grad_thresh, float densify_scale_thresh,
                    float prune_radii_ratio_thresh, float prune_scale_thresh, float min_opacity,
                    const float* grad_norm_accum, const float* counts, const float* max_radii, const float* log_scales,
                    const float* logit_opacities, int32_t* flags, int64_t* counters);
int gs_refine_apply(void* stream, int64_t n_old, int num_splits, int K, const int32_t* flags, const int32_t* flags_incl,
                    int64_t tot_old, int64_t tot_child, int64_t tot_clone, const float* noise, const float* old_params,
                    const float* old_exp_avg, const float* old_exp_avg_sq, const int64_t* old_offsets_host, float* new_params,
                    float* new_exp_avg, float* new_exp_avg_sq, const int64_t* new_offsets_host, int32_t* src_scratch,
                    int8_t* tag_scratch);

int gs_project_bwd_adam(void* stream, int64_t N, int K, int sh_degree, float* params, float* exp_avg, float* exp_avg_sq,
                        const int64_t* offsets_host, const float* viewmats, const float* Ks, int width, int height, float eps2d,
                        float near_plane, float far_plane, const int32_t* radii, const float* colors_post,
                        const int32_t* tiles_per_gauss, const int32_t* cum_tiles, const float* rows, const int32_t* row_base, const uint8_t* qmask,
                        float* v_means2d_abs, float beta1, float beta2, float eps, const float* hyper_dev, int64_t* applied_dev,
                        float* max_radii, float* grad_norm_accum, float* counts, const float* sh_jac);

size_t gs_scale_reg_workspace_floats(int64_t N);
int gs_scale_reg(void* stream, int64_t N, const float* log_scales, float max_ratio, float lambda, float* loss3, float* reg_ws,
                 float* v_log_scales);
int gs_project_bwd_adam_reg(void* stream, int64_t N, int K, int sh_degree, float* params, float* exp_avg, float* exp_avg_sq,
                            const int64_t* offsets_host, const float* viewmats, const float* Ks, int width, int height, float eps2d,
                            float near_plane, float far_plane, const int32_t* radii, const float* colors_post,
                            const int32_t* tiles_per_gauss, const int32_t* cum_tiles, const float* rows, const int32_t* row_base,
                            const uint8_t* qmask, float* v_means2d_abs, float beta1, float beta2, float eps, const float* hyper_dev,
                            int64_t* applied_dev, float* max_radii, float* grad_norm_accum, float* counts, const float* sh_jac,
                            float max_ratio, float lambda);

int gs_pack_view_step(void* stream, int64_t n, float max_hw, const float* v_means, const float* v_scales,
                      const float* v_quats, const float* v_opacities, const int32_t* radii, const float* absgrad,
                      float* flat);

int gs_update_statistics(void* stream, int64_t n, float max_hw, const int32_t* radii, const float* absgrad,
                         float* max_radii, float* grad_norm_accum, float* counts);

#ifdef __cplusplus
}
#endif
#endif
```

Baseline: 746.8.

## Fuse post-walk row scan and unit classification into one decoupled-lookback kernel

Replaces the three-kernel row scan (count, chunk scan, base) with a single-pass decoupled-lookback scan driven by an atomic ticket. The unit-class binning kernel moves into the same launch as extra blocks, and its header clear folds into the qmask clear kernel. The unit-class buffer is now allocated once, bound during the forward pass and reused in backward. The aim is fewer kernel launches and less global traffic on the post-walk path, at the cost of spin-waiting on inter-block status words and a doubled status region. Loss reduction entry points are also added.

```diff
diff --git a/easy_gaussian_splatting_amd/_native.py b/easy_gaussian_splatting_amd/_native.py
--- a/easy_gaussian_splatting_amd/_native.py
+++ b/easy_gaussian_splatting_amd/_native.py
@@ -45,6 +45,9 @@
     "gs_blend_fwd": (_I, [_P, _I, _I, _I, _P, _P, _P, _P, _P, _P, _L, _P, _P, _P, _P, _P, _P, _P, _L, _P, _L, _P]),
     "gs_blend_bwd": (_I, [_P, _I, _I, _I, _P, _P, _P, _P, _L, _P, _P, _P, _P, _P, _P, _P, _P, _P, _P]),
     "gs_unit_classes_ints": (_Z, [_L, _I, _I, _I]),
+    "gs_unit_classes_set": (_I, [_P]),
+    "gs_post_walk": (_I, [_P, _I, _I, _I, _P, _L, _P, _L, _P, _P, _P, _L, _P]),
+    "gs_walk_clear": (_I, [_P, _P, _L, _P, _P]),
     "gs_rec_colors": (_I, [_P, _I, _L, _I, _P, _I, _P, _P]),
     "gs_blend_fwd_ch": (_I, [_P, _I, _I, _I, _I, _P, _P, _P, _P, _P, _P, _L, _P, _P, _P, _P, _P, _P, _P, _L, _P, _L, _P, _P]),
     "gs_blend_bwd_ch": (_I, [_P, _I, _I, _I, _I, _P, _P, _P, _P, _L, _P, _P, _P, _P, _P, _P, _P, _P, _P, _P, _P]),
@@ -61,6 +64,7 @@
     "gs_loss_workspace_floats": (_Z, [_I, _I]),
     "gs_l1_ssim_fwd": (_I, [_P, _I, _I, _F, _P, _P, _P, _I, _P, _P]),
     "gs_l1_ssim_bwd": (_I, [_P, _I, _I, _F, _P, _P, _P, _I, _P, _P, _P]),
+    "gs_loss_reduce": (_I, [_P, _I, _I, _F, _P, _P]),
     "gs_l1_ssim_fwd_slots": (_I, [_P, _I, _I, _F, _P, _P, _I, _I, _P, _P]),
     "gs_l1_ssim_bwd_slots": (_I, [_P, _I, _I, _F, _P, _P, _I, _P, _P, _P]),
     "gs_clamp01": (_I, [_P, _L, _P, _P, _P]),
diff --git a/easy_gaussian_splatting_amd/csrc/gs_blend.hip b/easy_gaussian_splatting_amd/csrc/gs_blend.hip
--- a/easy_gaussian_splatting_amd/csrc/gs_blend.hip
+++ b/easy_gaussian_splatting_amd/csrc/gs_blend.hip
@@ -24,6 +24,7 @@
 constexpr int kWalkUnits = GS_WALK_UNITS, kWalkStorage = GS_WALK_STORAGE, kWalkRows = GS_WALK_ROWS,
               kWalkFlags = GS_WALK_FLAGS, kWalkSkip = GS_WALK_SKIP;
 constexpr int kScanThreads = 256, kScanPerThread = 32, kScanChunk = kScanThreads * kScanPerThread;
+constexpr int kClsHdrInts = 16, kClsUnits = 1024;
 
 struct BlendFwdArgs {
     const int32_t* tile_order;
@@ -119,7 +120,8 @@
 }
 
 __global__ __launch_bounds__(256) void qmask_clear_kernel(uint8_t* __restrict__ q, int64_t n_cap, int32_t* __restrict__ walk, int walk_ints,
-                                                          const int64_t* __restrict__ guard, const int64_t* __restrict__ rblk, int phase) {
+                                                          const int64_t* __restrict__ guard, const int64_t* __restrict__ rblk, int phase,
+                                                          int32_t* __restrict__ cls_hdr) {
     bool skip = guard_tripped(guard);
     if (phase == 2) skip = skip || walk[kWalkSkip] != 0;
     if (blockIdx.x == 0 && threadIdx.x == 0) walk[kWalkSkip] = skip ? 1 : 0;
@@ -127,9 +129,11 @@
     const int64_t first = phase == 2 ? min(rblk[GS_ROUND_BASE], slots_in_use(n_cap, guard)) : 0;
     const int64_t n = slots_in_use(n_cap, guard) - first;
     q += first;
-    if (phase != 2)
+    if (phase != 2) {
         for (int i = (int)blockIdx.x * 256 + (int)threadIdx.x; i < walk_ints; i += (int)gridDim.x * 256)
             if (i != kWalkSkip) walk[i] = 0;
+        if (cls_hdr != nullptr && blockIdx.x == 0 && threadIdx.x < kClsHdrInts) cls_hdr[threadIdx.x] = 0;
+    }
     const int64_t head = min(n, (int64_t)((16 - ((uintptr_t)q & 15)) & 15));
     const int64_t n16 = (n - head) >> 4;
     uint4* q16 = reinterpret_cast<uint4*>(q + head);
@@ -411,33 +415,68 @@
     return tot;
 }
 
-__global__ __launch_bounds__(kScanThreads) void row_count_kernel(const RowScanArgs a) {
+constexpr unsigned long long kStAggregate = 1ull << 32, kStPrefix = 2ull << 32;
+
+struct PostWalkArgs {
+    RowScanArgs s;
+    int scan_blocks;
+    const int4* unit_desc;
+    const int32_t* qcnt;
+    int cap_units, cls_cap;
+    int32_t* cls_hdr;
+    int4* cls;
+};
+
+__device__ __forceinline__ void row_scan_block(const RowScanArgs& a) {
     __shared__ int32_t scratch[20];
-    if (a.walk[kWalkSkip] != 0) return;
+    __shared__ int32_t s_chunk, s_excl;
+    if (threadIdx.x == 0) s_chunk = atomicAdd(a.walk + GS_WALK_TICKET, 1);
+    __syncthreads();
+    const int chunk = s_chunk;
     const int64_t n = slots_in_use(a.n_cap, a.guard);
-    const int64_t c0 = (int64_t)blockIdx.x * kScanChunk;
+    const int64_t c0 = (int64_t)chunk * kScanChunk;
     if (c0 > n) return;
+    const int64_t i0 = c0 + (int64_t)threadIdx.x * kScanPerThread;
     uint32_t w[8];
-    const int32_t tot = row_counts32(a.qmask, c0 + (int64_t)threadIdx.x * kScanPerThread, n, w);
+    const int32_t tot = row_counts32(a.qmask, i0, n, w);
     int32_t block_tot;
-    block_excl_scan_add<int32_t>(tot, scratch, &block_tot);
-    if (threadIdx.x == 0) a.walk[GS_WALK_WORDS + blockIdx.x] = block_tot;
-}
-
-__global__ __launch_bounds__(1024) void row_chunk_scan_kernel(const RowScanArgs a) {
-    __shared__ int32_t scratch[20];
-    if (a.walk[kWalkSkip] != 0) return;
-    const int64_t n = slots_in_use(a.n_cap, a.guard);
-    const int nb = (int)(n / kScanChunk) + 1;
-    int32_t* part = a.walk + GS_WALK_WORDS;
-    const int per = (nb + 1023) / 1024;
-    const int j0 = (int)threadIdx.x * per, j1 = min(nb, j0 + per);
-    int32_t mine = 0;
-    for (int j = j0; j < j1; ++j) mine += part[j];
-    int32_t total;
-    int32_t run = block_excl_scan_add<int32_t>(mine, scratch, &total);
-    for (int j = j0; j < j1; ++j) { const int32_t c = part[j]; part[j] = run; run += c; }
-    if (threadIdx.x == 0) {
+    const int32_t in_block = block_excl_scan_add<int32_t>(tot, scratch, &block_tot);
+    unsigned long long* status = reinterpret_cast<unsigned long long*>(a.walk + GS_WALK_WORDS);
+    if (threadIdx.x < 64) {
+        const int lane = (int)threadIdx.x;
+        if (lane == 0)
+            __hip_atomic_store(status + chunk, (chunk == 0 ? kStPrefix : kStAggregate) | (unsigned long long)(uint32_t)block_tot,
+                               __ATOMIC_RELAXED, __HIP_MEMORY_SCOPE_AGENT);
+        int32_t excl = 0;
+        int top = chunk - 1;
+        while (top >= 0) {
+            const int k = top - lane;
+            unsigned long long v = kStPrefix;
+            if (k >= 0) v = __hip_atomic_load(status + k, __ATOMIC_RELAXED, __HIP_MEMORY_SCOPE_AGENT);
+            const unsigned st = (unsigned)(v >> 32);
+            if (__ballot(st == 0u) != 0ull) { __builtin_amdgcn_s_sleep(2); continue; }
+            const unsigned long long pref = __ballot(st == 2u);
+            const int stop = pref ? (int)__ffsll((long long)pref) - 1 : 64;
+            excl += wave_reduce_add<int32_t>(lane <= stop ? (int32_t)(uint32_t)v : 0);
+            if (pref) break;
+            top -= 64;
+        }
+        if (lane == 0) {
+            if (chunk > 0)
+                __hip_atomic_store(status + chunk, kStPrefix | (unsigned long long)(uint32_t)(excl + block_tot), __ATOMIC_RELAXED,
+                                   __HIP_MEMORY_SCOPE_AGENT);
+            s_excl = excl;
+        }
+    }
+    __syncthreads();
+    const int32_t run = in_block + s_excl;
+    int32_t first16 = 0;
+#pragma unroll
+    for (int j = 0; j < 4; ++j) first16 += (int32_t)((w[j] * 0x01010101u) >> 24);
+    if (i0 <= n) a.row_base[i0 >> 4] = run;
+    if (i0 + 16 <= n) a.row_base[(i0 >> 4) + 1] = run + first16;
+    if (threadIdx.x == 0 && (int64_t)chunk == n / kScanChunk) {
+        const int32_t total = s_excl + block_tot;
         int32_t fullest = 0;
         for (int r = 0; r < GS_WALK_RANGES; ++r) fullest = max(fullest, a.walk[GS_WALK_RANGE0 + 32 * r]);
         a.walk[kWalkStorage] = GS_WALK_RANGES * fullest;
@@ -456,22 +495,55 @@
     }
 }
 
-__global__ __launch_bounds__(kScanThreads) void row_base_kernel(const RowScanArgs a) {
-    __shared__ int32_t scratch[20];
-    if (a.walk[kWalkSkip] != 0) return;
-    const int64_t n = slots_in_use(a.n_cap, a.guard);
-    const int64_t c0 = (int64_t)blockIdx.x * kScanChunk;
-    if (c0 > n) return;
-    const int64_t i0 = c0 + (int64_t)threadIdx.x * kScanPerThread;
-    uint32_t w[8];
-    const int32_t tot = row_counts32(a.qmask, i0, n, w);
-    int32_t block_tot;
-    const int32_t run = block_excl_scan_add<int32_t>(tot, scratch, &block_tot) + a.walk[GS_WALK_WORDS + blockIdx.x];
-    int32_t first16 = 0;
-#pragma unroll
-    for (int j = 0; j < 4; ++j) first16 += (int32_t)((w[j] * 0x01010101u) >> 24);
-    if (i0 <= n) a.row_base[i0 >> 4] = run;
-    if (i0 + 16 <= n) a.row_base[(i0 >> 4) + 1] = run + first16;
+__device__ __forceinline__ void unit_classes_block(const PostWalkArgs& a, int blk) {
+    constexpr int kRounds = kClsUnits / kScanThreads, kRuns = kClsUnits / 64;
+    __shared__ int s_cnt[kRuns][4], s_base[kRuns][4];
+    const int n_units = min(max(a.s.walk[kWalkUnits], 0), a.cap_units);
+    if (blk * kClsUnits >= n_units) return;
+    const int wave = threadIdx.x >> 6, lane = threadIdx.x & 63;
+    int c[kRounds];
+    int4 ud[kRounds];
+#pragma unroll
+    for (int k = 0; k < kRounds; ++k) {
+        const int u = blk * kClsUnits + k * kScanThreads + (int)threadIdx.x;
+        c[k] = 0;
+        ud[k] = make_int4(0, 0, 0, 0);
+        if (u < n_units) {
+            ud[k] = a.unit_desc[u];
+            const int n_in = min(kUnit, a.qcnt[ud[k].x] - ud[k].y * kUnit);
+            c[k] = min(max((n_in + 7) / 8, 1), 4);
+            ud[k].w = u;
+        }
+        unsigned long long m[4];
+#pragma unroll
+        for (int j = 0; j < 4; ++j) m[j] = __ballot(c[k] == j + 1);
+        if (lane < 4) s_cnt[k * (kScanThreads / 64) + wave][lane] = (int)__popcll(lane == 0 ? m[0] : (lane == 1 ? m[1] : (lane == 2 ? m[2] : m[3])));
+    }
+    __syncthreads();
+    if (threadIdx.x < 4) {
+        int tot = 0;
+        for (int w = 0; w < kRuns; ++w) { s_base[w][threadIdx.x] = tot; tot += s_cnt[w][threadIdx.x]; }
+        const int base = tot ? atomicAdd(a.cls_hdr + 1 + threadIdx.x, tot) : 0;
+        for (int w = 0; w < kRuns; ++w) s_base[w][threadIdx.x] += base;
+    }
+    __syncthreads();
+#pragma unroll
+    for (int k = 0; k < kRounds; ++k) {
+        unsigned long long m[4];
+#pragma unroll
+        for (int j = 0; j < 4; ++j) m[j] = __ballot(c[k] == j + 1);
+        const unsigned long long mine = c[k] == 1 ? m[0] : (c[k] == 2 ? m[1] : (c[k] == 3 ? m[2] : m[3]));
+        if (c[k]) {
+            const int i = s_base[k * (kScanThreads / 64) + wave][c[k] - 1] + (int)__popcll(mine & ((1ull << lane) - 1ull));
+            if (i >= 0 && i < (c[k] == 4 ? a.cap_units : a.cls_cap)) a.cls[(c[k] == 4 ? 0 : a.cap_units + (3 - c[k]) * a.cls_cap) + i] = ud[k];
+        }
+    }
+}
+
+__global__ __launch_bounds__(kScanThreads) void post_walk_kernel(const PostWalkArgs a) {
+    if (a.s.walk[kWalkSkip] != 0) return;
+    if ((int)blockIdx.x < a.scan_blocks) row_scan_block(a.s);
+    else unit_classes_block(a, (int)blockIdx.x - a.scan_blocks);
 }
 
 struct BlendBwdArgs {
@@ -690,45 +762,6 @@
     }
 }
 
-constexpr int kClsHdrInts = 16, kClsThreads = 1024;
-__global__ __launch_bounds__(64) void unit_classes_clear_kernel(int32_t* __restrict__ hdr) {
-    if (threadIdx.x < kClsHdrInts) hdr[threadIdx.x] = 0;
-}
-__global__ __launch_bounds__(kClsThreads) void unit_classes_kernel(const int32_t* __restrict__ walk, const int4* __restrict__ unit_desc,
-                                                                   const int32_t* __restrict__ qcnt, int cap_units, int cls_cap,
-                                                                   int32_t* __restrict__ hdr, int4* __restrict__ cls, const int64_t* __restrict__ guard) {
-    __shared__ int s_cnt[kClsThreads / 64][4], s_base[kClsThreads / 64][4];
-    if (guard_tripped(guard)) return;
-    const int n_units = min(walk[kWalkUnits], cap_units);
-    if ((int)blockIdx.x * kClsThreads >= n_units) return;
-    const int u = (int)blockIdx.x * kClsThreads + (int)threadIdx.x, wave = threadIdx.x >> 6, lane = threadIdx.x & 63;
-    int c = 0;
-    int4 ud = make_int4(0, 0, 0, 0);
-    if (u < n_units) {
-        ud = unit_desc[u];
-        const int n_in = min(kUnit, qcnt[ud.x] - ud.y * kUnit);
-        c = min(max((n_in + kPipeLanes - 1) / kPipeLanes, 1), 4);
-        ud.w = u;
-    }
-    unsigned long long m[4];
-#pragma unroll
-    for (int k = 0; k < 4; ++k) m[k] = __ballot(c == k + 1);
-    if (lane < 4) s_cnt[wave][lane] = (int)__popcll(lane == 0 ? m[0] : (lane == 1 ? m[1] : (lane == 2 ? m[2] : m[3])));
-    __syncthreads();
-    if (threadIdx.x < 4) {
-        int tot = 0;
-        for (int w = 0; w < kClsThreads / 64; ++w) { s_base[w][threadIdx.x] = tot; tot += s_cnt[w][threadIdx.x]; }
-        const int base = tot ? atomicAdd(hdr + 1 + threadIdx.x, tot) : 0;
-        for (int w = 0; w < kClsThreads / 64; ++w) s_base[w][threadIdx.x] += base;
-    }
-    __syncthreads();
-    if (c) {
-        const unsigned long long mine = c == 1 ? m[0] : (c == 2 ? m[1] : (c == 3 ? m[2] : m[3]));
-        const int i = s_base[wave][c - 1] + (int)__popcll(mine & ((1ull << lane) - 1ull));
-        if (i < (c == 4 ? cap_units : cls_cap)) cls[(c == 4 ? 0 : cap_units + (3 - c) * cls_cap) + i] = ud;
-    }
-}
-
 template <int NC>
 __device__ __forceinline__ void blend_bwd_body(const BlendBwdArgs& a, const float* __restrict__ ckpt_ext) {
     __shared__ float4 sd0_all[kBwdWaves][kUnitsPerWave][64];
@@ -800,7 +833,48 @@
 
 extern "C" size_t gs_walk_state_ints(int64_t n_isects) {
     if (n_isects < 0) return 0;
-    return (size_t)GS_WALK_WORDS + (size_t)(n_isects / kScanChunk + 1);
+    static_assert(GS_WALK_WORDS % 2 == 0, "the 64-bit status words behind the counters are 8-byte aligned");
+    return (size_t)GS_WALK_WORDS + 2 * (size_t)(n_isects / kScanChunk + 1);
+}
+
+static int64_t cls_region(int C, int width, int height) {
+    const int64_t tiles = (int64_t)((width + GS_TILE - 1) / GS_TILE) * ((height + GS_TILE - 1) / GS_TILE);
+    const int64_t per_block = kBwdWaves * kUnitsPerWave;
+    return (4 * (int64_t)C * tiles + per_block - 1) / per_block * per_block;
+}
+
+extern "C" int gs_post_walk(void* stream, int C, int width, int height, const uint8_t* qmask, int64_t n_isects, int32_t* row_base,
+                            int64_t cap_rows, int32_t* walk_state, const int32_t* unit_desc, const int32_t* qcnt, int64_t cap_units,
+                            int32_t* unit_classes) {
+    GS_REQUIRE(C >= 1 && width > 0 && height > 0 && n_isects >= 0 && n_isects < (1ll << 31) - kScanChunk, "C>=1, positive image size, 0 <= n_isects < 2^31 - 8192");
+    GS_REQUIRE(qmask && row_base && walk_state && cap_rows >= 0 && cap_rows < (1ll << 31), "null pointer / cap_rows out of range");
+    GS_REQUIRE(((uintptr_t)qmask & 15) == 0 && ((uintptr_t)row_base & 15) == 0 && ((uintptr_t)walk_state & 7) == 0,
+               "qmask / row_base 16-byte aligned, walk_state 8-byte aligned");
+    GS_REQUIRE(!unit_classes || (unit_desc && qcnt && cap_units >= 0 && cap_units < (1ll << 26) && ((uintptr_t)unit_classes & 15) == 0),
+               "unit_classes needs unit_desc, qcnt, 0 <= cap_units < 2^26 and 16-byte alignment");
+    PostWalkArgs p;
+    p.s.qmask = qmask; p.s.row_base = row_base; p.s.walk = walk_state; p.s.n_cap = n_isects; p.s.cap_rows = cap_rows;
+    p.s.guard = current_guard().info;
+    p.s.flags = p.s.guard ? reinterpret_cast<unsigned long long*>(const_cast<int64_t*>(p.s.guard) + 3) : nullptr;
+    p.s.mirror = current_walk_mirror();
+    p.scan_blocks = (int)(n_isects / kScanChunk + 1);
+    p.unit_desc = reinterpret_cast<const int4*>(unit_desc); p.qcnt = qcnt;
+    p.cap_units = unit_classes ? (int)cap_units : 0; p.cls_cap = (int)cls_region(C, width, height);
+    p.cls_hdr = unit_classes; p.cls = unit_classes ? reinterpret_cast<int4*>(unit_classes + kClsHdrInts) : nullptr;
+    const unsigned cls_blocks = unit_classes ? (unsigned)((cap_units + kClsUnits - 1) / kClsUnits) : 0u;
+    hipLaunchKernelGGL(post_walk_kernel, dim3((unsigned)p.scan_blocks + cls_blocks), dim3(kScanThreads), 0, (hipStream_t)stream, p);
+    GS_LAUNCH_CHECK("post_walk_kernel");
+    return GS_OK;
+}
+
+extern "C" int gs_walk_clear(void* stream, uint8_t* qmask, int64_t n_isects, int32_t* walk_state, int32_t* unit_classes) {
+    GS_REQUIRE(qmask && walk_state && n_isects >= 0 && n_isects < (1ll << 31) - kScanChunk, "null pointer / n_isects out of range");
+    GS_REQUIRE(((uintptr_t)walk_state & 7) == 0, "walk_state 8-byte aligned");
+    const unsigned cg = (unsigned)std::min<int64_t>(1024, std::max<int64_t>(1, (n_isects / 16 + 255) / 256));
+    hipLaunchKernelGGL(qmask_clear_kernel, dim3(cg), dim3(256), 0, (hipStream_t)stream, qmask, n_isects, walk_state,
+                       (int)gs_walk_state_ints(n_isects), current_guard().info, (const int64_t*)nullptr, 0, unit_classes);
+    GS_LAUNCH_CHECK("qmask_clear_kernel");
+    return GS_OK;
 }
 
 template <int NC>
@@ -817,7 +891,7 @@
     GS_REQUIRE(!train || (cap_units >= kChunk * GS_WALK_RANGES && cap_units < (1ll << 26) && cap_rows >= 0 && cap_rows < (1ll << 31)),
                "training mode: 256 <= cap_units < 2^26 work units, cap_rows < 2^31 gradient rows");
     GS_REQUIRE(!train || n_isects < (1ll << 31) - kScanChunk, "training mode: the slots of a call are indexed by int32");
-    static_assert(kScanPerThread == 32, "row_base_kernel writes two groups of 16 slots per thread");
+    static_assert(kScanPerThread == 32, "row_scan_block writes two groups of 16 slots per thread");
     GS_REQUIRE(!train || (((uintptr_t)qmask & 15) == 0 && ((uintptr_t)row_base & 15) == 0 && ((uintptr_t)walk_state & 7) == 0),
                "training mode: qmask / row_base 16-byte aligned, walk_state 8-byte aligned");
     BlendFwdArgs a;
@@ -849,8 +923,9 @@
     if (train) {
         const int walk_ints = (int)gs_walk_state_ints(n_isects);
         const unsigned cg = (unsigned)std::min<int64_t>(1024, std::max<int64_t>(1, (n_isects / 16 + 255) / 256));
+        int32_t* unit_classes = current_unit_classes();
         hipLaunchKernelGGL(qmask_clear_kernel, dim3(cg), dim3(256), 0, st, qmask, n_isects, walk_state, walk_ints, a.guard,
-                           (const int64_t*)R.blk, phase);
+                           (const int64_t*)R.blk, phase, unit_classes);
         GS_LAUNCH_CHECK("qmask_clear_kernel");
         if constexpr (NC != 3) hipLaunchKernelGGL((chan_fwd_kernel<true, kFwdWaves, NC>), grid, block, 0, st, a, ckpt_ext);
         else if (phase == 1) hipLaunchKernelGGL((blend_fwd_kernel<true, kFwdWaves, 1>), grid, block, 0, st, a);
@@ -858,14 +933,7 @@
         else hipLaunchKernelGGL((blend_fwd_kernel<true, kFwdWaves, 0>), grid, block, 0, st, a);
         GS_LAUNCH_CHECK("blend_fwd_kernel");
         if (phase == 1 && !a.solo) return GS_OK;
-        RowScanArgs s;
-        s.qmask = qmask; s.row_base = row_base; s.walk = walk_state; s.n_cap = n_isects; s.cap_rows = cap_rows;
-        s.flags = a.flags; s.guard = a.guard; s.mirror = current_walk_mirror();
-        const unsigned chunks = (unsigned)(n_isects / kScanChunk + 1);
-        hipLaunchKernelGGL(row_count_kernel, dim3(chunks), dim3(kScanThreads), 0, st, s);
-        hipLaunchKernelGGL(row_chunk_scan_kernel, dim3(1), dim3(1024), 0, st, s);
-        hipLaunchKernelGGL(row_base_kernel, dim3(chunks), dim3(kScanThreads), 0, st, s);
-        GS_LAUNCH_CHECK("row_base_kernel");
+        return gs_post_walk(stream, C, width, height, qmask, n_isects, row_base, cap_rows, walk_state, unit_desc, qcnt, cap_units, unit_classes);
     } else {
         if constexpr (NC != 3) hipLaunchKernelGGL((chan_fwd_kernel<false, kFwdWaves, NC>), grid, block, 0, st, a, nullptr);
         else if (phase == 1) hipLaunchKernelGGL((blend_fwd_kernel<false, kFwdWaves, 1>), grid, block, 0, st, a);
@@ -903,12 +971,6 @@
         default: return GS_FWD_CH(4);
     }
 #undef GS_FWD_CH
-}
-
-static int64_t cls_region(int C, int width, int height) {
-    const int64_t tiles = (int64_t)((width + GS_TILE - 1) / GS_TILE) * ((height + GS_TILE - 1) / GS_TILE);
-    const int64_t per_block = kBwdWaves * kUnitsPerWave;
-    return (4 * (int64_t)C * tiles + per_block - 1) / per_block * per_block;
 }
 
 extern "C" size_t gs_unit_classes_ints(int64_t cap_units, int C, int width, int height) {
@@ -946,11 +1008,6 @@
         GS_REQUIRE(((uintptr_t)unit_classes & 15) == 0, "unit_classes must be 16-byte aligned");
         a.cls_hdr = unit_classes; a.cls_desc = reinterpret_cast<const int4*>(unit_classes + kClsHdrInts);
         a.cls_cap = (int)cls_region(C, width, height);
-        hipLaunchKernelGGL(unit_classes_clear_kernel, dim3(1), dim3(64), 0, (hipStream_t)stream, unit_classes);
-        hipLaunchKernelGGL(unit_classes_kernel, dim3((unsigned)((cap_units + kClsThreads - 1) / kClsThreads)), dim3(kClsThreads), 0, (hipStream_t)stream,
-                           walk_state, a.unit_desc, qcnt, (int)cap_units, a.cls_cap, unit_classes, reinterpret_cast<int4*>(unit_classes + kClsHdrInts),
-                           a.guard);
-        GS_LAUNCH_CHECK("unit_classes_kernel");
         grid += 3u * (unsigned)(a.cls_cap / (kUnitsPerWave * kBwdWaves));
     }
     if constexpr (NC == 3) hipLaunchKernelGGL(blend_bwd_kernel, dim3(grid), dim3(kBwdWaves * 64), 0, (hipStream_t)stream, a);
diff --git a/easy_gaussian_splatting_amd/csrc/gs_capi.hip b/easy_gaussian_splatting_amd/csrc/gs_capi.hip
--- a/easy_gaussian_splatting_amd/csrc/gs_capi.hip
+++ b/easy_gaussian_splatting_amd/csrc/gs_capi.hip
@@ -16,6 +16,8 @@
 int64_t* current_info_mirror() { return g_info_mirror; }
 static thread_local int64_t* g_walk_mirror = nullptr;
 int64_t* current_walk_mirror() { return g_walk_mirror; }
+static thread_local int32_t* g_unit_classes = nullptr;
+int32_t* current_unit_classes() { return g_unit_classes; }
 static thread_local Rounds g_rounds = {nullptr, nullptr, nullptr, nullptr, 0};
 Rounds current_rounds() { return g_rounds; }
 }
@@ -44,6 +46,15 @@
 
 extern "C" int gs_walk_mirror_set(int64_t* walk_host_mapped) {
     gs::g_walk_mirror = walk_host_mapped;
+    return GS_OK;
+}
+
+extern "C" int gs_unit_classes_set(int32_t* unit_classes) {
+    if (((uintptr_t)unit_classes & 15) != 0) {
+        gs::set_error("invalid argument: unit_classes must be 16-byte aligned");
+        return GS_ERR_ARG;
+    }
+    gs::g_unit_classes = unit_classes;
     return GS_OK;
 }
 
diff --git a/easy_gaussian_splatting_amd/csrc/gs_common.h b/easy_gaussian_splatting_amd/csrc/gs_common.h
--- a/easy_gaussian_splatting_amd/csrc/gs_common.h
+++ b/easy_gaussian_splatting_amd/csrc/gs_common.h
@@ -68,6 +68,7 @@
 Guard current_guard();
 int64_t* current_info_mirror();
 int64_t* current_walk_mirror();
+int32_t* current_unit_classes();
 __device__ __forceinline__ bool guard_tripped(const int64_t* info) { return info != nullptr && info[3] != 0; }
 
 struct Rounds {
diff --git a/easy_gaussian_splatting_amd/csrc/gs_loss.hip b/easy_gaussian_splatting_amd/csrc/gs_loss.hip
--- a/easy_gaussian_splatting_amd/csrc/gs_loss.hip
+++ b/easy_gaussian_splatting_amd/csrc/gs_loss.hip
@@ -44,6 +44,14 @@
     *reinterpret_cast<F3*>(reinterpret_cast<char*>(base) + byte_off) = F3{x, y, z};
 }
 
+__device__ __forceinline__ void loss_partial_store(float* partial, int i, float l1, float ssim) {
+    __hip_atomic_store(partial + 2 * i, l1, __ATOMIC_RELAXED, __HIP_MEMORY_SCOPE_AGENT);
+    __hip_atomic_store(partial + 2 * i + 1, ssim, __ATOMIC_RELAXED, __HIP_MEMORY_SCOPE_AGENT);
+}
+__device__ __forceinline__ float loss_partial_load(const float* partial, int i) {
+    return __hip_atomic_load(partial + i, __ATOMIC_RELAXED, __HIP_MEMORY_SCOPE_AGENT);
+}
+
 __device__ __forceinline__ bool loss_tile(const LossArgs& a, int& x0, int& y0) {
     const int ntx = (a.W + kLT - 1) / kLT, nt = ntx * ((a.H + kLT - 1) / kLT), per = (nt + 7) >> 3;
     const int id = blockIdx.x, t = (id & 7) * per + (id >> 3);
@@ -66,7 +74,7 @@
 constexpr int kHOut = 6, kHWin = kHOut + 10;
 
 template <bool MASK>
-__global__ __launch_bounds__(256) void l1_ssim_fwd_kernel(const LossArgs a) {
+__device__ __forceinline__ void l1_ssim_fwd_body(const LossArgs& a) {
     constexpr float kWin[11] = GS_WIN_TAPS;
     extern __shared__ __attribute__((aligned(16))) float lds[];
     float* sx = lds;
@@ -75,7 +83,7 @@
     __shared__ float red[2][4];
     int x0, y0;
     if (!loss_tile(a, x0, y0)) {
-        if (threadIdx.x == 0) { a.partial[2 * blockIdx.x] = 0.f; a.partial[2 * blockIdx.x + 1] = 0.f; }
+        if (threadIdx.x == 0) loss_partial_store(a.partial, blockIdx.x, 0.f, 0.f);
         return;
     }
     const int tid = threadIdx.x;
@@ -192,17 +200,13 @@
     ssim_sum = wave_reduce_add(ssim_sum);
     if (lane_id() == 0) { red[0][tid >> 6] = l1; red[1][tid >> 6] = ssim_sum; }
     __syncthreads();
-    if (tid == 0) {
-        a.partial[2 * blockIdx.x] = red[0][0] + red[0][1] + red[0][2] + red[0][3];
-        a.partial[2 * blockIdx.x + 1] = red[1][0] + red[1][1] + red[1][2] + red[1][3];
-    }
-}
-
-__global__ __launch_bounds__(256) void loss_reduce_kernel(int nblocks, const float* __restrict__ partial, int H, int W,
-                                                          float lambda_ssim, float* __restrict__ out) {
+    if (tid == 0) loss_partial_store(a.partial, blockIdx.x, red[0][0] + red[0][1] + red[0][2] + red[0][3], red[1][0] + red[1][1] + red[1][2] + red[1][3]);
+}
+
+__device__ __forceinline__ void loss_reduce_body(int nblocks, const float* partial, int H, int W, float lambda_ssim, float* out) {
     __shared__ double red[2][4];
     double s0 = 0.0, s1 = 0.0;
-    for (int i = threadIdx.x; i < nblocks; i += 256) { s0 += partial[2 * i]; s1 += partial[2 * i + 1]; }
+    for (int i = threadIdx.x; i < nblocks; i += 256) { s0 += loss_partial_load(partial, 2 * i); s1 += loss_partial_load(partial, 2 * i + 1); }
 #pragma unroll
     for (int d = 32; d > 0; d >>= 1) { s0 += __shfl_xor(s0, d, 64); s1 += __shfl_xor(s1, d, 64); }
     if (lane_id() == 0) { red[0][threadIdx.x >> 6] = s0; red[1][threadIdx.x >> 6] = s1; }
@@ -214,6 +218,25 @@
         out[0] = (float)l1; out[1] = (float)(1.0 - ssim);
         out[2] = (float)((1.0 - lambda_ssim) * l1 + lambda_ssim * (1.0 - ssim));
     }
+}
+
+template <bool MASK>
+__global__ __launch_bounds__(256) void l1_ssim_fwd_kernel(const LossArgs a, int* ticket, float* out3) {
+    __shared__ int s_last;
+    l1_ssim_fwd_body<MASK>(a);
+    if (threadIdx.x == 0) {
+        __builtin_amdgcn_fence(__ATOMIC_RELEASE, "workgroup");
+        __builtin_amdgcn_s_waitcnt(0);
+        s_last = __hip_atomic_fetch_add(ticket, 1, __ATOMIC_RELAXED, __HIP_MEMORY_SCOPE_AGENT) == (int)gridDim.x - 1;
+    }
+    __syncthreads();
+    if (!s_last) return;
+    loss_reduce_body((int)gridDim.x, a.partial, a.H, a.W, a.lambda_ssim, out3);
+    if (threadIdx.x == 0) *ticket = 0;
+}
+
+__global__ __launch_bounds__(256) void loss_reduce_kernel(int nblocks, const float* partial, int H, int W, float lambda_ssim, float* out) {
+    loss_reduce_body(nblocks, partial, H, W, lambda_ssim, out);
 }
 
 __global__ __launch_bounds__(256) void l1_ssim_bwd_kernel(const LossArgs a) {
@@ -370,6 +393,9 @@
     const size_t nb = (size_t)((width + kLT - 1) / kLT) * ((height + kLT - 1) / kLT);
     return 9 * (size_t)height * width + 2 * (nb + 8);
 }
+static int* loss_ticket(float* workspace, int height, int width) {
+    return reinterpret_cast<int*>(workspace + gs_loss_workspace_floats(height, width) - 2);
+}
 
 static int loss_fwd_launch(void* stream, int height, int width, float lambda_ssim, const float* render, const float* gt,
                            const float* mask, const float* const* slots, bool has_mask, int clamp_input, float* workspace, float* out3) {
@@ -384,10 +410,19 @@
     const int blocks = (int)loss_grid(loss_tile_count(height, width)).x;
     const size_t lds = sizeof(float) * (2 * kLR * kLRP + 4 * kLR * kHP);
     hipStream_t st = (hipStream_t)stream;
-    if (has_mask) hipLaunchKernelGGL(l1_ssim_fwd_kernel<true>, dim3((unsigned)blocks), dim3(256), lds, st, a);
-    else hipLaunchKernelGGL(l1_ssim_fwd_kernel<false>, dim3((unsigned)blocks), dim3(256), lds, st, a);
+    int* ticket = loss_ticket(workspace, height, width);
+    if (has_mask) hipLaunchKernelGGL(l1_ssim_fwd_kernel<true>, dim3((unsigned)blocks), dim3(256), lds, st, a, ticket, out3);
+    else hipLaunchKernelGGL(l1_ssim_fwd_kernel<false>, dim3((unsigned)blocks), dim3(256), lds, st, a, ticket, out3);
     GS_LAUNCH_CHECK("l1_ssim_fwd_kernel");
-    hipLaunchKernelGGL(loss_reduce_kernel, dim3(1), dim3(256), 0, st, blocks, a.partial, height, width, lambda_ssim, out3);
+    return GS_OK;
+}
+
+extern "C" int gs_loss_reduce(void* stream, int height, int width, float lambda_ssim, const float* workspace, float* out3) {
+    GS_REQUIRE(height > 2 * kHalo && width > 2 * kHalo, "image must be larger than the 11x11 window");
+    GS_REQUIRE(workspace && out3, "null pointer");
+    const int blocks = (int)loss_grid(loss_tile_count(height, width)).x;
+    hipLaunchKernelGGL(loss_reduce_kernel, dim3(1), dim3(256), 0, (hipStream_t)stream, blocks, workspace + 9 * (size_t)height * width,
+                       height, width, lambda_ssim, out3);
     GS_LAUNCH_CHECK("loss_reduce_kernel");
     return GS_OK;
 }
diff --git a/easy_gaussian_splatting_amd/loss.py b/easy_gaussian_splatting_amd/loss.py
--- a/easy_gaussian_splatting_amd/loss.py
+++ b/easy_gaussian_splatting_amd/loss.py
@@ -48,6 +48,7 @@
         r, g = render_img.contiguous(), gt_img.contiguous()
         m = None if mask is None else mask.contiguous()
         ws = torch.empty((int(L.gs_loss_workspace_floats(H, W)),), dtype=torch.float32, device=dev)
+        ws[-2:].zero_()
         out = torch.empty((3,), dtype=torch.float32, device=dev)
         st = torch.cuda.current_stream(dev).cuda_stream
         with torch.cuda.device(dev):
diff --git a/easy_gaussian_splatting_amd/rendering.py b/easy_gaussian_splatting_amd/rendering.py
--- a/easy_gaussian_splatting_amd/rendering.py
+++ b/easy_gaussian_splatting_amd/rendering.py
@@ -458,6 +458,7 @@
         cap_units = _quantize_up(max(int(hint.get("cap_units", 0)), (cap // 16 + 12 * C * tiles) if "cap_units" not in hint else 0, 256))
         cap_rows = _quantize_up(max(int(hint.get("cap_rows", 0)), cap if "cap_rows" not in hint else 0, 4096))
     walk = _WalkRecord() if need_grad else None
+    ucls = {"buf": None}
 
     lease = WS.pool.acquire(dev, st)
     lease.bind(WS.Layout(C, N, W, H, cap, coarse_cap, shift, flags, max(cap_units, 256), cap_rows), st)
@@ -500,6 +501,7 @@
                 P(WS.SLOTS)), "gs_bin_emit_sort"))
         if walk is not None:
             nat.check(L.gs_walk_mirror_set(walk.host.data_ptr()), "gs_walk_mirror_set")
+            nat.check(L.gs_unit_classes_set(_ptr(_unit_classes(ucls, lease.layout.cap_units, C, W, H, dev))), "gs_unit_classes_set")
         try:
             if ch == 3:
                 _stage("gs_blend_fwd", dev, lambda: nat.check(L.gs_blend_fwd(
@@ -516,6 +518,7 @@
         finally:
             if walk is not None:
                 L.gs_walk_mirror_set(None)
+                L.gs_unit_classes_set(None)
                 walk.event = torch.cuda.Event()
                 walk.event.record(tstream)
 
@@ -697,11 +700,21 @@
         meta._lease = ref
     state = dict(C=C, N=N, K=K, deg=deg, per_cam=per_cam, ch=ch, sh_jac=use_jac, n_isects=n_isects, n_buckets=n_buckets, radii=radii, lease=lease,
                  lease_ref=WS.LeaseRef(lease) if need_grad else None, factorised=factorised, pending=pending, late=state_late,
-                 walk=walk, hint_key=hint_key, backgrounds=backgrounds)
+                 walk=walk, ucls=ucls, hint_key=hint_key, backgrounds=backgrounds)
     if pending is not None:
         pending.lease_ref = WS.LeaseRef(lease)
     del ref
     return render_colors, render_alphas, meta, state
+
+
+def _unit_classes(holder: dict, cap_units: int, C: int, W: int, H: int, dev) -> Optional[Tensor]:
+    if not _BWD_CLASSES:
+        holder["buf"] = None
+        return None
+    n = int(nat.lib().gs_unit_classes_ints(cap_units, C, W, H))
+    if holder["buf"] is None or holder["buf"].numel() != n:
+        holder["buf"] = torch.empty((n,), dtype=torch.int32, device=dev)
+    return holder["buf"]
 
 
 def _settle_walk(s: dict, cfg: dict, render_colors: Tensor, render_alphas: Tensor) -> int:
@@ -731,6 +744,7 @@
             st = _stream(dev)
             sc, sa = torch.empty_like(render_colors), torch.empty_like(render_alphas)
             nat.check(L.gs_walk_mirror_set(walk.host.data_ptr()), "gs_walk_mirror_set")
+            nat.check(L.gs_unit_classes_set(_ptr(_unit_classes(s["ucls"], cu, C, W, H, dev))), "gs_unit_classes_set")
             try:
                 if s["ch"] == 3:
                     nat.check(L.gs_blend_fwd(st, C, W, H, P(WS.REC), _ptr(s["backgrounds"]), P(WS.ISECT_OFFSETS), P(WS.TILE_ORDER),
@@ -743,6 +757,7 @@
                                                 lease.ckpt_ext() if s["ch"] == 4 else None), "gs_blend_fwd_ch")
             finally:
                 L.gs_walk_mirror_set(None)
+                L.gs_unit_classes_set(None)
             torch.cuda.current_stream(dev).synchronize()
         units, storage, rows, fl = (int(v) for v in walk.host.tolist())
     with _state_lock:
@@ -767,7 +782,9 @@
             lease, tiles = state["lease"], meta["tile_width"] * meta["tile_height"]
             wstate = lease.view(WS.WALK_STATE, 8).clone()
             holder.debug.update(unit_counter=wstate[WS.WALK_UNITS:WS.WALK_UNITS + 1], walk_state=wstate,
-                                qcnt=lease.view(WS.QCNT, state["C"] * tiles * 4).clone(), unit_entries=nat.GS_UNIT)
+                                qcnt=lease.view(WS.QCNT, state["C"] * tiles * 4).clone(), unit_entries=nat.GS_UNIT,
+                                cap_units=lease.layout.cap_units, unit_desc=lease.view(WS.UNIT_DESC, 4 * lease.layout.cap_units).clone(),
+                                unit_classes=None if state["ucls"]["buf"] is None else state["ucls"]["buf"].clone())
             if state["n_isects"] is not None:
                 holder.debug["walked_isects"] = lease.view(WS.QMASK, max(state["n_isects"], 1))[: state["n_isects"]].count_nonzero()
         holder.lease_ref = state.pop("lease_ref")
@@ -801,7 +818,7 @@
             s["n_isects"], s["n_buckets"] = s["late"]["n_isects"], s["late"]["n_buckets"]
         P = lease.ptr
         n_rows = _settle_walk(s, cfg, render_colors, render_alphas)
-        ucls = torch.empty((int(L.gs_unit_classes_ints(lease.layout.cap_units, C, W, H)),), dtype=torch.int32, device=dev) if _BWD_CLASSES else None
+        ucls = s["ucls"]["buf"] if _BWD_CLASSES else None
         ch = s["ch"]
         if ch == 3:
             _stage("gs_blend_bwd", dev, lambda: nat.check(L.gs_blend_bwd(st, C, W, H, P(WS.REC), P(WS.QLIST), P(WS.QCNT),
diff --git a/easy_gaussian_splatting_amd/train_graph.py b/easy_gaussian_splatting_amd/train_graph.py
--- a/easy_gaussian_splatting_amd/train_graph.py
+++ b/easy_gaussian_splatting_amd/train_graph.py
@@ -131,6 +131,7 @@
         b["render_colors"] = torch.empty((1, H, W, 3), **f32)
         b["render_alphas"] = torch.empty((1, H, W, 1), **f32)
         b["loss_ws"] = torch.empty((int(L.gs_loss_workspace_floats(H, W)),), **f32)
+        b["loss_ws"][-2:].zero_()
         b["loss3"] = torch.zeros((3,), **f32)
         b["loss_ring"] = torch.zeros((self.LOSS_RING, 3), **f32)
         b["one"] = torch.ones((), **f32)
@@ -497,11 +498,15 @@
             self._ck(L.gs_bin_emit_sort(st, 1, N, self.tw, self.th, _p(b[bbox]), _p(b["depths"]), _p(b["ws"]), self.ws_bytes,
                                          _p(b["isect_offsets"]), self.cap, self.cap_tile, _p(b["keys_tmp"]), _p(b["slot_gid"]),
                                          _p(b["cum_tiles"]), None, _p(b["flatten_ids"]), _p(b["slots"])), "gs_bin_emit_sort")
-        self._ck(L.gs_blend_fwd(st, 1, W, H, _p(b["rec"]), _p(b["bg"]), _p(b["isect_offsets"]),
-                                 _p(b["tile_order"]), _p(b["flatten_ids"]), _p(b["slots"]), self.cap, _p(b["render_colors"]),
-                                 _p(b["render_alphas"]), _p(b["ckpt"]), _p(b["qlist"]), _p(b["qcnt"]), _p(b["qmask"]),
-                                 _p(b["unit_desc"]), self.cap_units, _p(b["row_base"]), self.cap_rows, _p(b["walk_state"])),
-                 "gs_blend_fwd")
+        nat.check(L.gs_unit_classes_set(_p(b["unit_cls"])), "gs_unit_classes_set")
+        try:
+            self._ck(L.gs_blend_fwd(st, 1, W, H, _p(b["rec"]), _p(b["bg"]), _p(b["isect_offsets"]),
+                                     _p(b["tile_order"]), _p(b["flatten_ids"]), _p(b["slots"]), self.cap, _p(b["render_colors"]),
+                                     _p(b["render_alphas"]), _p(b["ckpt"]), _p(b["qlist"]), _p(b["qcnt"]), _p(b["qmask"]),
+                                     _p(b["unit_desc"]), self.cap_units, _p(b["row_base"]), self.cap_rows, _p(b["walk_state"])),
+                     "gs_blend_fwd")
+        finally:
+            L.gs_unit_classes_set(None)
 
     def _enqueue_step(self):
         L, b, m, opt = nat.lib(), self.buf, self.model, self.opt
diff --git a/include/gs_raster.h b/include/gs_raster.h
--- a/include/gs_raster.h
+++ b/include/gs_raster.h
@@ -21,6 +21,7 @@
 #define GS_WALK_ROWS 3
 #define GS_WALK_FLAGS 4
 #define GS_WALK_SKIP 5
+#define GS_WALK_TICKET 8
 #define GS_WALK_RANGES 32
 #define GS_WALK_RANGE0 32
 #define GS_WALK_WORDS (GS_WALK_RANGE0 + 32 * GS_WALK_RANGES)
@@ -139,6 +140,10 @@
                   int32_t* slots, const int64_t* info_dev);
 
 size_t gs_walk_state_ints(int64_t n_isects);
+int gs_unit_classes_set(int32_t* unit_classes);
+int gs_post_walk(void* stream, int C, int width, int height, const uint8_t* qmask, int64_t n_isects, int32_t* row_base, int64_t cap_rows,
+                 int32_t* walk_state, const int32_t* unit_desc, const int32_t* qcnt, int64_t cap_units, int32_t* unit_classes);
+int gs_walk_clear(void* stream, uint8_t* qmask, int64_t n_isects, int32_t* walk_state, int32_t* unit_classes);
 int gs_blend_fwd(void* stream, int C, int width, int height, const float* rec,
                  const float* backgrounds, const int32_t* isect_offsets, const int32_t* tile_order,
                  const int32_t* flatten_ids, const int32_t* slots, int64_t n_isects, float* render_colors,
@@ -214,6 +219,7 @@
 int gs_l1_ssim_bwd(void* stream, int height, int width, float lambda_ssim, const float* render,
                    const float* gt, const float* mask, int clamp_input, const float* workspace,
                    const float* v_total, float* v_render);
+int gs_loss_reduce(void* stream, int height, int width, float lambda_ssim, const float* workspace, float* out3);
 
 int gs_l1_ssim_fwd_slots(void* stream, int height, int width, float lambda_ssim, const float* render,
                          const float* const* slots_dev, int has_mask, int clamp_input, float* workspace, float* out3);
```

New measurement: 741.8. No clear change (-0.7%).
